# NVIDIA-Merlin/distributed-embeddings

Measured on NVIDIA H100. Metric: DLRM global samples/sec (device-timed, max over ranks), higher is better.
Workload: dtype bf16

## Files before the change

### distributed_embeddings_b200/models/dlrm_fast.py

```python
from __future__ import annotations

import os
from typing import Optional

import torch
from torch import nn

from ..ops import _native
from ..parallel.comm import CommContext
from ..parallel.fused import FusedEngine
from ..utils import nvtx
from ..utils.lr_schedule import LearningRateScheduler
from .dlrm import DLRM


def _pad8(n: int) -> int:
  return (n + 7) // 8 * 8


class _Layer:

  def __init__(self, lin: nn.Linear, relu: bool):
    self.lin = lin
    self.relu = relu
    self.out_f, self.in_f = lin.weight.shape
    self.in_pad = _pad8(self.in_f)
    self.w_off = self.b_off = 0
    self.w_numel = self.out_f * self.in_pad
    self.b_numel = _pad8(self.out_f)


class DLRMTrainStep:

  def __init__(self, model: DLRM, lr: float = 24.0, embedding_optimizer: str = "sgd",
               scheduler: Optional[LearningRateScheduler] = None, use_cuda_graph: bool = True,
               embedding_optimizer_kwargs: Optional[dict] = None, overlap: bool = True,
               gemm: str = "cublas"):
    if gemm not in ("cublas", "fused_dgrad", "tcgen05", "tcgen05_pair"):
      raise ValueError("gemm must be cublas | fused_dgrad | tcgen05 | tcgen05_pair")
    self.gemm = gemm
    self.model = model
    self.emb = model.embedding
    if self.emb.backend != "fused":
      raise ValueError("DLRMTrainStep needs the fused embedding back end")
    self.dev = self.emb.device
    self.ops = _native.require()
    self.world = self.emb.world_size
    self.ctx = CommContext.for_group(self.emb.group, self.dev)
    self.scheduler = scheduler
    self.use_cuda_graph = use_cuda_graph
    self.overlap = overlap
    self.emb.set_optimizer(embedding_optimizer, lr=lr, **(embedding_optimizer_kwargs or {}))
    if self.emb._engine is None:
      self.emb._engine = FusedEngine(self.emb)
    self.engine: FusedEngine = self.emb._engine
    self.n_emb = len(model.table_sizes)
    self.dim = model.embedding_dim
    sp_env = os.environ.get("DE_B200_STREAM_PUSH", "auto")
    self._stream_push = self.world > 1 and (sp_env == "1" or (sp_env == "auto" and self.world >= 4))
    self._push_stream = torch.cuda.Stream(device=self.dev) if self._stream_push else None
    self._push_ready = torch.cuda.Event() if self._stream_push else None

    lins_b = [m for m in model.bottom_mlp.net if isinstance(m, nn.Linear)]
    lins_t = [m for m in model.top_mlp.net if isinstance(m, nn.Linear)]
    self.bottom = [_Layer(l, True) for l in lins_b]
    self.top = [_Layer(l, True) for l in lins_t[:-1]]
    self.head = _Layer(lins_t[-1], False)
    if self.head.out_f != 1:
      raise ValueError("the top MLP must end in a single logit")
    layers = self.bottom + self.top + [self.head]
    self._dp_slots = []
    pos = 0
    if len(self.emb.dp_layers):
      if embedding_optimizer != "sgd":
        raise ValueError("replicated tables in the fast step are updated by the dense SGD "
                         "kernel: use embedding_optimizer='sgd' or data_parallel_threshold=None")
      for layer in self.emb.dp_layers:
        w = layer.embeddings
        self._dp_slots.append((pos, tuple(w.shape)))
        pos += _pad8(w.numel())
    for L in layers:
      L.w_off = pos
      pos += L.w_numel
      L.b_off = pos
      pos += L.b_numel
    self.n_flat = pos
    dev = self.dev
    self.p32 = torch.zeros(pos, dtype=torch.float32, device=dev)
    self.p16 = torch.zeros(pos, dtype=torch.bfloat16, device=dev)
    if self.world > 1:
      self.gsym = self.ctx.alloc_multicast(pos * 4, "dense_grads") or \
          self.ctx.alloc(pos * 4, "dense_grads")
      self.allreduce_kind = "nvls_multimem" if getattr(self.gsym, "mc_ptr", 0) else "p2p"
      self.g32 = self.gsym.view(torch.float32, (pos,))
    else:
      self.gsym = None
      self.allreduce_kind = "none"
      self.g32 = torch.zeros(pos, dtype=torch.float32, device=dev)
    with torch.no_grad():
      dp_targets = []
      for layer, (off, shape) in zip(self.emb.dp_layers, self._dp_slots):
        n = shape[0] * shape[1]
        view = self.p32[off:off + n].view(shape)
        view.copy_(layer.embeddings.data)
        layer.embeddings.data = view
        dp_targets.append(self.g32[off:off + n].view(shape))
      if self._dp_slots:
        self.engine.set_dp_grad_targets(dp_targets)
        self.engine._tables_dirty = True
        self.engine._key = None
      for L in layers:
        wv = self.p32[L.w_off:L.w_off + L.w_numel].view(L.out_f, L.in_pad)
        wv[:, :L.in_f].copy_(L.lin.weight)
        L.lin.weight.data = wv[:, :L.in_f]
        bv = self.p32[L.b_off:L.b_off + L.out_f]
        bv.copy_(L.lin.bias)
        L.lin.bias.data = bv
        L.w16 = self.p16[L.w_off:L.w_off + L.w_numel].view(L.out_f, L.in_pad)
        L.b16 = self.p16[L.b_off:L.b_off + L.out_f]
        L.gw = self.g32[L.w_off:L.w_off + L.w_numel].view(L.out_f, L.in_pad)
        L.gb = self.g32[L.b_off:L.b_off + L.b_numel]
        L.w16T = torch.empty(L.in_pad, L.out_f, dtype=torch.bfloat16, device=dev)
      self.p16.copy_(self.p32)
      self._refresh_transposes()
    self.lr_t = torch.full((1,), float(lr), dtype=torch.float32, device=dev)
    self.engine.share_lr(self.lr_t)
    self.lr = float(lr)
    self.loss = torch.zeros(1, dtype=torch.float32, device=dev)
    self._batch = None
    self._graph = None
    self._side = torch.cuda.Stream(device=dev) if overlap else None
    self._wgrad_overlap = os.environ.get("DE_B200_WGRAD_STREAM", "auto")
    self._wstream = torch.cuda.Stream(device=dev) if overlap else None
    ar_env = os.environ.get("DE_B200_AR_OVERLAP", "auto")
    ar_on = ar_env == "1" or (ar_env == "auto" and self.world >= 4)
    self._ar_stream = torch.cuda.Stream(device=dev) if (overlap and self.world > 1 and ar_on) \
        else None

  def _refresh_transposes(self):
    if self.gemm == "cublas":
      return
    for L in self.bottom[1:] + self.top[1:]:
      L.w16T.copy_(L.w16.t())

  def _linear_fwd(self, L, x):
    if self.gemm in ("tcgen05", "tcgen05_pair"):
      pair = self.gemm == "tcgen05_pair" and L.out_f >= 256
      self.ops.gemm_tn_bias_act(x, L.w16, L.b16, L.y, True, 512 if pair else 0)
    else:
      torch._addmm_activation(L.b16, x, L.w16.t(), out=L.y)
    return L.y

  def _wgrad(self, L, x):
    use = self._wstream is not None and (
        self._wgrad_overlap == "1" or
        (self._wgrad_overlap == "auto" and (self._batch or 0) >= 49152))
    if not use:
      torch.mm(L.dy.t(), x, out_dtype=torch.float32, out=L.gw)
      return
    self._w_used = True
    self._wstream.wait_stream(torch.cuda.current_stream())
    with torch.cuda.stream(self._wstream):
      torch.mm(L.dy.t(), x, out_dtype=torch.float32, out=L.gw)

  def _dgrad_relu(self, L, x_below, dx, gb_below):
    if self.gemm == "cublas":
      torch.mm(L.dy, L.w16, out=dx)
      self.ops.relu_bwd_bias(dx, x_below, gb_below)
    else:
      self.ops.gemm_dgrad_relu_bias(L.dy, L.w16T, x_below, dx, gb_below, 0)

  def _alloc(self, b: int):
    dev, bf = self.dev, torch.bfloat16
    if self._stream_push:
      self.engine.enable_streamed_push(max(1024, -(-b // 16)))
    self.engine.prepare(b, [1] * self.n_emb, ids64=False)
    self.cat_stage = self.engine.in_flat[:self.n_emb * b].view(self.n_emb, b)
    self.num_in = torch.zeros(b, self.bottom[0].in_f, dtype=torch.float32, device=dev)
    self.lab_in = torch.zeros(b, dtype=torch.float32, device=dev)
    self.x0 = torch.zeros(b, self.bottom[0].in_pad, dtype=bf, device=dev)
    for L in self.bottom + self.top:
      L.y = torch.empty(b, L.out_f, dtype=bf, device=dev)
      L.dy = torch.empty(b, L.out_f, dtype=bf, device=dev)
    self.z = torch.zeros(b, self.top[0].in_pad, dtype=bf, device=dev)
    self.dz = torch.empty(b, self.top[0].in_pad, dtype=bf, device=dev)
    self._batch = b
    self._graph = None
    self._stage = [(torch.zeros_like(self.cat_stage), torch.zeros_like(self.num_in),
                    torch.zeros_like(self.lab_in)) for _ in range(2)]
    self._slot_dev = torch.zeros(1, dtype=torch.int32, device=dev)
    self._slot_host = torch.tensor([[0], [1]], dtype=torch.int32).pin_memory()
    self._h2d_done = [torch.cuda.Event(), torch.cuda.Event()]
    self._consumed = [torch.cuda.Event(), torch.cuda.Event()]
    self._prefetched = 0
    self._consumed_n = 0
    self._use_stage = False

  def _forward(self):
    ops = self.ops
    if self._use_stage:
      a, b_ = self._stage
      ops.select_copy([a[0], a[1], a[2]], [b_[0], b_[1], b_[2]],
                      [self.cat_stage, self.num_in, self.lab_in], self._slot_dev)
    eng = self.engine
    if self._side is not None:
      self._side.wait_stream(torch.cuda.current_stream())
      with torch.cuda.stream(self._side):
        eng.launch_forward()
    ops.cast_pad(self.num_in, self.x0)
    x = self.x0
    for L in self.bottom:
      x = self._linear_fwd(L, x)
    if self._side is not None:
      torch.cuda.current_stream().wait_stream(self._side)
    else:
      eng.launch_forward()
    if eng.out_needs_reduce:
      eng.wait_output()
      ops.interact_fwd(x, eng.out, self.n_emb, self.z, [])
    else:
      ops.interact_fwd(x, eng.out, self.n_emb, self.z, eng.sync_out_wait())
    x = self.z
    for L in self.top:
      x = self._linear_fwd(L, x)

  def _backward(self):
    ops, eng = self.ops, self.engine
    b = self._batch
    last = self.top[-1]
    self.loss.zero_()
    H = self.head
    ops.head_loss(last.y, H.w16.view(-1), H.b16, self.lab_in, 1.0 / b, last.dy,
                  H.gw.view(-1), H.gb, last.gb, self.loss, None)
    for i in range(len(self.top) - 1, -1, -1):
      L = self.top[i]
      x = self.top[i - 1].y if i > 0 else self.z
      dx = self.top[i - 1].dy if i > 0 else self.dz
      self._wgrad(L, x)
      if i > 0:
        self._dgrad_relu(L, x, dx, self.top[i - 1].gb)
      else:
        torch.mm(L.dy, L.w16, out=dx)
    if self._ar_stream is not None:
      ar = self._ar_stream
      ar.wait_stream(torch.cuda.current_stream())
      if getattr(self, "_w_used", False):
        ar.wait_stream(self._wstream)
      off = self.top[0].w_off
      with torch.cuda.stream(ar):
        self.ctx.allreduce_(self.gsym, self.n_flat - off, torch.float32, scale=1.0 / self.world,
                            byte_offset=off * 4, max_blocks=32)
    hb = self.bottom[-1]
    pushed = eng.streamed_push
    if pushed:
      eng.push_counters.zero_()
      self._push_ready.record(torch.cuda.current_stream())
      ops.interact_bwd(hb.y, eng.out, self.n_emb, self.dz, hb.dy, 0, 0, 1.0, eng.routes_stage,
                       len(eng.routes_stage_np), [], eng.push_counters, eng.push_chunk_rows)
      self._push_stream.wait_event(self._push_ready)
      with torch.cuda.stream(self._push_stream):
        eng.launch_streamed_push()
    else:
      ops.interact_bwd(hb.y, eng.out, self.n_emb, self.dz, hb.dy, 0, 0, 1.0, eng.routes_all,
                       len(eng.routes_all_np), eng.sync_grad_signal(), None, 0)
    if self._side is not None:
      self._side.wait_stream(torch.cuda.current_stream())
      if pushed:
        self._side.wait_stream(self._push_stream)
      with torch.cuda.stream(self._side):
        eng.backward_inplace()
    else:
      if pushed:
        torch.cuda.current_stream().wait_stream(self._push_stream)
      eng.backward_inplace()
    ops.relu_bwd_bias(hb.dy, hb.y, hb.gb)
    for i in range(len(self.bottom) - 1, -1, -1):
      L = self.bottom[i]
      x = self.bottom[i - 1].y if i > 0 else self.x0
      self._wgrad(L, x)
      if i > 0:
        self._dgrad_relu(L, x, self.bottom[i - 1].dy, self.bottom[i - 1].gb)
    if self._dp_slots and self._side is not None:
      torch.cuda.current_stream().wait_stream(self._side)
    if getattr(self, "_w_used", False):
      torch.cuda.current_stream().wait_stream(self._wstream)
      self._w_used = False
    if self.world > 1:
      if self._ar_stream is not None:
        ar = self._ar_stream
        ar.wait_stream(torch.cuda.current_stream())
        with torch.cuda.stream(ar):
          self.ctx.allreduce_(self.gsym, self.top[0].w_off, torch.float32, scale=1.0 / self.world)
        torch.cuda.current_stream().wait_stream(ar)
      else:
        self.ctx.allreduce_(self.gsym, self.n_flat, torch.float32, scale=1.0 / self.world)
    ops.dense_sgd(self.p32, self.p16, self.g32, self.lr_t, 1.0)
    self._refresh_transposes()
    if self._side is not None:
      torch.cuda.current_stream().wait_stream(self._side)

  def _step_impl(self):
    with nvtx.range("dlrm_forward"):
      self._forward()
    with nvtx.range("dlrm_backward_update"):
      self._backward()

  def set_lr(self, lr: float):
    self.lr = float(lr)
    self.lr_t.fill_(self.lr)
    if self.emb._fused_optimizer is not None:
      self.emb._fused_optimizer["lr"] = self.lr

  def load_batch(self, numerical, categorical, labels):
    b = int(numerical.shape[0])
    if b != self._batch:
      self._alloc(b)
    self.num_in.copy_(numerical, non_blocking=True)
    self.lab_in.copy_(labels.reshape(-1), non_blocking=True)
    if isinstance(categorical, (list, tuple)):
      for v, c in zip(self.engine.in_views, categorical):
        v.copy_(c.reshape(v.shape), non_blocking=True)
    else:
      self.cat_stage.copy_(categorical, non_blocking=True)

  def prefetch(self, numerical, categorical, labels):
    b = int(numerical.shape[0])
    if b != self._batch:
      self._alloc(b)
    if not self._use_stage:
      self._use_stage = True
      self._graph = None
      self._copy_stream = torch.cuda.Stream(device=self.dev)
    slot = self._prefetched & 1
    cs = self._copy_stream
    if self._prefetched >= 2:
      cs.wait_event(self._consumed[slot])
    with torch.cuda.stream(cs):
      st = self._stage[slot]
      st[0].copy_(categorical, non_blocking=True)
      st[1].copy_(numerical, non_blocking=True)
      st[2].copy_(labels.reshape(-1), non_blocking=True)
      self._h2d_done[slot].record(cs)
    self._prefetched += 1

  def run_prefetched(self) -> torch.Tensor:
    assert self._consumed_n < self._prefetched, "call prefetch() first"
    slot = self._consumed_n & 1
    main = torch.cuda.current_stream()
    main.wait_event(self._h2d_done[slot])
    self._slot_dev.copy_(self._slot_host[slot], non_blocking=True)
    loss = self.run()
    self._consumed[slot].record(main)
    self._consumed_n += 1
    return loss

  def run(self) -> torch.Tensor:
    if self.scheduler is not None:
      self.set_lr(self.scheduler.step())
    if not self.use_cuda_graph:
      self._step_impl()
      return self.loss
    if self._graph is None:
      self.lr_t.zero_()
      self.engine.dry_updates(True)
      s = torch.cuda.Stream(device=self.dev)
      s.wait_stream(torch.cuda.current_stream())
      with torch.cuda.stream(s):
        for _ in range(2):
          self._step_impl()
      torch.cuda.current_stream().wait_stream(s)
      torch.cuda.synchronize()
      self.engine.dry_updates(False)
      g = torch.cuda.CUDAGraph()
      with torch.cuda.graph(g):
        self._step_impl()
      self._graph = g
      self.set_lr(self.lr)
    self._graph.replay()
    return self.loss

  def step(self, numerical, categorical, labels) -> torch.Tensor:
    self.load_batch(numerical, categorical, labels)
    return self.run()
```

### distributed_embeddings_b200/ops/_native.py

```python
from __future__ import annotations

import os
import threading

import numpy as np
import torch

_PKG_DIR = os.path.dirname(os.path.dirname(os.path.abspath(__file__)))
SO_PATH = os.path.join(_PKG_DIR, "_C.so")

_lock = threading.Lock()
_loaded = False
_error = None

INPUT_DESC = np.dtype([
    ("table", "<u8"),
    ("ids", "<u8"),
    ("offsets", "<u8"),
    ("ids_off", "<i8"),
    ("id_shift", "<i8"),
    ("sub_rows", "<i8"),
    ("row_base", "<i8"),
    ("width", "<i4"),
    ("hotness", "<i4"),
    ("dst_col", "<i4"),
    ("combiner", "<i4"),
    ("local_table", "<i4"),
    ("flags", "<i4"),
    ("item_off", "<i8"),
    ("pad1", "<i8"),
])
TABLE_DESC = np.dtype([
    ("weight", "<u8"),
    ("state0", "<u8"),
    ("state1", "<u8"),
    ("rows", "<i8"),
    ("key_base", "<i8"),
    ("width", "<i4"),
    ("pad", "<i4"),
])

GRAD_ROUTE = np.dtype([
    ("dst", "<u8"),
    ("dst_stride", "<i8"),
    ("src_col", "<i4"),
    ("width", "<i4"),
    ("dst_col", "<i4"),
    ("pad", "<i4"),
])
SYNC_STATE_WORDS = 64
DTYPE_CODE = {torch.float32: 0, torch.bfloat16: 1, torch.float16: 2}

OPT_SGD, OPT_ADAGRAD, OPT_ROWWISE_ADAGRAD, OPT_ADAM, OPT_EMIT = 0, 1, 2, 3, 4
MAX_PEERS = 16


def load(required: bool = False) -> bool:
  global _loaded, _error
  if _loaded:
    return True
  with _lock:
    if _loaded:
      return True
    if _error is not None and not required:
      return False
    try:
      if not os.path.exists(SO_PATH):
        raise FileNotFoundError(
            f"{SO_PATH} is missing - run `python -m distributed_embeddings_b200.ops._build` "
            "(or `make`) to compile the sm_90a kernels")
      torch.ops.load_library(SO_PATH)
      sizes = list(torch.ops.de_b200.struct_sizes())
      mine = [INPUT_DESC.itemsize, TABLE_DESC.itemsize, MAX_PEERS, GRAD_ROUTE.itemsize,
              SYNC_STATE_WORDS]
      if sizes != mine:
        raise RuntimeError(f"descriptor layout mismatch: native {sizes} vs python {mine} "
                           "(stale _C.so? rebuild with python -m distributed_embeddings_b200.ops._build)")
      _loaded = True
      return True
    except Exception as e:
      _error = e
      if required:
        raise
      return False


def available() -> bool:
  return load(required=False)


_KERNELS_PER_OP = {
    "lookup_fwd": 1, "scatter_add_bwd": 1, "sort_items": 12, "segment_update": 1,
    "sync_only": 1, "push_segments": 1, "push_grad": 1, "rowslice_reduce": 1,
    "embedding_lookup_fwd": 1, "embedding_scatter_add": 1, "embedding_lookup_grad": 14,
    "row_to_split": 1, "hash_init": 1, "integer_lookup": 1, "barrier": 1, "allreduce": 1,
    "gather_segments": 1, "gather_ragged": 1, "copy_cast_2d": 1, "dense_sgd": 1, "interact_fwd": 1, "interact_bwd": 1,
    "relu_bwd_bias": 1, "head_loss": 1, "select_copy": 1, "cast_pad": 1, "gemm_tn_bias_act": 1, "gemm_dgrad_relu_bias": 1,
}
_launches = 0


class _OpsProxy:

  def __init__(self, ns):
    self._ns = ns
    self._cache = {}

  def __getattr__(self, name):
    fn = self._cache.get(name)
    if fn is None:
      raw = getattr(self._ns, name)
      k = _KERNELS_PER_OP.get(name, 0)

      def fn(*args, __raw=raw, __k=k, **kwargs):
        global _launches
        _launches += __k
        return __raw(*args, **kwargs)

      self._cache[name] = fn
    return fn


_proxy = None


def reset_launch_count():
  global _launches
  _launches = 0


def launch_count() -> int:
  return _launches


def require():
  global _proxy
  if not load(required=False):
    raise RuntimeError(
        "distributed_embeddings_b200: the native sm_90a extension is required for CUDA tensors "
        f"but could not be loaded ({_error!r}). There is no eager fallback on GPU.")
  if _proxy is None:
    _proxy = _OpsProxy(torch.ops.de_b200)
  return _proxy


def ops():
  return require()


def upload_struct_array(arr: np.ndarray, device) -> torch.Tensor:
  raw = torch.from_numpy(np.frombuffer(arr.tobytes(), dtype=np.uint8).copy())
  return raw.to(device)
```

### distributed_embeddings_b200/ops/csrc/bindings.cpp

```cpp
#include <ATen/cuda/CUDAContext.h>
#include <c10/cuda/CUDAGuard.h>
#include <c10/cuda/CUDAStream.h>
#include <cuda_runtime.h>
#include <torch/library.h>
#include <torch/torch.h>

#include <cstdlib>
#include <cstring>
#include <mutex>
#include <string>
#include <unordered_map>
#include <vector>

#include "de_b200.h"

namespace {

using at::Tensor;

#define DE_CUDA_CHECK(expr)                                                              \
  do {                                                                                   \
    cudaError_t _e = (expr);                                                             \
    TORCH_CHECK(_e == cudaSuccess, "CUDA error in " #expr ": ", cudaGetErrorString(_e)); \
  } while (0)

cudaStream_t cur_stream() { return at::cuda::getCurrentCUDAStream().stream(); }

int sm_count() {
  static int cached = -1;
  if (cached < 0) cached = at::cuda::getCurrentDeviceProperties()->multiProcessorCount;
  return cached;
}

de::PeerPtrs to_peers(at::IntArrayRef ptrs) {
  TORCH_CHECK(ptrs.size() <= de::kMaxPeers, "at most ", de::kMaxPeers, " peers are supported");
  de::PeerPtrs p;
  std::memset(&p, 0, sizeof(p));
  for (size_t i = 0; i < ptrs.size(); ++i) p.p[i] = reinterpret_cast<void*>(ptrs[i]);
  return p;
}

void check_launch() {
  cudaError_t e = cudaGetLastError();
  TORCH_CHECK(e == cudaSuccess, "kernel launch failed: ", cudaGetErrorString(e));
}

struct SyncCtx {
  de::PeerPtrs flags;
  uint32_t* state;
  int* error_flag;
  unsigned long long timeout;
  int rank, world;
};
std::vector<SyncCtx>& sync_ctxs() {
  static std::vector<SyncCtx> v;
  return v;
}
std::mutex& sync_mutex() {
  static std::mutex m;
  return m;
}

int64_t sync_ctx_create(at::IntArrayRef flag_ptrs, Tensor state, int64_t rank, int64_t world,
                        int64_t timeout_cycles, int64_t error_ptr) {
  TORCH_CHECK(state.is_cuda() && state.scalar_type() == at::kInt && state.is_contiguous() &&
                  state.numel() >= de::kSyncStateWords,
              "sync state must be an int32 CUDA tensor of >= ", de::kSyncStateWords, " words");
  SyncCtx c;
  c.flags = to_peers(flag_ptrs);
  c.state = reinterpret_cast<uint32_t*>(state.data_ptr<int>());
  c.error_flag = reinterpret_cast<int*>(error_ptr);
  c.timeout = static_cast<unsigned long long>(timeout_cycles);
  c.rank = static_cast<int>(rank);
  c.world = static_cast<int>(world);
  std::lock_guard<std::mutex> lock(sync_mutex());
  sync_ctxs().push_back(c);
  return static_cast<int64_t>(sync_ctxs().size()) - 1;
}

de::SyncArgs to_sync(at::IntArrayRef spec) {
  de::SyncArgs a = de::no_sync();
  if (spec.size() == 0) return a;
  TORCH_CHECK(spec.size() == 5, "sync spec = {handle, wait_ch, wait_abs_ch, signal_ch, slot}");
  SyncCtx c;
  {
    std::lock_guard<std::mutex> lock(sync_mutex());
    TORCH_CHECK(spec[0] >= 0 && spec[0] < static_cast<int64_t>(sync_ctxs().size()),
                "unknown sync context");
    c = sync_ctxs()[spec[0]];
  }
  for (int i = 1; i <= 3; ++i)
    TORCH_CHECK(spec[i] >= -1 && spec[i] < de::kSyncChannels, "sync channel out of range");
  TORCH_CHECK(spec[4] >= 0 && spec[4] < 2 * de::kSyncChannels, "sync counter slot out of range");
  a.flags = c.flags;
  a.state = c.state;
  a.error_flag = c.error_flag;
  a.timeout = c.timeout;
  a.rank = c.rank;
  a.world = c.world;
  a.wait_ch = static_cast<int32_t>(spec[1]);
  a.wait_abs_ch = static_cast<int32_t>(spec[2]);
  a.signal_ch = static_cast<int32_t>(spec[3]);
  a.counter_slot = static_cast<int32_t>(spec[4]);
  return a;
}

int dtype_code(at::ScalarType t) {
  if (t == at::kFloat) return 0;
  if (t == at::kBFloat16) return 1;
  if (t == at::kHalf) return 2;
  TORCH_CHECK(false, "activations / gradients must be fp32, bf16 or fp16");
  return -1;
}

void sync_only(at::IntArrayRef sync) {
  de::launch_sync_only(to_sync(sync), cur_stream());
  check_launch();
}

std::vector<int64_t> struct_sizes() {
  return {static_cast<int64_t>(sizeof(de::InputDesc)), static_cast<int64_t>(sizeof(de::TableDesc)),
          static_cast<int64_t>(de::kMaxPeers), static_cast<int64_t>(sizeof(de::GradRoute)),
          static_cast<int64_t>(de::kSyncStateWords)};
}

void lookup_fwd(const Tensor& descs, int64_t n_inputs, int64_t batch, int64_t src_batch,
                int64_t dst_batch, int64_t dst_stride, at::IntArrayRef src_ptrs,
                at::IntArrayRef dst_ptrs, int64_t rot, bool ids64, int64_t act_dtype, bool vec4,
                at::IntArrayRef sync, int64_t tile_samples, int64_t table_dtype, bool vec8) {
  TORCH_CHECK(descs.is_cuda(), "descs must live on the GPU");
  TORCH_CHECK(table_dtype >= 0 && table_dtype <= 2, "table_dtype: 0 fp32, 1 bf16, 2 fp16");
  c10::cuda::CUDAGuard guard(descs.device());
  de::launch_lookup_fwd(reinterpret_cast<const de::InputDesc*>(descs.data_ptr()),
                        static_cast<int>(n_inputs), batch, src_batch, dst_batch, dst_stride,
                        to_peers(src_ptrs), to_peers(dst_ptrs), static_cast<int>(rot), ids64,
                        static_cast<int>(act_dtype), vec4, sm_count(), cur_stream(),
                        to_sync(sync), static_cast<int>(tile_samples),
                        static_cast<int>(table_dtype), vec8);
  check_launch();
}

void scatter_add_bwd(const Tensor& descs, int64_t n_inputs, int64_t batch, int64_t src_batch,
                     int64_t grad_batch, int64_t grad_stride, at::IntArrayRef src_ptrs,
                     at::IntArrayRef grad_ptrs, int64_t rot, double scale, int64_t scale_ptr,
                     bool ids64, int64_t act_dtype, bool vec4, bool vec8, at::IntArrayRef sync,
                     bool staged) {
  TORCH_CHECK(descs.is_cuda(), "descs must live on the GPU");
  c10::cuda::CUDAGuard guard(descs.device());
  de::launch_scatter_add_bwd(reinterpret_cast<const de::InputDesc*>(descs.data_ptr()),
                             static_cast<int>(n_inputs), batch, src_batch, grad_batch, grad_stride,
                             to_peers(src_ptrs), to_peers(grad_ptrs), static_cast<int>(rot),
                             static_cast<float>(scale), reinterpret_cast<const float*>(scale_ptr),
                             ids64, static_cast<int>(act_dtype), vec4, sm_count(), cur_stream(),
                             vec8, to_sync(sync), staged);
  check_launch();
}

int bit_length(int64_t v) {
  int b = 0;
  while (v > 0) {
    ++b;
    v >>= 1;
  }
  return b < 1 ? 1 : b;
}

bool use_own_sort() {
  static const bool own = [] {
    const char* v = std::getenv("DE_B200_SORT");
    return !(v != nullptr && std::string(v) == "cub");
  }();
  return own;
}

std::tuple<Tensor, Tensor> radix_sort_pairs(const Tensor& keys, const Tensor& items,
                                            int64_t end_bit) {
  TORCH_CHECK(keys.is_cuda() && keys.scalar_type() == at::kLong && keys.is_contiguous());
  TORCH_CHECK(items.is_cuda() && items.scalar_type() == at::kInt && items.is_contiguous() &&
              items.numel() == keys.numel());
  c10::cuda::CUDAGuard guard(keys.device());
  const int64_t n = keys.numel();
  TORCH_CHECK(n < (int64_t(1) << 31), "own radix sort: too many items");
  Tensor ka = keys.clone(), ia = items.clone();
  Tensor kb = at::empty_like(ka), ib = at::empty_like(ia);
  if (n == 0) return {ka, ia};
  Tensor temp = at::empty({static_cast<int64_t>(de::radix_sort_temp_bytes(n))},
                          at::TensorOptions().device(keys.device()).dtype(at::kByte));
  int where = de::radix_sort_pairs(temp.data_ptr(), ka.data_ptr<int64_t>(),
                                   reinterpret_cast<uint32_t*>(ia.data_ptr<int>()),
                                   kb.data_ptr<int64_t>(),
                                   reinterpret_cast<uint32_t*>(ib.data_ptr<int>()), n,
                                   static_cast<int>(end_bit), cur_stream());
  check_launch();
  if (where == 0) return {ka, ia};
  return {kb, ib};
}

std::tuple<Tensor, Tensor> radix_sort_pairs32(const Tensor& keys, const Tensor& items,
                                              int64_t end_bit) {
  TORCH_CHECK(keys.is_cuda() && keys.scalar_type() == at::kInt && keys.is_contiguous());
  TORCH_CHECK(items.is_cuda() && items.scalar_type() == at::kInt && items.is_contiguous() &&
              items.numel() == keys.numel());
  c10::cuda::CUDAGuard guard(keys.device());
  const int64_t n = keys.numel();
  TORCH_CHECK(n < (int64_t(1) << 31), "own radix sort: too many items");
  Tensor ka = keys.clone(), ia = items.clone();
  Tensor kb = at::empty_like(ka), ib = at::empty_like(ia);
  Tensor out = at::empty({n}, keys.options().dtype(at::kLong));
  if (n == 0) return {out, ia};
  Tensor temp = at::empty({static_cast<int64_t>(de::radix_sort_temp_bytes(n))},
                          at::TensorOptions().device(keys.device()).dtype(at::kByte));
  int where = de::radix_sort_pairs32(
      temp.data_ptr(), reinterpret_cast<uint32_t*>(ka.data_ptr<int>()),
      reinterpret_cast<uint32_t*>(ia.data_ptr<int>()),
      reinterpret_cast<uint32_t*>(kb.data_ptr<int>()),
      reinterpret_cast<uint32_t*>(ib.data_ptr<int>()), out.data_ptr<int64_t>(), n,
      static_cast<int>(end_bit), cur_stream());
  check_launch();
  return {out, where == 0 ? ia : ib};
}

std::tuple<Tensor, Tensor> head_segments(const Tensor& sorted_keys) {
  TORCH_CHECK(sorted_keys.is_cuda() && sorted_keys.scalar_type() == at::kLong &&
              sorted_keys.is_contiguous());
  c10::cuda::CUDAGuard guard(sorted_keys.device());
  const int64_t n = sorted_keys.numel();
  auto i64 = at::TensorOptions().device(sorted_keys.device()).dtype(at::kLong);
  Tensor seg_start = at::empty({n + 1}, i64);
  Tensor n_unique = at::zeros({1}, i64);
  if (n == 0) return {seg_start, n_unique};
  Tensor temp = at::empty({static_cast<int64_t>(de::head_segments_temp_bytes(n))},
                          at::TensorOptions().device(sorted_keys.device()).dtype(at::kByte));
  de::head_segments(temp.data_ptr(), sorted_keys.data_ptr<int64_t>(), n,
                    seg_start.data_ptr<int64_t>(), n_unique.data_ptr<int64_t>(), cur_stream());
  check_launch();
  return {seg_start, n_unique};
}

std::tuple<Tensor, Tensor, Tensor, Tensor> sort_items(const Tensor& descs, const Tensor& tables,
                                                      int64_t n_tables, int64_t n_inputs,
                                                      int64_t batch, int64_t src_batch,
                                                      at::IntArrayRef src_ptrs, bool ids64,
                                                      int64_t n_items, int64_t total_rows,
                                                      bool prefill_sentinel) {
  TORCH_CHECK(descs.is_cuda() && tables.is_cuda());
  TORCH_CHECK(n_inputs * batch < (int64_t(1) << 32),
              "sorted update: n_inputs * batch = ", n_inputs * batch, " does not fit 32-bit items");
  c10::cuda::CUDAGuard guard(descs.device());
  auto stream = cur_stream();
  auto i64 = at::TensorOptions().device(descs.device()).dtype(at::kLong);
  auto i32 = at::TensorOptions().device(descs.device()).dtype(at::kInt);
  Tensor keys = prefill_sentinel ? at::full({n_items}, total_rows, i64) : at::empty({n_items}, i64);
  Tensor keys_sorted = at::empty({n_items}, i64);
  Tensor items = at::empty({n_items}, i32), items_sorted = at::empty({n_items}, i32);
  Tensor seg_start = at::empty({n_items + 1}, i64);
  Tensor n_unique = at::zeros({1}, i64);
  if (n_items == 0) return {keys_sorted, items_sorted, seg_start, n_unique};
  if (use_own_sort() && total_rows < (int64_t(1) << 32) - 1) {
    TORCH_CHECK(n_items < (int64_t(1) << 31), "own radix sort: too many items");
    Tensor k32a = prefill_sentinel
                      ? at::full({n_items}, static_cast<int64_t>(static_cast<int32_t>(
                                                static_cast<uint32_t>(total_rows))), i32)
                      : at::empty({n_items}, i32);
    Tensor k32b = at::empty({n_items}, i32);
    de::launch_build_keys(reinterpret_cast<const de::InputDesc*>(descs.data_ptr()),
                          reinterpret_cast<const de::TableDesc*>(tables.data_ptr()),
                          static_cast<int>(n_tables), static_cast<int>(n_inputs), batch,
                          src_batch, to_peers(src_ptrs), ids64, k32a.data_ptr(),
                          reinterpret_cast<uint32_t*>(items.data_ptr<int>()), sm_count(), stream,
                          true);
    check_launch();
    size_t sort_bytes = de::radix_sort_temp_bytes(n_items);
    size_t head_bytes = de::head_segments_temp_bytes(n_items);
    Tensor temp = at::empty({static_cast<int64_t>(std::max(sort_bytes, head_bytes))},
                            at::TensorOptions().device(descs.device()).dtype(at::kByte));
    int where = de::radix_sort_pairs32(
        temp.data_ptr(), reinterpret_cast<uint32_t*>(k32a.data_ptr<int>()),
        reinterpret_cast<uint32_t*>(items.data_ptr<int>()),
        reinterpret_cast<uint32_t*>(k32b.data_ptr<int>()),
        reinterpret_cast<uint32_t*>(items_sorted.data_ptr<int>()),
        keys_sorted.data_ptr<int64_t>(), n_items, bit_length(total_rows), stream);
    if (where == 0) std::swap(items, items_sorted);
    de::head_segments(temp.data_ptr(), keys_sorted.data_ptr<int64_t>(), n_items,
                      seg_start.data_ptr<int64_t>(), n_unique.data_ptr<int64_t>(), stream);
    check_launch();
    return {keys_sorted, items_sorted, seg_start, n_unique};
  }
  de::launch_build_keys(reinterpret_cast<const de::InputDesc*>(descs.data_ptr()),
                        reinterpret_cast<const de::TableDesc*>(tables.data_ptr()),
                        static_cast<int>(n_tables), static_cast<int>(n_inputs), batch, src_batch,
                        to_peers(src_ptrs), ids64, keys.data_ptr<int64_t>(),
                        reinterpret_cast<uint32_t*>(items.data_ptr<int>()), sm_count(), stream);
  check_launch();
  if (use_own_sort()) {
    TORCH_CHECK(n_items < (int64_t(1) << 31), "own radix sort: too many items");
    size_t sort_bytes = de::radix_sort_temp_bytes(n_items);
    size_t head_bytes = de::head_segments_temp_bytes(n_items);
    Tensor temp = at::empty({static_cast<int64_t>(std::max(sort_bytes, head_bytes))},
                            at::TensorOptions().device(descs.device()).dtype(at::kByte));
    int where = de::radix_sort_pairs(temp.data_ptr(), keys.data_ptr<int64_t>(),
                                     reinterpret_cast<uint32_t*>(items.data_ptr<int>()),
                                     keys_sorted.data_ptr<int64_t>(),
                                     reinterpret_cast<uint32_t*>(items_sorted.data_ptr<int>()),
                                     n_items, bit_length(total_rows), stream);
    if (where == 0) {
      std::swap(keys, keys_sorted);
      std::swap(items, items_sorted);
    }
    de::head_segments(temp.data_ptr(), keys_sorted.data_ptr<int64_t>(), n_items,
                      seg_start.data_ptr<int64_t>(), n_unique.data_ptr<int64_t>(), stream);
    check_launch();
    return {keys_sorted, items_sorted, seg_start, n_unique};
  }
  size_t sort_bytes = de::sort_pairs_temp_bytes(n_items);
  size_t uniq_bytes = de::unique_temp_bytes(n_items);
  Tensor temp = at::empty({static_cast<int64_t>(std::max(sort_bytes, uniq_bytes)) + 16},
                          at::TensorOptions().device(descs.device()).dtype(at::kByte));
  de::sort_pairs(temp.data_ptr(), sort_bytes, keys.data_ptr<int64_t>(),
                 keys_sorted.data_ptr<int64_t>(),
                 reinterpret_cast<const uint32_t*>(items.data_ptr<int>()),
                 reinterpret_cast<uint32_t*>(items_sorted.data_ptr<int>()), n_items,
                 bit_length(total_rows), stream);
  de::unique_segments(temp.data_ptr(), uniq_bytes, keys_sorted.data_ptr<int64_t>(), n_items,
                      seg_start.data_ptr<int64_t>(), n_unique.data_ptr<int64_t>(), stream);
  check_launch();
  return {keys_sorted, items_sorted, seg_start, n_unique};
}

void segment_update(const Tensor& descs, const Tensor& tables, int64_t n_tables, int64_t batch,
                    int64_t grad_batch, int64_t grad_stride, at::IntArrayRef grad_ptrs,
                    const Tensor& sorted_keys, const Tensor& sorted_items, const Tensor& seg_start,
                    const Tensor& n_unique, int64_t opt_kind, double lr, double eps, double beta1,
                    double beta2, double bias1, double bias2, double grad_scale,
                    double weight_decay, int64_t lr_ptr, const c10::optional<Tensor>& emit_keys,
                    const c10::optional<Tensor>& emit_rows, int64_t max_width, int64_t act_dtype,
                    bool vec4, const c10::optional<Tensor>& scratch, int64_t step_ptr,
                    int64_t table_dtype) {
  c10::cuda::CUDAGuard guard(descs.device());
  TORCH_CHECK(table_dtype >= 0 && table_dtype <= 2, "table_dtype: 0 fp32, 1 bf16, 2 fp16");
  de::OptimizerArgs opt;
  opt.kind = static_cast<int32_t>(opt_kind);
  opt.lr = static_cast<float>(lr);
  opt.eps = static_cast<float>(eps);
  opt.beta1 = static_cast<float>(beta1);
  opt.beta2 = static_cast<float>(beta2);
  opt.bias1 = static_cast<float>(bias1);
  opt.bias2 = static_cast<float>(bias2);
  opt.grad_scale = static_cast<float>(grad_scale);
  opt.weight_decay = static_cast<float>(weight_decay);
  opt.lr_ptr = reinterpret_cast<const float*>(lr_ptr);
  opt.step_ptr = reinterpret_cast<const float*>(step_ptr);
  if (opt.kind == de::kOptEmit) TORCH_CHECK(emit_keys.has_value() && emit_rows.has_value());
  if (scratch.has_value() && vec4 && max_width <= 128 && opt.kind != de::kOptEmit) {
    const int64_t n_items = sorted_keys.numel();
    const int64_t sw = (max_width + 3) / 4 * 4;
    TORCH_CHECK(scratch->scalar_type() == at::kFloat && scratch->is_contiguous() &&
                    scratch->numel() >= ((n_items + 31) / 32) * sw,
                "scratch too small for the balanced update");
    bool ok = de::launch_balanced_update(
        reinterpret_cast<const de::InputDesc*>(descs.data_ptr()),
        reinterpret_cast<const de::TableDesc*>(tables.data_ptr()), static_cast<int>(n_tables),
        batch, grad_batch, grad_stride, to_peers(grad_ptrs), sorted_keys.data_ptr<int64_t>(),
        reinterpret_cast<const uint32_t*>(sorted_items.data_ptr<int>()), n_items,
        seg_start.data_ptr<int64_t>(), n_unique.data_ptr<int64_t>(), opt,
        scratch->data_ptr<float>(), static_cast<int>(sw), static_cast<int>(max_width),
        static_cast<int>(act_dtype), sm_count(), cur_stream(), static_cast<int>(table_dtype));
    TORCH_CHECK(ok, "balanced update launch failed");
    check_launch();
    return;
  }
  de::launch_segment_update(
      reinterpret_cast<const de::InputDesc*>(descs.data_ptr()),
      reinterpret_cast<const de::TableDesc*>(tables.data_ptr()), static_cast<int>(n_tables), batch,
      grad_batch, grad_stride, to_peers(grad_ptrs), sorted_keys.data_ptr<int64_t>(),
      reinterpret_cast<const uint32_t*>(sorted_items.data_ptr<int>()),
      seg_start.data_ptr<int64_t>(), n_unique.data_ptr<int64_t>(), sorted_keys.numel(), opt,
      emit_keys.has_value() ? emit_keys->data_ptr<int64_t>() : nullptr,
      emit_rows.has_value() ? emit_rows->data_ptr<float>() : nullptr, static_cast<int>(max_width),
      static_cast<int>(act_dtype), vec4, sm_count(), cur_stream(), static_cast<int>(table_dtype));
  check_launch();
}

Tensor upload_bytes(const void* host, size_t bytes, const at::Device& dev) {
  Tensor t = at::empty({static_cast<int64_t>(bytes)},
                       at::TensorOptions().device(dev).dtype(at::kByte));
  DE_CUDA_CHECK(cudaMemcpyAsync(t.data_ptr(), host, bytes, cudaMemcpyHostToDevice, cur_stream()));
  return t;
}

de::InputDesc single_desc(const void* table, const Tensor& values,
                          const c10::optional<Tensor>& offsets, int64_t hotness, int64_t rows,
                          int64_t width, int64_t combiner) {
  de::InputDesc d;
  std::memset(&d, 0, sizeof(d));
  d.table = table;
  d.ids = values.data_ptr();
  d.offsets = offsets.has_value() ? offsets->data_ptr<int64_t>() : nullptr;
  d.sub_rows = rows;
  d.width = static_cast<int32_t>(width);
  d.hotness = offsets.has_value() ? 0 : static_cast<int32_t>(hotness);
  d.combiner = static_cast<int32_t>(combiner);
  return d;
}

void check_ids(const Tensor& values, const c10::optional<Tensor>& offsets) {
  TORCH_CHECK(values.is_cuda() && values.is_contiguous(), "ids must be a contiguous CUDA tensor");
  TORCH_CHECK(values.scalar_type() == at::kInt || values.scalar_type() == at::kLong,
              "ids must be int32 or int64");
  if (offsets.has_value())
    TORCH_CHECK(offsets->is_cuda() && offsets->scalar_type() == at::kLong &&
                    offsets->is_contiguous(),
                "row_splits must be a contiguous int64 CUDA tensor");
}

Tensor embedding_lookup_fwd(const Tensor& param, const Tensor& values,
                            const c10::optional<Tensor>& offsets, int64_t hotness, int64_t batch,
                            int64_t combiner, bool out_bf16) {
  const auto pt = param.scalar_type();
  TORCH_CHECK(param.is_cuda() && param.dim() == 2 &&
                  (pt == at::kFloat || pt == at::kBFloat16 || pt == at::kHalf) &&
                  param.is_contiguous(),
              "param must be a contiguous fp32, bf16 or fp16 [rows, width] CUDA tensor");
  check_ids(values, offsets);
  c10::cuda::CUDAGuard guard(param.device());
  const int64_t width = param.size(1);
  const int tdt = dtype_code(pt);
  Tensor out = at::empty({batch, width}, param.options().dtype(out_bf16 ? at::kBFloat16 : pt));
  if (batch == 0) return out;
  de::InputDesc d = single_desc(param.data_ptr(), values, offsets, hotness, param.size(0), width,
                                combiner);
  Tensor dd = upload_bytes(&d, sizeof(d), param.device());
  de::PeerPtrs src, dst;
  std::memset(&src, 0, sizeof(src));
  std::memset(&dst, 0, sizeof(dst));
  dst.p[0] = out.data_ptr();
  const int64_t avg_hot = std::max<int64_t>(1, values.numel() / std::max<int64_t>(batch, 1));
  int64_t lanes_per_row = 1;
  while (lanes_per_row < (width + 3) / 4 && lanes_per_row < 32) lanes_per_row *= 2;
  const int64_t ts = std::max<int64_t>(32 / lanes_per_row, std::min<int64_t>(32, 64 / avg_hot));
  de::launch_lookup_fwd(reinterpret_cast<const de::InputDesc*>(dd.data_ptr()), 1, batch, batch,
                        batch, width, src, dst, 0, values.scalar_type() == at::kLong,
                        out_bf16 ? 1 : tdt, width % 4 == 0, sm_count(), cur_stream(),
                        de::no_sync(), static_cast<int>(std::max<int64_t>(1, ts)), tdt,
                        width % 8 == 0 && reinterpret_cast<uintptr_t>(param.data_ptr()) % 16 == 0);
  check_launch();
  return out;
}

void embedding_scatter_add(Tensor dst, const Tensor& values, const c10::optional<Tensor>& offsets,
                           int64_t hotness, int64_t batch, int64_t combiner, const Tensor& grad,
                           double scale) {
  TORCH_CHECK(dst.is_cuda() && dst.dim() == 2 && dst.scalar_type() == at::kFloat &&
              dst.is_contiguous());
  TORCH_CHECK(grad.is_cuda() && grad.dim() == 2 && grad.stride(1) == 1);
  check_ids(values, offsets);
  if (batch == 0) return;
  c10::cuda::CUDAGuard guard(dst.device());
  const int64_t width = dst.size(1);
  de::InputDesc d = single_desc(dst.data_ptr(), values, offsets, hotness, dst.size(0), width,
                                combiner);
  Tensor dd = upload_bytes(&d, sizeof(d), dst.device());
  de::PeerPtrs src, gp;
  std::memset(&src, 0, sizeof(src));
  std::memset(&gp, 0, sizeof(gp));
  gp.p[0] = grad.data_ptr();
  const int gdt = dtype_code(grad.scalar_type());
  const int64_t gstride = grad.stride(0);
  const bool vec4 = (width % 4 == 0) && (gstride % 4 == 0) &&
                    (reinterpret_cast<uintptr_t>(grad.data_ptr()) % 16 == 0);
  de::launch_scatter_add_bwd(reinterpret_cast<const de::InputDesc*>(dd.data_ptr()), 1, batch,
                             batch, batch, gstride, src, gp, 0, static_cast<float>(scale), nullptr,
                             values.scalar_type() == at::kLong, gdt, vec4, sm_count(),
                             cur_stream(), false, de::no_sync());
  check_launch();
}

std::tuple<Tensor, Tensor> embedding_lookup_grad(const Tensor& values,
                                                 const c10::optional<Tensor>& offsets,
                                                 int64_t hotness, int64_t batch, int64_t combiner,
                                                 const Tensor& grad, int64_t num_rows) {
  TORCH_CHECK(grad.is_cuda() && grad.dim() == 2 && grad.stride(1) == 1);
  check_ids(values, offsets);
  c10::cuda::CUDAGuard guard(grad.device());
  const int64_t width = grad.size(1);
  const int64_t n_items = values.numel();
  auto f32 = grad.options().dtype(at::kFloat);
  auto i64 = grad.options().dtype(at::kLong);
  if (n_items == 0) return {at::empty({0}, i64), at::empty({0, width}, f32)};
  de::InputDesc d = single_desc(nullptr, values, offsets, hotness, num_rows, width, combiner);
  de::TableDesc t;
  std::memset(&t, 0, sizeof(t));
  t.rows = num_rows;
  t.width = static_cast<int32_t>(width);
  Tensor dd = upload_bytes(&d, sizeof(d), grad.device());
  Tensor td = upload_bytes(&t, sizeof(t), grad.device());
  auto sorted = sort_items(dd, td, 1, 1, batch, batch, {}, values.scalar_type() == at::kLong,
                           n_items, num_rows, false);
  Tensor emit_keys = at::empty({n_items}, i64);
  Tensor emit_rows = at::empty({n_items, width}, f32);
  const int gdt = dtype_code(grad.scalar_type());
  const int64_t gstride = grad.stride(0);
  const bool vec4 = (width % 4 == 0) && (gstride % 4 == 0) &&
                    (reinterpret_cast<uintptr_t>(grad.data_ptr()) % 16 == 0);
  std::vector<int64_t> gp = {reinterpret_cast<int64_t>(grad.data_ptr())};
  segment_update(dd, td, 1, batch, batch, gstride, gp, std::get<0>(sorted), std::get<1>(sorted),
                 std::get<2>(sorted), std::get<3>(sorted), de::kOptEmit, 0, 0, 0, 0, 1, 1, 1.0, 0, 0,
                 emit_keys, emit_rows, width, gdt, vec4, c10::nullopt, 0, 0);
  int64_t n_unique = std::get<3>(sorted).item<int64_t>();
  if (n_unique > 0) {
    int64_t last = emit_keys.narrow(0, n_unique - 1, 1).item<int64_t>();
    if (last >= num_rows) --n_unique;
  }
  return {emit_keys.narrow(0, 0, n_unique), emit_rows.narrow(0, 0, n_unique)};
}

Tensor row_to_split(const Tensor& indices, int64_t num_rows) {
  TORCH_CHECK(indices.is_cuda() && indices.dim() == 2 && indices.size(1) == 2 &&
                  indices.scalar_type() == at::kLong && indices.is_contiguous(),
              "indices must be a contiguous int64 [nnz, 2] CUDA tensor");
  c10::cuda::CUDAGuard guard(indices.device());
  Tensor splits = at::empty({num_rows + 1}, indices.options());
  de::launch_row_to_split(indices.data_ptr<int64_t>(), indices.size(0), num_rows,
                          splits.data_ptr<int64_t>(), cur_stream());
  check_launch();
  return splits;
}

void hash_init(Tensor table) {
  TORCH_CHECK(table.is_cuda() && table.scalar_type() == at::kLong && table.is_contiguous());
  c10::cuda::CUDAGuard guard(table.device());
  de::launch_hash_init(table.data_ptr<int64_t>(), table.numel() / 2, cur_stream());
  check_launch();
}

Tensor integer_lookup(Tensor table, Tensor count, Tensor next_index, const Tensor& keys,
                      int64_t capacity) {
  TORCH_CHECK(table.is_cuda() && count.is_cuda() && next_index.is_cuda() && keys.is_cuda());
  TORCH_CHECK(table.scalar_type() == at::kLong && keys.scalar_type() == at::kLong &&
              next_index.scalar_type() == at::kLong && count.scalar_type() == at::kInt);
  c10::cuda::CUDAGuard guard(table.device());
  Tensor k = keys.contiguous();
  Tensor out = at::empty_like(k);
  de::launch_integer_lookup(table.data_ptr<int64_t>(), table.numel() / 2,
                            reinterpret_cast<uint32_t*>(count.data_ptr<int>()),
                            next_index.data_ptr<int64_t>(), k.data_ptr<int64_t>(), k.numel(),
                            capacity, out.data_ptr<int64_t>(), cur_stream());
  check_launch();
  return out;
}

void barrier(at::IntArrayRef flag_ptrs, Tensor epoch, int64_t rank, int64_t world, int64_t channel,
             int64_t timeout_cycles, int64_t error_ptr) {
  c10::cuda::CUDAGuard guard(epoch.device());
  de::launch_barrier(to_peers(flag_ptrs), reinterpret_cast<uint32_t*>(epoch.data_ptr<int>()),
                     static_cast<int>(rank), static_cast<int>(world), static_cast<int>(channel),
                     static_cast<unsigned long long>(timeout_cycles),
                     reinterpret_cast<int*>(error_ptr), cur_stream());
  check_launch();
}

void allreduce(at::IntArrayRef buf_ptrs, at::IntArrayRef flag_ptrs, Tensor epoch, int64_t rank,
               int64_t world, int64_t n_elems, double scale, bool bf16, int64_t channel,
               int64_t timeout_cycles, int64_t error_ptr, int64_t mc_ptr, int64_t max_blocks) {
  c10::cuda::CUDAGuard guard(epoch.device());
  if (mc_ptr != 0) {
    de::launch_allreduce_multimem(reinterpret_cast<void*>(mc_ptr), to_peers(flag_ptrs),
                                  reinterpret_cast<uint32_t*>(epoch.data_ptr<int>()),
                                  static_cast<int>(rank), static_cast<int>(world), n_elems,
                                  static_cast<float>(scale), bf16, static_cast<int>(channel),
                                  static_cast<unsigned long long>(timeout_cycles),
                                  reinterpret_cast<int*>(error_ptr), sm_count(), cur_stream(),
                         static_cast<int>(max_blocks));
  } else {
    de::launch_allreduce(to_peers(buf_ptrs), to_peers(flag_ptrs),
                         reinterpret_cast<uint32_t*>(epoch.data_ptr<int>()),
                         static_cast<int>(rank), static_cast<int>(world), n_elems,
                         static_cast<float>(scale), bf16, static_cast<int>(channel),
                         static_cast<unsigned long long>(timeout_cycles),
                         reinterpret_cast<int*>(error_ptr), sm_count(), cur_stream(),
                         static_cast<int>(max_blocks));
  }
  check_launch();
}

void p2p_store_bench(const Tensor& src, int64_t dst_ptr, int64_t n_rows, int64_t row_bytes,
                     int64_t vec_bytes, int64_t dst_stride, int64_t unroll, int64_t blocks,
                     int64_t threads) {
  TORCH_CHECK(src.is_cuda() && src.is_contiguous() &&
              src.numel() * src.element_size() >= n_rows * row_bytes);
  TORCH_CHECK(row_bytes % vec_bytes == 0 && (vec_bytes == 4 || vec_bytes == 8 || vec_bytes == 16));
  TORCH_CHECK((row_bytes / vec_bytes >= 32 && (row_bytes / vec_bytes) % 32 == 0) ||
              32 % (row_bytes / vec_bytes) == 0);
  TORCH_CHECK(unroll >= 1 && unroll <= 8 && threads % 32 == 0 && threads <= 1024);
  c10::cuda::CUDAGuard guard(src.device());
  de::launch_p2p_store_bench(src.data_ptr(), reinterpret_cast<void*>(dst_ptr), n_rows,
                             static_cast<int>(row_bytes), static_cast<int>(vec_bytes), dst_stride,
                             static_cast<int>(unroll), static_cast<int>(blocks),
                             static_cast<int>(threads), cur_stream());
  check_launch();
}

void push_segments(const Tensor& segs, const Tensor& src, at::IntArrayRef dst_ptrs,
                   int64_t max_seg_elems, at::IntArrayRef sync) {
  TORCH_CHECK(segs.is_cuda() && segs.scalar_type() == at::kLong && segs.is_contiguous() &&
              segs.dim() == 2 && segs.size(1) == 4);
  TORCH_CHECK(src.is_cuda() && src.is_contiguous() &&
              (src.element_size() == 4 || src.element_size() == 8));
  c10::cuda::CUDAGuard guard(src.device());
  de::launch_push_segments(segs.data_ptr<int64_t>(), static_cast<int>(segs.size(0)),
                           src.data_ptr(), to_peers(dst_ptrs),
                           static_cast<int>(src.element_size()), max_seg_elems, sm_count(),
                           cur_stream(), to_sync(sync));
  check_launch();
}

void push_grad(const Tensor& routes, int64_t n_routes, const Tensor& src, int64_t dst_dtype,
               double scale, at::IntArrayRef sync) {
  TORCH_CHECK(routes.is_cuda() && routes.scalar_type() == at::kByte &&
              routes.numel() >= n_routes * static_cast<int64_t>(sizeof(de::GradRoute)));
  TORCH_CHECK(src.is_cuda() && src.dim() == 2 && src.stride(1) == 1);
  c10::cuda::CUDAGuard guard(src.device());
  de::launch_push_grad(reinterpret_cast<const de::GradRoute*>(routes.data_ptr()),
                       static_cast<int>(n_routes), src.data_ptr(), src.stride(0),
                       dtype_code(src.scalar_type()), static_cast<int>(dst_dtype), src.size(0),
                       static_cast<float>(scale), sm_count(), cur_stream(), to_sync(sync));
  check_launch();
}

void stream_push(at::IntArrayRef src_ptrs, at::IntArrayRef dst_ptrs, at::IntArrayRef row_bytes,
                 const Tensor& counters, int64_t chunk_rows, int64_t rows, int64_t blocks,
                 at::IntArrayRef sync) {
  TORCH_CHECK(src_ptrs.size() == dst_ptrs.size() && src_ptrs.size() == row_bytes.size() &&
              src_ptrs.size() <= de::kMaxPeers);
  TORCH_CHECK(counters.is_cuda() && counters.scalar_type() == at::kInt && chunk_rows > 0 &&
              counters.numel() >= (rows + chunk_rows - 1) / chunk_rows);
  de::PushPlan plan;
  std::memset(&plan, 0, sizeof(plan));
  plan.n = static_cast<int32_t>(src_ptrs.size());
  for (size_t i = 0; i < src_ptrs.size(); ++i) {
    TORCH_CHECK(row_bytes[i] % 16 == 0 && src_ptrs[i] % 16 == 0 && dst_ptrs[i] % 16 == 0,
                "streamed push needs 16-byte aligned rows");
    plan.src[i] = reinterpret_cast<const void*>(src_ptrs[i]);
    plan.dst[i] = reinterpret_cast<void*>(dst_ptrs[i]);
    plan.row_bytes[i] = row_bytes[i];
  }
  c10::cuda::CUDAGuard guard(counters.device());
  de::SyncArgs sa = to_sync(sync);
  de::launch_stream_push(plan, reinterpret_cast<const uint32_t*>(counters.data_ptr<int>()),
                         static_cast<int>(chunk_rows), rows, sa.timeout, sa.error_flag,
                         static_cast<int>(blocks), cur_stream(), sa);
  check_launch();
}

void rowslice_reduce(const Tensor& partial, int64_t out_ptr, int64_t out_stride,
                     int64_t out_dtype, const Tensor& cols) {
  TORCH_CHECK(partial.is_cuda() && partial.dim() == 3 && partial.scalar_type() == at::kFloat &&
              partial.is_contiguous());
  TORCH_CHECK(cols.is_cuda() && cols.scalar_type() == at::kInt && cols.is_contiguous() &&
              cols.dim() == 2 && cols.size(1) == 3);
  c10::cuda::CUDAGuard guard(partial.device());
  de::launch_rowslice_reduce(partial.data_ptr<float>(), static_cast<int>(partial.size(0)),
                             partial.size(1), partial.size(2), reinterpret_cast<void*>(out_ptr),
                             out_stride, static_cast<int>(out_dtype), cols.data_ptr<int>(),
                             static_cast<int>(cols.size(0)), cur_stream());
  check_launch();
}

void gather_segments(const Tensor& segs, at::IntArrayRef src_ptrs, Tensor dst,
                     int64_t max_seg_elems) {
  TORCH_CHECK(segs.is_cuda() && segs.scalar_type() == at::kLong && segs.is_contiguous());
  TORCH_CHECK(dst.is_cuda() && dst.is_contiguous());
  c10::cuda::CUDAGuard guard(dst.device());
  de::launch_gather_segments(segs.data_ptr<int64_t>(), static_cast<int>(segs.size(0)),
                             to_peers(src_ptrs), dst.data_ptr(),
                             static_cast<int>(dst.element_size()), max_seg_elems, cur_stream());
  check_launch();
}

void gather_ragged(const Tensor& segs, at::IntArrayRef val_ptrs, at::IntArrayRef split_ptrs,
                   Tensor dst_vals, Tensor goff, int64_t b, int64_t max_cap) {
  TORCH_CHECK(segs.is_cuda() && segs.scalar_type() == at::kLong && segs.is_contiguous());
  TORCH_CHECK(goff.is_cuda() && goff.scalar_type() == at::kLong && dst_vals.is_cuda());
  c10::cuda::CUDAGuard guard(dst_vals.device());
  de::launch_gather_ragged(segs.data_ptr<int64_t>(), static_cast<int>(segs.size(0)),
                           to_peers(val_ptrs), to_peers(split_ptrs), dst_vals.data_ptr(),
                           goff.data_ptr<int64_t>(), b, static_cast<int>(val_ptrs.size()),
                           static_cast<int>(dst_vals.element_size()), max_cap, cur_stream());
  check_launch();
}

void select_copy(at::TensorList src0, at::TensorList src1, at::TensorList dst,
                 const Tensor& slot_flag) {
  TORCH_CHECK(src0.size() == dst.size() && src1.size() == dst.size() && dst.size() <= 4);
  TORCH_CHECK(slot_flag.is_cuda() && slot_flag.scalar_type() == at::kInt);
  const void* s0[4];
  const void* s1[4];
  void* d[4];
  int64_t nb[4];
  for (size_t i = 0; i < dst.size(); ++i) {
    TORCH_CHECK(src0[i].is_contiguous() && src1[i].is_contiguous() && dst[i].is_contiguous());
    nb[i] = dst[i].numel() * dst[i].element_size();
    TORCH_CHECK(src0[i].numel() * src0[i].element_size() == nb[i] &&
                src1[i].numel() * src1[i].element_size() == nb[i] && nb[i] % 16 == 0,
                "select_copy segments must match and be multiples of 16 bytes");
    s0[i] = src0[i].data_ptr();
    s1[i] = src1[i].data_ptr();
    d[i] = dst[i].data_ptr();
  }
  c10::cuda::CUDAGuard guard(slot_flag.device());
  de::launch_select_copy(s0, s1, d, nb, static_cast<int>(dst.size()), slot_flag.data_ptr<int>(),
                         sm_count(), cur_stream());
  check_launch();
}

void copy_cast_2d(const Tensor& src, int64_t dst_ptr, int64_t dst_stride, int64_t dst_dtype,
                  double scale) {
  TORCH_CHECK(src.is_cuda() && src.dim() == 2 && src.stride(1) == 1);
  c10::cuda::CUDAGuard guard(src.device());
  de::launch_copy_cast_2d(src.data_ptr(), src.stride(0), reinterpret_cast<void*>(dst_ptr),
                          dst_stride, src.size(0), src.size(1), dtype_code(src.scalar_type()),
                          static_cast<int>(dst_dtype), static_cast<float>(scale), cur_stream());
  check_launch();
}

void check_bf16_2d(const Tensor& t, const char* name) {
  TORCH_CHECK(t.is_cuda() && t.dim() == 2 && t.scalar_type() == at::kBFloat16 && t.stride(1) == 1,
              name, " must be a 2-D bf16 CUDA tensor with unit inner stride");
}

void interact_fwd(const Tensor& bottom, const Tensor& emb, int64_t n_emb, Tensor z,
                  at::IntArrayRef sync) {
  check_bf16_2d(bottom, "bottom");
  check_bf16_2d(emb, "emb");
  check_bf16_2d(z, "z");
  c10::cuda::CUDAGuard guard(bottom.device());
  const int64_t dim = bottom.size(1);
  TORCH_CHECK(emb.size(1) == n_emb * dim);
  const int64_t need = (n_emb + 1) * n_emb / 2 + dim;
  TORCH_CHECK(z.size(1) >= need, "z is too narrow");
  bool ok = de::launch_interact_fwd(bottom.data_ptr(), bottom.stride(0), emb.data_ptr(),
                                    emb.stride(0), static_cast<int>(n_emb), static_cast<int>(dim),
                                    z.data_ptr(), z.stride(0), static_cast<int>(z.size(1)),
                                    bottom.size(0), sm_count(), cur_stream(), to_sync(sync));
  TORCH_CHECK(ok, "unsupported interaction shape (n_emb <= 31, dim in {16,32,64,128})");
  check_launch();
}

void interact_bwd(const Tensor& bottom, const Tensor& emb, int64_t n_emb, const Tensor& dz,
                  Tensor dbottom, int64_t demb_ptr, int64_t demb_stride, double emb_grad_scale,
                  const c10::optional<Tensor>& routes, int64_t n_routes, at::IntArrayRef sync,
                  const c10::optional<Tensor>& done_counters, int64_t chunk_rows) {
  check_bf16_2d(bottom, "bottom");
  check_bf16_2d(emb, "emb");
  check_bf16_2d(dz, "dz");
  check_bf16_2d(dbottom, "dbottom");
  if (routes.has_value())
    TORCH_CHECK(routes->is_cuda() && routes->scalar_type() == at::kByte &&
                routes->numel() >= n_routes * static_cast<int64_t>(sizeof(de::GradRoute)));
  c10::cuda::CUDAGuard guard(bottom.device());
  const int64_t dim = bottom.size(1);
  bool ok = de::launch_interact_bwd(bottom.data_ptr(), bottom.stride(0), emb.data_ptr(),
                                    emb.stride(0), static_cast<int>(n_emb), static_cast<int>(dim),
                                    dz.data_ptr(), dz.stride(0), dbottom.data_ptr(),
                                    dbottom.stride(0), reinterpret_cast<void*>(demb_ptr),
                                    demb_stride, static_cast<float>(emb_grad_scale),
                                    bottom.size(0), sm_count(), cur_stream(),
                                    routes.has_value()
                                        ? reinterpret_cast<const de::GradRoute*>(routes->data_ptr())
                                        : nullptr,
                                    static_cast<int>(n_routes), to_sync(sync),
                                    done_counters.has_value()
                                        ? reinterpret_cast<uint32_t*>(done_counters->data_ptr<int>())
                                        : nullptr,
                                    static_cast<int>(chunk_rows));
  TORCH_CHECK(ok, "unsupported interaction shape (n_emb <= 31, dim in {32,64,128}; routed / "
                  "signalling launches need dim in {64,128} and 16-byte aligned rows)");
  check_launch();
}

void avgpool_fwd(const Tensor& x, int64_t n, Tensor out, int64_t stride) {
  check_bf16_2d(x, "x");
  check_bf16_2d(out, "out");
  const int64_t out_len = (n + stride - 1) / stride;
  TORCH_CHECK(x.size(1) >= n && out.size(1) >= out_len && out.size(0) == x.size(0));
  const int64_t pad = std::max<int64_t>(0, (out_len - 1) * stride + stride - n);
  c10::cuda::CUDAGuard guard(x.device());
  de::launch_avgpool_fwd(x.data_ptr(), x.stride(0), static_cast<int>(n), out.data_ptr(),
                         out.stride(0), static_cast<int>(out_len), static_cast<int>(stride),
                         static_cast<int>(pad / 2), x.size(0), cur_stream());
  check_launch();
}

void avgpool_bwd(const Tensor& dout, Tensor dx, int64_t n, int64_t stride) {
  check_bf16_2d(dout, "dout");
  check_bf16_2d(dx, "dx");
  const int64_t out_len = (n + stride - 1) / stride;
  TORCH_CHECK(dx.size(1) >= n && dout.size(1) >= out_len && dout.size(0) == dx.size(0));
  const int64_t pad = std::max<int64_t>(0, (out_len - 1) * stride + stride - n);
  c10::cuda::CUDAGuard guard(dx.device());
  de::launch_avgpool_bwd(dout.data_ptr(), dout.stride(0), static_cast<int>(out_len),
                         dx.data_ptr(), dx.stride(0), static_cast<int>(n),
                         static_cast<int>(stride), static_cast<int>(pad / 2), dx.size(0),
                         cur_stream());
  check_launch();
}

void relu_bwd_bias(Tensor dy, const Tensor& y, Tensor db) {
  check_bf16_2d(dy, "dy");
  check_bf16_2d(y, "y");
  TORCH_CHECK(dy.is_contiguous() && y.is_contiguous() && dy.size(1) % 8 == 0);
  TORCH_CHECK(db.is_cuda() && db.scalar_type() == at::kFloat && db.numel() >= dy.size(1));
  c10::cuda::CUDAGuard guard(dy.device());
  de::launch_relu_bwd_bias(dy.data_ptr(), y.data_ptr(), db.data_ptr<float>(), dy.size(0),
                           static_cast<int>(dy.size(1)), cur_stream());
  check_launch();
}

void head_loss(const Tensor& x, const Tensor& w, const Tensor& bias, const Tensor& labels,
               double inv_batch, Tensor dx, Tensor dw, Tensor db, Tensor dbias_prev,
               Tensor loss_sum, const c10::optional<Tensor>& logits) {
  check_bf16_2d(x, "x");
  TORCH_CHECK(x.is_contiguous() && dx.is_contiguous());
  TORCH_CHECK(w.scalar_type() == at::kBFloat16 && bias.scalar_type() == at::kBFloat16);
  TORCH_CHECK(labels.scalar_type() == at::kFloat && labels.is_contiguous());
  c10::cuda::CUDAGuard guard(x.device());
  bool ok = de::launch_head_loss(x.data_ptr(), static_cast<int>(x.size(1)), w.data_ptr(),
                                 bias.data_ptr(), labels.data_ptr<float>(), x.size(0),
                                 static_cast<float>(inv_batch), dx.data_ptr(),
                                 dw.data_ptr<float>(), db.data_ptr<float>(),
                                 dbias_prev.data_ptr<float>(), loss_sum.data_ptr<float>(),
                                 logits.has_value() ? logits->data_ptr<float>() : nullptr,
                                 sm_count(), cur_stream());
  TORCH_CHECK(ok, "head_loss supports K in {64,128,256,512,1024}");
  check_launch();
}

void dense_sgd(Tensor p32, Tensor p16, Tensor g32, const Tensor& lr, double grad_scale) {
  TORCH_CHECK(p32.is_cuda() && p32.scalar_type() == at::kFloat && g32.scalar_type() == at::kFloat &&
              p16.scalar_type() == at::kBFloat16 && lr.scalar_type() == at::kFloat);
  TORCH_CHECK(p32.numel() % 4 == 0 && p32.numel() == g32.numel() && p32.numel() == p16.numel());
  c10::cuda::CUDAGuard guard(p32.device());
  de::launch_sgd_update(p32.data_ptr<float>(), p16.data_ptr(), g32.data_ptr<float>(),
                        lr.data_ptr<float>(), static_cast<float>(grad_scale), p32.numel(),
                        sm_count(), cur_stream());
  check_launch();
}

void cast_pad(const Tensor& src, Tensor dst) {
  TORCH_CHECK(src.is_cuda() && src.scalar_type() == at::kFloat && src.is_contiguous());
  TORCH_CHECK(dst.scalar_type() == at::kBFloat16 && dst.is_contiguous() &&
              dst.size(0) == src.size(0) && dst.size(1) >= src.size(1));
  c10::cuda::CUDAGuard guard(src.device());
  de::launch_cast_pad(src.data_ptr<float>(), static_cast<int>(src.size(1)), dst.data_ptr(),
                      static_cast<int>(dst.size(1)), src.size(0), cur_stream());
  check_launch();
}

void gemm_tn_bias_act(const Tensor& a, const Tensor& b, const c10::optional<Tensor>& bias,
                      Tensor out, bool relu, int64_t block_n) {
  check_bf16_2d(a, "a");
  check_bf16_2d(b, "b");
  check_bf16_2d(out, "out");
  TORCH_CHECK(a.size(1) == b.size(1) && out.size(0) == a.size(0) && out.size(1) == b.size(0),
              "shape mismatch");
  if (bias.has_value())
    TORCH_CHECK(bias->is_cuda() && bias->scalar_type() == at::kBFloat16 && bias->is_contiguous() &&
                bias->numel() == b.size(0));
  c10::cuda::CUDAGuard guard(a.device());
  bool ok = de::launch_gemm_tn_bias_act(
      a.data_ptr(), a.stride(0), b.data_ptr(), b.stride(0),
      bias.has_value() ? bias->data_ptr() : nullptr, out.data_ptr(), out.stride(0),
      static_cast<int>(a.size(0)), static_cast<int>(b.size(0)), static_cast<int>(a.size(1)), relu,
      static_cast<int>(block_n), sm_count(), cur_stream());
  TORCH_CHECK(ok, "gemm_tn_bias_act: unsupported shape/alignment or launch failure");
  check_launch();
}

void gemm_dgrad_relu_bias(const Tensor& dy, const Tensor& wt, const Tensor& act, Tensor dx,
                          Tensor colsum, int64_t block_n) {
  check_bf16_2d(dy, "dy");
  check_bf16_2d(wt, "wt");
  check_bf16_2d(act, "act");
  check_bf16_2d(dx, "dx");
  TORCH_CHECK(dy.size(1) == wt.size(1) && dx.size(0) == dy.size(0) && dx.size(1) == wt.size(0) &&
              act.size(0) == dx.size(0) && act.size(1) == dx.size(1), "shape mismatch");
  TORCH_CHECK(colsum.is_cuda() && colsum.scalar_type() == at::kFloat &&
              colsum.numel() >= dx.size(1));
  c10::cuda::CUDAGuard guard(dy.device());
  bool ok = de::launch_gemm_tn_fused(
      dy.data_ptr(), dy.stride(0), wt.data_ptr(), wt.stride(0), nullptr, dx.data_ptr(),
      dx.stride(0), static_cast<int>(dy.size(0)), static_cast<int>(wt.size(0)),
      static_cast<int>(dy.size(1)), 2, act.data_ptr(), act.stride(0), colsum.data_ptr<float>(),
      static_cast<int>(block_n), sm_count(), cur_stream());
  TORCH_CHECK(ok, "gemm_dgrad_relu_bias: unsupported shape/alignment or launch failure");
  check_launch();
}

Tensor symm_alloc(int64_t nbytes, int64_t device_index) {
  c10::cuda::CUDAGuard guard(static_cast<c10::DeviceIndex>(device_index));
  void* ptr = nullptr;
  const size_t padded = (static_cast<size_t>(nbytes) + 255) & ~static_cast<size_t>(255);
  DE_CUDA_CHECK(cudaMalloc(&ptr, padded));
  DE_CUDA_CHECK(cudaMemset(ptr, 0, padded));
  DE_CUDA_CHECK(cudaDeviceSynchronize());
  auto deleter = [](void* p) { cudaFree(p); };
  return at::from_blob(ptr, {static_cast<int64_t>(padded)}, deleter,
                       at::TensorOptions()
                           .device(at::Device(at::kCUDA, static_cast<c10::DeviceIndex>(device_index)))
                           .dtype(at::kByte));
}

Tensor ipc_get_handle(const Tensor& buf) {
  TORCH_CHECK(buf.is_cuda());
  cudaIpcMemHandle_t h;
  DE_CUDA_CHECK(cudaIpcGetMemHandle(&h, buf.data_ptr()));
  Tensor out = at::empty({static_cast<int64_t>(sizeof(h))}, at::TensorOptions().dtype(at::kByte));
  std::memcpy(out.data_ptr(), &h, sizeof(h));
  return out;
}

int64_t ipc_open(const Tensor& handle, int64_t device_index) {
  TORCH_CHECK(!handle.is_cuda() && handle.numel() == sizeof(cudaIpcMemHandle_t));
  c10::cuda::CUDAGuard guard(static_cast<c10::DeviceIndex>(device_index));
  cudaIpcMemHandle_t h;
  std::memcpy(&h, handle.data_ptr(), sizeof(h));
  void* ptr = nullptr;
  DE_CUDA_CHECK(cudaIpcOpenMemHandle(&ptr, h, cudaIpcMemLazyEnablePeerAccess));
  return reinterpret_cast<int64_t>(ptr);
}

void ipc_close(int64_t ptr, int64_t device_index) {
  c10::cuda::CUDAGuard guard(static_cast<c10::DeviceIndex>(device_index));
  cudaIpcCloseMemHandle(reinterpret_cast<void*>(ptr));
}

int64_t host_device_pointer(const Tensor& host) {
  TORCH_CHECK(!host.is_cuda());
  void* dptr = nullptr;
  DE_CUDA_CHECK(cudaHostGetDevicePointer(&dptr, host.data_ptr(), 0));
  return reinterpret_cast<int64_t>(dptr);
}

}

TORCH_LIBRARY(de_b200, m) {
  m.def("struct_sizes() -> int[]", &struct_sizes);
  m.def(
      "sync_ctx_create(int[] flag_ptrs, Tensor state, int rank, int world, int timeout_cycles, "
      "int error_ptr) -> int",
      &sync_ctx_create);
  m.def("sync_only(int[] sync) -> ()", &sync_only);
  m.def(
      "lookup_fwd(Tensor descs, int n_inputs, int batch, int src_batch, int dst_batch, "
      "int dst_stride, int[] src_ptrs, int[] dst_ptrs, int rot, bool ids64, int act_dtype, "
      "bool vec4, int[] sync, int tile_samples, int table_dtype=0, bool vec8=False) -> ()",
      &lookup_fwd);
  m.def(
      "scatter_add_bwd(Tensor descs, int n_inputs, int batch, int src_batch, int grad_batch, "
      "int grad_stride, int[] src_ptrs, int[] grad_ptrs, int rot, float scale, int scale_ptr, bool ids64, "
      "int act_dtype, bool vec4, bool vec8, int[] sync, bool staged) -> ()",
      &scatter_add_bwd);
  m.def(
      "sort_items(Tensor descs, Tensor tables, int n_tables, int n_inputs, int batch, "
      "int src_batch, int[] src_ptrs, bool ids64, int n_items, int total_rows, "
      "bool prefill_sentinel) -> "
      "(Tensor, Tensor, Tensor, Tensor)",
      &sort_items);
  m.def("radix_sort_pairs(Tensor keys, Tensor items, int end_bit) -> (Tensor, Tensor)",
        &radix_sort_pairs);
  m.def("radix_sort_pairs32(Tensor keys, Tensor items, int end_bit) -> (Tensor, Tensor)",
        &radix_sort_pairs32);
  m.def("head_segments(Tensor sorted_keys) -> (Tensor, Tensor)", &head_segments);
  m.def(
      "segment_update(Tensor descs, Tensor tables, int n_tables, int batch, int grad_batch, "
      "int grad_stride, int[] grad_ptrs, Tensor sorted_keys, Tensor sorted_items, "
      "Tensor seg_start, Tensor n_unique, int opt_kind, float lr, float eps, float beta1, "
      "float beta2, float bias1, float bias2, float grad_scale, float weight_decay, int lr_ptr, "
      "Tensor? emit_keys, Tensor? emit_rows, int max_width, int act_dtype, bool vec4, "
      "Tensor? scratch, int step_ptr, int table_dtype=0) -> ()",
      &segment_update);
  m.def(
      "embedding_lookup_fwd(Tensor param, Tensor values, Tensor? offsets, int hotness, int batch, "
      "int combiner, bool out_bf16) -> Tensor",
      &embedding_lookup_fwd);
  m.def(
      "embedding_scatter_add(Tensor(a!) dst, Tensor values, Tensor? offsets, int hotness, "
      "int batch, int combiner, Tensor grad, float scale) -> ()",
      &embedding_scatter_add);
  m.def(
      "embedding_lookup_grad(Tensor values, Tensor? offsets, int hotness, int batch, int combiner, "
      "Tensor grad, int num_rows) -> (Tensor, Tensor)",
      &embedding_lookup_grad);
  m.def("row_to_split(Tensor indices, int num_rows) -> Tensor", &row_to_split);
  m.def("hash_init(Tensor(a!) table) -> ()", &hash_init);
  m.def(
      "integer_lookup(Tensor(a!) table, Tensor(b!) count, Tensor(c!) next_index, Tensor keys, "
      "int capacity) -> Tensor",
      &integer_lookup);
  m.def(
      "barrier(int[] flag_ptrs, Tensor(a!) epoch, int rank, int world, int channel, "
      "int timeout_cycles, int error_ptr) -> ()",
      &barrier);
  m.def(
      "allreduce(int[] buf_ptrs, int[] flag_ptrs, Tensor(a!) epoch, int rank, int world, "
      "int n_elems, float scale, bool bf16, int channel, int timeout_cycles, "
      "int error_ptr, int mc_ptr, int max_blocks) -> ()",
      &allreduce);
  m.def("gather_segments(Tensor segs, int[] src_ptrs, Tensor(a!) dst, int max_seg_elems) -> ()",
        &gather_segments);
  m.def(
      "p2p_store_bench(Tensor src, int dst_ptr, int n_rows, int row_bytes, int vec_bytes, "
      "int dst_stride, int unroll, int blocks, int threads) -> ()",
      &p2p_store_bench);
  m.def(
      "push_segments(Tensor segs, Tensor src, int[] dst_ptrs, int max_seg_elems, int[] sync) -> ()",
      &push_segments);
  m.def(
      "push_grad(Tensor routes, int n_routes, Tensor src, int dst_dtype, float scale, int[] sync) "
      "-> ()",
      &push_grad);
  m.def(
      "stream_push(int[] src_ptrs, int[] dst_ptrs, int[] row_bytes, Tensor counters, "
      "int chunk_rows, int rows, int blocks, int[] sync) -> ()",
      &stream_push);
  m.def(
      "rowslice_reduce(Tensor partial, int out_ptr, int out_stride, int out_dtype, Tensor cols) "
      "-> ()",
      &rowslice_reduce);
  m.def(
      "gather_ragged(Tensor segs, int[] val_ptrs, int[] split_ptrs, Tensor(a!) dst_vals, "
      "Tensor(b!) goff, int b, int max_cap) -> ()",
      &gather_ragged);
  m.def("select_copy(Tensor[] src0, Tensor[] src1, Tensor(a!)[] dst, Tensor slot_flag) -> ()",
        &select_copy);
  m.def("copy_cast_2d(Tensor src, int dst_ptr, int dst_stride, int dst_dtype, float scale) -> ()",
        &copy_cast_2d);
  m.def("interact_fwd(Tensor bottom, Tensor emb, int n_emb, Tensor(a!) z, int[] sync) -> ()",
        &interact_fwd);
  m.def(
      "interact_bwd(Tensor bottom, Tensor emb, int n_emb, Tensor dz, Tensor(a!) dbottom, "
      "int demb_ptr, int demb_stride, float emb_grad_scale, Tensor? routes, int n_routes, "
      "int[] sync, Tensor? done_counters, int chunk_rows) -> ()",
      &interact_bwd);
  m.def("avgpool_fwd(Tensor x, int n, Tensor(a!) out, int stride) -> ()", &avgpool_fwd);
  m.def("avgpool_bwd(Tensor dout, Tensor(a!) dx, int n, int stride) -> ()", &avgpool_bwd);
  m.def("relu_bwd_bias(Tensor(a!) dy, Tensor y, Tensor(b!) db) -> ()", &relu_bwd_bias);
  m.def(
      "head_loss(Tensor x, Tensor w, Tensor bias, Tensor labels, float inv_batch, Tensor(a!) dx, "
      "Tensor(b!) dw, Tensor(c!) db, Tensor(d!) dbias_prev, Tensor(e!) loss_sum, Tensor? logits) "
      "-> ()",
      &head_loss);
  m.def(
      "dense_sgd(Tensor(a!) p32, Tensor(b!) p16, Tensor(c!) g32, Tensor lr, float grad_scale) "
      "-> ()",
      &dense_sgd);
  m.def("cast_pad(Tensor src, Tensor(a!) dst) -> ()", &cast_pad);
  m.def(
      "gemm_tn_bias_act(Tensor a, Tensor b, Tensor? bias, Tensor(a!) out, bool relu, int block_n) "
      "-> ()",
      &gemm_tn_bias_act);
  m.def(
      "gemm_dgrad_relu_bias(Tensor dy, Tensor wt, Tensor act, Tensor(a!) dx, Tensor(b!) colsum, "
      "int block_n) -> ()",
      &gemm_dgrad_relu_bias);
  m.def("symm_alloc(int nbytes, int device_index) -> Tensor", &symm_alloc);
  m.def("ipc_get_handle(Tensor buf) -> Tensor", &ipc_get_handle);
  m.def("ipc_open(Tensor handle, int device_index) -> int", &ipc_open);
  m.def("ipc_close(int ptr, int device_index) -> ()", &ipc_close);
  m.def("host_device_pointer(Tensor host) -> int", &host_device_pointer);
}
```

### distributed_embeddings_b200/ops/csrc/de_b200.h

```cpp
#pragma once
#include <cuda_runtime.h>
#include <stdint.h>

namespace de {

constexpr int kMaxPeers = 16;
constexpr int kGridCapSms = 132;

struct alignas(16) InputDesc {
  const void* table;
  const void* ids;
  const int64_t* offsets;
  int64_t ids_off;
  int64_t id_shift;
  int64_t sub_rows;
  int64_t row_base;
  int32_t width;
  int32_t hotness;
  int32_t dst_col;
  int32_t combiner;
  int32_t local_table;
  int32_t flags;
  int64_t item_off;
};

struct PeerPtrs {
  void* p[kMaxPeers];
};

constexpr int kSyncChannels = 16;
constexpr int kSyncStateWords = 64;
struct SyncArgs {
  PeerPtrs flags;
  uint32_t* state;
  int* error_flag;
  unsigned long long timeout;
  int32_t rank, world;
  int32_t wait_ch;
  int32_t wait_abs_ch;
  int32_t signal_ch;
  int32_t counter_slot;
};
inline SyncArgs no_sync() {
  SyncArgs s{};
  s.state = nullptr;
  s.wait_ch = s.wait_abs_ch = s.signal_ch = -1;
  return s;
}

struct alignas(16) GradRoute {
  void* dst;
  int64_t dst_stride;
  int32_t src_col;
  int32_t width;
  int32_t dst_col;
  int32_t pad;
};

enum OptimizerKind : int32_t { kOptSGD = 0, kOptAdagrad = 1, kOptRowwiseAdagrad = 2, kOptAdam = 3, kOptEmit = 4 };

struct alignas(16) TableDesc {
  void* weight;
  void* state0;
  void* state1;
  int64_t rows;
  int64_t key_base;
  int32_t width;
  int32_t pad;
};

struct OptimizerArgs {
  int32_t kind;
  float lr;
  float eps;
  float beta1, beta2;
  float bias1, bias2;
  float grad_scale;
  float weight_decay;
  const float* lr_ptr;
  const float* step_ptr;
};

void launch_lookup_fwd(const InputDesc* descs, int n_inputs, int64_t batch, int64_t src_batch,
                       int64_t dst_batch, int64_t dst_stride, const PeerPtrs& src,
                       const PeerPtrs& dst, int rot, bool ids64, int act_dtype, bool vec4,
                       int sm_count, cudaStream_t stream, const SyncArgs& sync,
                       int tile_samples = 32, int table_dtype = 0, bool vec8 = false);

void launch_scatter_add_bwd(const InputDesc* descs, int n_inputs, int64_t batch, int64_t src_batch,
                            int64_t grad_batch, int64_t grad_stride, const PeerPtrs& src,
                            const PeerPtrs& grad, int rot, float scale, const float* scale_ptr,
                            bool ids64, int act_dtype, bool vec4, int sm_count,
                            cudaStream_t stream, bool vec8, const SyncArgs& sync,
                            bool staged = false);

void launch_build_keys(const InputDesc* descs, const TableDesc* tables, int n_tables, int n_inputs,
                       int64_t batch, int64_t src_batch, const PeerPtrs& src, bool ids64, void* keys,
                       uint32_t* items, int sm_count, cudaStream_t stream, bool keys32 = false);
size_t sort_pairs_temp_bytes(int64_t n);
void sort_pairs(void* temp, size_t temp_bytes, const int64_t* keys_in, int64_t* keys_out,
                const uint32_t* items_in, uint32_t* items_out, int64_t n, int end_bit,
                cudaStream_t stream);
size_t unique_temp_bytes(int64_t n);
void unique_segments(void* temp, size_t temp_bytes, const int64_t* sorted_keys, int64_t n,
                     int64_t* seg_start, int64_t* n_unique, cudaStream_t stream);
size_t radix_sort_temp_bytes(int64_t n);
int radix_sort_pairs(void* temp, int64_t* keys_a, uint32_t* items_a, int64_t* keys_b,
                     uint32_t* items_b, int64_t n, int end_bit, cudaStream_t stream);
int radix_sort_pairs32(void* temp, uint32_t* keys_a, uint32_t* items_a, uint32_t* keys_b,
                       uint32_t* items_b, int64_t* keys_out64, int64_t n, int end_bit,
                       cudaStream_t stream);
size_t head_segments_temp_bytes(int64_t n);
void head_segments(void* temp, const int64_t* sorted_keys, int64_t n, int64_t* seg_start,
                   int64_t* n_unique, cudaStream_t stream);
void launch_segment_update(const InputDesc* descs, const TableDesc* tables, int n_tables,
                           int64_t batch, int64_t grad_batch, int64_t grad_stride,
                           const PeerPtrs& grad, const int64_t* sorted_keys,
                           const uint32_t* sorted_items, const int64_t* seg_start,
                           const int64_t* n_unique, int64_t n_items, const OptimizerArgs& opt,
                           int64_t* emit_keys, float* emit_rows, int max_width, int act_dtype,
                           bool vec4, int sm_count, cudaStream_t stream, int table_dtype = 0);

bool launch_balanced_update(const InputDesc* descs, const TableDesc* tables, int n_tables,
                            int64_t batch, int64_t grad_batch, int64_t grad_stride,
                            const PeerPtrs& grad, const int64_t* sorted_keys,
                            const uint32_t* sorted_items, int64_t n_items,
                            const int64_t* seg_start, const int64_t* n_unique,
                            const OptimizerArgs& opt, float* scratch, int scratch_width,
                            int max_width, int act_dtype, int sm_count, cudaStream_t stream,
                            int table_dtype = 0);

void launch_row_to_split(const int64_t* coo_indices, int64_t nnz, int64_t num_rows,
                         int64_t* row_splits, cudaStream_t stream);
void launch_hash_init(int64_t* table, int64_t n_slots, cudaStream_t stream);
void launch_integer_lookup(int64_t* table, int64_t n_slots, uint32_t* counts, int64_t* next_index,
                           const int64_t* keys, int64_t n, int64_t capacity, int64_t* out,
                           cudaStream_t stream);

void launch_barrier(const PeerPtrs& flags, uint32_t* epoch, int rank, int world, int channel,
                    unsigned long long timeout_cycles, int* error_flag, cudaStream_t stream);
void launch_allreduce(const PeerPtrs& bufs, const PeerPtrs& flags, uint32_t* epoch, int rank,
                      int world, int64_t n_elems, float scale, bool bf16, int channel,
                      unsigned long long timeout_cycles, int* error_flag, int sm_count,
                      cudaStream_t stream, int max_blocks = 0);
void launch_allreduce_multimem(void* mc_ptr, const PeerPtrs& flags, uint32_t* epoch, int rank,
                               int world, int64_t n_elems, float scale, bool bf16, int channel,
                               unsigned long long timeout_cycles, int* error_flag, int sm_count,
                               cudaStream_t stream, int max_blocks = 0);
void launch_p2p_store_bench(const void* src, void* dst, int64_t n_rows, int row_bytes,
                            int vec_bytes, int64_t dst_stride, int unroll, int blocks, int threads,
                            cudaStream_t stream);
void launch_sync_only(const SyncArgs& sync, cudaStream_t stream);
void launch_push_segments(const int64_t* segs, int n_seg, const void* src, const PeerPtrs& dst,
                          int elem_bytes, int64_t max_seg_elems, int sm_count,
                          cudaStream_t stream, const SyncArgs& sync);
void launch_push_grad(const GradRoute* routes, int n_routes, const void* src, int64_t src_stride,
                      int src_dtype, int dst_dtype, int64_t rows, float scale, int sm_count,
                      cudaStream_t stream, const SyncArgs& sync);
struct PushPlan {
  const void* src[kMaxPeers];
  void* dst[kMaxPeers];
  int64_t row_bytes[kMaxPeers];
  int32_t n;
};
void launch_stream_push(const PushPlan& plan, const uint32_t* counters, int chunk_rows,
                        int64_t rows, unsigned long long timeout, int* error_flag, int blocks,
                        cudaStream_t stream, const SyncArgs& sync);
void launch_rowslice_reduce(const float* partial, int world, int64_t rows, int64_t part_stride,
                            void* out, int64_t out_stride, int out_dtype, const int32_t* cols,
                            int n_cols, cudaStream_t stream);
void launch_gather_segments(const int64_t* segs, int n_seg, const PeerPtrs& src, void* dst,
                            int elem_bytes, int64_t max_seg_elems, cudaStream_t stream);
void launch_gather_ragged(const int64_t* segs, int n_seg, const PeerPtrs& src_vals,
                          const PeerPtrs& src_splits, void* dst_vals, int64_t* goff, int64_t b,
                          int world, int elem_bytes, int64_t max_cap, cudaStream_t stream);
void launch_select_copy(const void* const* src0, const void* const* src1, void* const* dst,
                        const int64_t* nbytes, int count, const int* slot_flag, int sm_count,
                        cudaStream_t stream);
void launch_copy_cast_2d(const void* src, int64_t src_stride, void* dst, int64_t dst_stride,
                         int64_t rows, int64_t cols, int src_dtype, int dst_dtype, float scale,
                         cudaStream_t stream);

bool launch_interact_fwd(const void* bottom, int64_t bottom_stride, const void* emb,
                         int64_t emb_stride, int n_emb, int dim, void* z, int64_t z_stride,
                         int z_width, int64_t batch, int sm_count, cudaStream_t stream,
                         const SyncArgs& sync);
bool launch_interact_bwd(const void* bottom, int64_t bottom_stride, const void* emb,
                         int64_t emb_stride, int n_emb, int dim, const void* dz,
                         int64_t dz_stride, void* dbottom, int64_t dbottom_stride, void* demb,
                         int64_t demb_stride, float emb_grad_scale, int64_t batch, int sm_count,
                         cudaStream_t stream, const GradRoute* routes, int n_routes,
                         const SyncArgs& sync, uint32_t* done_counters = nullptr,
                         int chunk_rows = 0);
void launch_avgpool_fwd(const void* x, int64_t x_stride, int n, void* out, int64_t out_stride,
                        int out_len, int stride, int left, int64_t rows, cudaStream_t stream);
void launch_avgpool_bwd(const void* dout, int64_t dout_stride, int out_len, void* dx,
                        int64_t dx_stride, int n, int stride, int left, int64_t rows,
                        cudaStream_t stream);
void launch_relu_bwd_bias(void* dy, const void* y, float* db, int64_t rows, int cols,
                          cudaStream_t stream);
bool launch_head_loss(const void* x, int K, const void* w, const void* bias, const float* labels,
                      int64_t batch, float inv_batch, void* dx, float* dw, float* db,
                      float* dbias_prev, float* loss_sum, float* logits_out, int sm_count,
                      cudaStream_t stream);
void launch_sgd_update(float* p32, void* p16, float* g32, const float* lr_ptr, float grad_scale,
                       int64_t n, int sm_count, cudaStream_t stream);
void launch_cast_pad(const float* src, int src_cols, void* dst, int dst_cols, int64_t rows,
                     cudaStream_t stream);

bool launch_gemm_tn_fused(const void* A, int64_t lda, const void* B, int64_t ldb, const void* bias,
                          void* C, int64_t ldc, int M, int N, int K, int epi, const void* act,
                          int64_t ldact, float* colsum, int block_n, int sm_count,
                          cudaStream_t stream);
bool launch_gemm_tn_bias_act(const void* A, int64_t lda, const void* B, int64_t ldb,
                             const void* bias, void* C, int64_t ldc, int M, int N, int K,
                             bool relu, int block_n, int sm_count, cudaStream_t stream);

}
```

### distributed_embeddings_b200/ops/csrc/dense_kernels.cu

```cuda
#include <cuda_bf16.h>
#include <cuda_runtime.h>
#include <stdint.h>

#include <cstdlib>

#include "common.cuh"
#include "de_b200.h"

namespace de {

namespace {

using bf16 = __nv_bfloat16;

__device__ __forceinline__ uint32_t smem_u32(const void* p) {
  return static_cast<uint32_t>(__cvta_generic_to_shared(p));
}

__device__ __forceinline__ void ldmatrix_x4(uint32_t (&r)[4], uint32_t addr) {
  asm volatile("ldmatrix.sync.aligned.m8n8.x4.shared.b16 {%0,%1,%2,%3}, [%4];"
               : "=r"(r[0]), "=r"(r[1]), "=r"(r[2]), "=r"(r[3])
               : "r"(addr));
}
__device__ __forceinline__ void ldmatrix_x4_trans(uint32_t (&r)[4], uint32_t addr) {
  asm volatile("ldmatrix.sync.aligned.m8n8.x4.trans.shared.b16 {%0,%1,%2,%3}, [%4];"
               : "=r"(r[0]), "=r"(r[1]), "=r"(r[2]), "=r"(r[3])
               : "r"(addr));
}
__device__ __forceinline__ void mma_bf16(float (&c)[4], const uint32_t (&a)[4], uint32_t b0,
                                         uint32_t b1) {
  asm volatile(
      "mma.sync.aligned.m16n8k16.row.col.f32.bf16.bf16.f32 {%0,%1,%2,%3}, {%4,%5,%6,%7}, "
      "{%8,%9}, {%0,%1,%2,%3};"
      : "+f"(c[0]), "+f"(c[1]), "+f"(c[2]), "+f"(c[3])
      : "r"(a[0]), "r"(a[1]), "r"(a[2]), "r"(a[3]), "r"(b0), "r"(b1));
}

constexpr int kMaxFeat = 32;
constexpr int kWarps = 4;

__host__ __device__ constexpr int fwd_warp_bytes(int d) {
  return (kMaxFeat * (d + 8) * 2 > kMaxFeat * 33 * 4) ? kMaxFeat * (d + 8) * 2 : kMaxFeat * 33 * 4;
}

__device__ __forceinline__ void cp_async16(void* smem_dst, const void* gmem_src) {
  asm volatile("cp.async.cg.shared.global [%0], [%1], 16;" ::"r"(smem_u32(smem_dst)),
               "l"(gmem_src)
               : "memory");
}
__device__ __forceinline__ void cp_async_wait_all() {
  asm volatile("cp.async.commit_group;\ncp.async.wait_group 0;" ::: "memory");
}

template <int D>
__device__ __forceinline__ void stage_features(bf16* sF, int LD, const bf16* bottom,
                                               const bf16* emb, int n_emb, int lane) {
  constexpr int kChunks = D / 8;
  const int total = (n_emb + 1) * kChunks;
#pragma unroll 4
  for (int c = lane; c < total; c += 32) {
    const int row = c / kChunks, ch = c - row * kChunks;
    const bf16* src = row == 0 ? bottom + ch * 8 : emb + (row - 1) * D + ch * 8;
    cp_async16(sF + row * LD + ch * 8, src);
  }
  cp_async_wait_all();
}

template <int D>
__device__ __forceinline__ void zero_pad_rows(bf16* sF, int LD, int n_emb, int lane) {
  constexpr int kChunks = D / 8;
  for (int c = (n_emb + 1) * kChunks + lane; c < kMaxFeat * kChunks; c += 32) {
    const int row = c / kChunks, ch = c - row * kChunks;
    *reinterpret_cast<uint4*>(sF + row * LD + ch * 8) = make_uint4(0, 0, 0, 0);
  }
}

template <int D>
__global__ void __launch_bounds__(kWarps * 32)
interact_fwd_kernel(const bf16* __restrict__ bottom, int64_t bottom_stride,
                    const bf16* __restrict__ emb, int64_t emb_stride, int n_emb,
                    bf16* __restrict__ z, int64_t z_stride, int z_width, int64_t batch,
                    const __grid_constant__ SyncArgs sync) {
  sync_head(sync);
  constexpr int LD = D + 8;
  constexpr int kWarpBytes = fwd_warp_bytes(D);
  extern __shared__ __align__(16) unsigned char smem_raw[];
  const int warp = threadIdx.x >> 5, lane = threadIdx.x & 31;
  bf16* sF = reinterpret_cast<bf16*>(smem_raw + warp * kWarpBytes);
  float* sC = reinterpret_cast<float*>(sF);
  const int nf = n_emb + 1;
  const int n_inter = nf * (nf - 1) / 2;

  for (int64_t s = static_cast<int64_t>(blockIdx.x) * kWarps + warp; s < batch;
       s += static_cast<int64_t>(gridDim.x) * kWarps) {
    const bf16* bp = bottom + s * bottom_stride;
    zero_pad_rows<D>(sF, LD, n_emb, lane);
    stage_features<D>(sF, LD, bp, emb + s * emb_stride, n_emb, lane);
    __syncwarp();
    float acc0[2][4] = {}, acc1[4][4] = {};
#pragma unroll
    for (int k = 0; k < D; k += 16) {
      uint32_t a0[4], a1[4], b01[4], b23[4];
      const int arow = lane & 15, acol = k + ((lane >> 4) << 3);
      ldmatrix_x4(a0, smem_u32(sF + arow * LD + acol));
      ldmatrix_x4(a1, smem_u32(sF + (16 + arow) * LD + acol));
      const int brow = (lane & 7) + ((lane >> 4) << 3), bcol = k + (((lane >> 3) & 1) << 3);
      ldmatrix_x4(b01, smem_u32(sF + brow * LD + bcol));
      ldmatrix_x4(b23, smem_u32(sF + (16 + brow) * LD + bcol));
      mma_bf16(acc0[0], a0, b01[0], b01[1]);
      mma_bf16(acc0[1], a0, b01[2], b01[3]);
      mma_bf16(acc1[0], a1, b01[0], b01[1]);
      mma_bf16(acc1[1], a1, b01[2], b01[3]);
      mma_bf16(acc1[2], a1, b23[0], b23[1]);
      mma_bf16(acc1[3], a1, b23[2], b23[3]);
    }
    __syncwarp();
    const int cr = lane >> 2, cc = (lane & 3) << 1;
#pragma unroll
    for (int nt = 0; nt < 2; ++nt) {
      sC[cr * 33 + nt * 8 + cc] = acc0[nt][0];
      sC[cr * 33 + nt * 8 + cc + 1] = acc0[nt][1];
      sC[(cr + 8) * 33 + nt * 8 + cc] = acc0[nt][2];
      sC[(cr + 8) * 33 + nt * 8 + cc + 1] = acc0[nt][3];
    }
#pragma unroll
    for (int nt = 0; nt < 4; ++nt) {
      sC[(16 + cr) * 33 + nt * 8 + cc] = acc1[nt][0];
      sC[(16 + cr) * 33 + nt * 8 + cc + 1] = acc1[nt][1];
      sC[(24 + cr) * 33 + nt * 8 + cc] = acc1[nt][2];
      sC[(24 + cr) * 33 + nt * 8 + cc + 1] = acc1[nt][3];
    }
    __syncwarp();
    bf16* zp = z + s * z_stride;
    for (int idx = lane; idx < n_inter; idx += 32) {
      int i = static_cast<int>((1.0f + sqrtf(1.0f + 8.0f * idx)) * 0.5f);
      while (i * (i - 1) / 2 > idx) --i;
      while ((i + 1) * i / 2 <= idx) ++i;
      const int j = idx - i * (i - 1) / 2;
      zp[idx] = __float2bfloat16_rn(sC[i * 33 + j]);
    }
    for (int c = lane; c < D; c += 32) zp[n_inter + c] = bp[c];
    for (int c = n_inter + D + lane; c < z_width; c += 32) zp[c] = __float2bfloat16_rn(0.f);
    __syncwarp();
  }
  sync_tail(sync);
}

template <int D>
__global__ void __launch_bounds__(kWarps * 32)
interact_bwd_kernel(const bf16* __restrict__ bottom, int64_t bottom_stride,
                    const bf16* __restrict__ emb, int64_t emb_stride, int n_emb,
                    const bf16* __restrict__ dz, int64_t dz_stride, bf16* __restrict__ dbottom,
                    int64_t dbottom_stride, bf16* __restrict__ demb, int64_t demb_stride,
                    float emb_grad_scale, int64_t batch) {
  constexpr int LD = D + 8;
  constexpr int LDG = 40;
  extern __shared__ __align__(16) unsigned char smem_raw[];
  const int warp = threadIdx.x >> 5, lane = threadIdx.x & 31;
  bf16* sF = reinterpret_cast<bf16*>(smem_raw) + warp * (kMaxFeat * LD + kMaxFeat * LDG);
  bf16* sG = sF + kMaxFeat * LD;
  const int nf = n_emb + 1;
  const int n_inter = nf * (nf - 1) / 2;
  zero_pad_rows<D>(sF, LD, n_emb, lane);

  for (int64_t s = static_cast<int64_t>(blockIdx.x) * kWarps + warp; s < batch;
       s += static_cast<int64_t>(gridDim.x) * kWarps) {
    stage_features<D>(sF, LD, bottom + s * bottom_stride, emb + s * emb_stride, n_emb, lane);
    const bf16* dzp = dz + s * dz_stride;
    for (int c = lane; c < kMaxFeat * LDG / 8; c += 32)
      reinterpret_cast<uint4*>(sG)[c] = make_uint4(0, 0, 0, 0);
    __syncwarp();
    for (int idx = lane; idx < n_inter; idx += 32) {
      int i = static_cast<int>((1.0f + sqrtf(1.0f + 8.0f * idx)) * 0.5f);
      while (i * (i - 1) / 2 > idx) --i;
      while ((i + 1) * i / 2 <= idx) ++i;
      const int j = idx - i * (i - 1) / 2;
      const bf16 v = dzp[idx];
      sG[i * LDG + j] = v;
      sG[j * LDG + i] = v;
    }
    __syncwarp();
    uint32_t ga[2][2][4];
#pragma unroll
    for (int mt = 0; mt < 2; ++mt)
#pragma unroll
      for (int ks = 0; ks < 2; ++ks)
        ldmatrix_x4(ga[mt][ks],
                    smem_u32(sG + (mt * 16 + (lane & 15)) * LDG + ks * 16 + ((lane >> 4) << 3)));
    const int cr = lane >> 2, cc = (lane & 3) << 1;
    bf16* dbp = dbottom + s * dbottom_stride;
    bf16* dep = demb + s * demb_stride;
#pragma unroll 1
    for (int n0 = 0; n0 < D; n0 += 32) {
      float acc[2][4][4] = {};
#pragma unroll
      for (int ks = 0; ks < 2; ++ks) {
        uint32_t b01[4], b23[4];
        const int krow = ks * 16 + (lane & 7) + (((lane >> 3) & 1) << 3);
        const int ncol = n0 + ((lane >> 4) << 3);
        ldmatrix_x4_trans(b01, smem_u32(sF + krow * LD + ncol));
        ldmatrix_x4_trans(b23, smem_u32(sF + krow * LD + ncol + 16));
#pragma unroll
        for (int mt = 0; mt < 2; ++mt) {
          mma_bf16(acc[mt][0], ga[mt][ks], b01[0], b01[1]);
          mma_bf16(acc[mt][1], ga[mt][ks], b01[2], b01[3]);
          mma_bf16(acc[mt][2], ga[mt][ks], b23[0], b23[1]);
          mma_bf16(acc[mt][3], ga[mt][ks], b23[2], b23[3]);
        }
      }
#pragma unroll
      for (int mt = 0; mt < 2; ++mt) {
#pragma unroll
        for (int nt = 0; nt < 4; ++nt) {
#pragma unroll
          for (int half = 0; half < 2; ++half) {
            const int row = mt * 16 + cr + half * 8;
            const int col = n0 + nt * 8 + cc;
            float v0 = acc[mt][nt][half * 2], v1 = acc[mt][nt][half * 2 + 1];
            if (row == 0) {
              v0 += __bfloat162float(dzp[n_inter + col]);
              v1 += __bfloat162float(dzp[n_inter + col + 1]);
              *reinterpret_cast<__nv_bfloat162*>(dbp + col) = __floats2bfloat162_rn(v0, v1);
            } else if (row <= n_emb) {
              *reinterpret_cast<__nv_bfloat162*>(dep + (row - 1) * D + col) =
                  __floats2bfloat162_rn(v0 * emb_grad_scale, v1 * emb_grad_scale);
            }
          }
        }
      }
    }
    __syncwarp();
  }
}

__device__ __forceinline__ void cp_async_commit() {
  asm volatile("cp.async.commit_group;" ::: "memory");
}
template <int N>
__device__ __forceinline__ void cp_async_wait_group() {
  asm volatile("cp.async.wait_group %0;" ::"n"(N) : "memory");
}

constexpr int kDzMax = 512;

template <int D>
__device__ __forceinline__ void issue_sample(bf16* sF, int LD, bf16* sDz, const bf16* bottom,
                                             const bf16* emb, const bf16* dz, int n_emb,
                                             int dz_chunks, int lane) {
  constexpr int kChunks = D / 8;
  const int total = (n_emb + 1) * kChunks;
#pragma unroll 4
  for (int c = lane; c < total; c += 32) {
    const int row = c / kChunks, ch = c - row * kChunks;
    const bf16* src = row == 0 ? bottom + ch * 8 : emb + (row - 1) * D + ch * 8;
    cp_async16(sF + row * LD + ch * 8, src);
  }
  for (int c = lane; c < dz_chunks; c += 32) cp_async16(sDz + c * 8, dz + c * 8);
}

struct ChunkDst {
  unsigned long long base;
  long long stride;
};

template <int D>
__global__ void __launch_bounds__(kWarps * 32)
interact_bwd_v2_kernel(const bf16* __restrict__ bottom, int64_t bottom_stride,
                       const bf16* __restrict__ emb, int64_t emb_stride, int n_emb,
                       const bf16* __restrict__ dz, int64_t dz_stride, bf16* __restrict__ dbottom,
                       int64_t dbottom_stride, bf16* __restrict__ demb, int64_t demb_stride,
                       float emb_grad_scale, int64_t batch,
                       const GradRoute* __restrict__ routes, int n_routes,
                       const __grid_constant__ SyncArgs sync, uint32_t* __restrict__ done_counters,
                       int chunk_rows) {
  constexpr int LD = D + 8;
  constexpr int LDG = 40;
  constexpr int kWarpElems = 2 * kMaxFeat * LD + 2 * kDzMax + kMaxFeat * LDG;
  constexpr int kRowChunks = D / 8;
  extern __shared__ __align__(16) unsigned char smem_raw[];
  const int warp = threadIdx.x >> 5, lane = threadIdx.x & 31;
  bf16* base = reinterpret_cast<bf16*>(smem_raw) + warp * kWarpElems;
  bf16* sDz0 = base + 2 * kMaxFeat * LD;
  bf16* sG = sDz0 + 2 * kDzMax;
  ChunkDst* sDst = reinterpret_cast<ChunkDst*>(reinterpret_cast<bf16*>(smem_raw) +
                                               kWarps * kWarpElems);
  const int nf = n_emb + 1;
  const int n_inter = nf * (nf - 1) / 2;
  const int dz_chunks = (n_inter + D + 7) >> 3;
  const int n_chunks = n_emb * kRowChunks;
  if (routes == nullptr) {
    for (int c = threadIdx.x; c < n_chunks; c += blockDim.x) {
      sDst[c].base = reinterpret_cast<unsigned long long>(demb + c * 8);
      sDst[c].stride = demb_stride * 2;
    }
  } else {
    for (int r = 0; r < n_routes; ++r) {
      const GradRoute R = routes[r];
      const int c0 = R.src_col >> 3, nc = R.width >> 3;
      for (int c = threadIdx.x; c < nc; c += blockDim.x) {
        sDst[c0 + c].base =
            reinterpret_cast<unsigned long long>(reinterpret_cast<bf16*>(R.dst) + R.dst_col + c * 8);
        sDst[c0 + c].stride = R.dst_stride * 2;
      }
    }
  }
  zero_pad_rows<D>(base, LD, n_emb, lane);
  zero_pad_rows<D>(base + kMaxFeat * LD, LD, n_emb, lane);
  __syncthreads();

  const int64_t stride = static_cast<int64_t>(gridDim.x) * kWarps;
  int64_t s = static_cast<int64_t>(blockIdx.x) * kWarps + warp;
  int cur = 0;
  if (s < batch)
    issue_sample<D>(base, LD, sDz0, bottom + s * bottom_stride, emb + s * emb_stride,
                    dz + s * dz_stride, n_emb, dz_chunks, lane);
  cp_async_commit();
  for (; s < batch; s += stride, cur ^= 1) {
    const int64_t nxt = s + stride;
    if (nxt < batch)
      issue_sample<D>(base + (cur ^ 1) * (kMaxFeat * LD), LD, sDz0 + (cur ^ 1) * kDzMax,
                      bottom + nxt * bottom_stride, emb + nxt * emb_stride, dz + nxt * dz_stride,
                      n_emb, dz_chunks, lane);
    cp_async_commit();
    cp_async_wait_group<1>();
    __syncwarp();
    bf16* sF = base + cur * (kMaxFeat * LD);
    const bf16* sDz = sDz0 + cur * kDzMax;
    for (int c = lane; c < kMaxFeat * LDG / 8; c += 32)
      reinterpret_cast<uint4*>(sG)[c] = make_uint4(0, 0, 0, 0);
    __syncwarp();
    for (int idx = lane; idx < n_inter; idx += 32) {
      int i = static_cast<int>((1.0f + sqrtf(1.0f + 8.0f * idx)) * 0.5f);
      while (i * (i - 1) / 2 > idx) --i;
      while ((i + 1) * i / 2 <= idx) ++i;
      const int j = idx - i * (i - 1) / 2;
      const bf16 v = sDz[idx];
      sG[i * LDG + j] = v;
      sG[j * LDG + i] = v;
    }
    __syncwarp();
    uint32_t ga[2][2][4];
#pragma unroll
    for (int mt = 0; mt < 2; ++mt)
#pragma unroll
      for (int ks = 0; ks < 2; ++ks)
        ldmatrix_x4(ga[mt][ks],
                    smem_u32(sG + (mt * 16 + (lane & 15)) * LDG + ks * 16 + ((lane >> 4) << 3)));
    const int cr = lane >> 2, cc = (lane & 3) << 1;
#pragma unroll 1
    for (int n0 = 0; n0 < D; n0 += 32) {
      float acc[2][4][4] = {};
#pragma unroll
      for (int ks = 0; ks < 2; ++ks) {
        uint32_t b01[4], b23[4];
        const int krow = ks * 16 + (lane & 7) + (((lane >> 3) & 1) << 3);
        const int ncol = n0 + ((lane >> 4) << 3);
        ldmatrix_x4_trans(b01, smem_u32(sF + krow * LD + ncol));
        ldmatrix_x4_trans(b23, smem_u32(sF + krow * LD + ncol + 16));
#pragma unroll
        for (int mt = 0; mt < 2; ++mt) {
          mma_bf16(acc[mt][0], ga[mt][ks], b01[0], b01[1]);
          mma_bf16(acc[mt][1], ga[mt][ks], b01[2], b01[3]);
          mma_bf16(acc[mt][2], ga[mt][ks], b23[0], b23[1]);
          mma_bf16(acc[mt][3], ga[mt][ks], b23[2], b23[3]);
        }
      }
#pragma unroll
      for (int mt = 0; mt < 2; ++mt) {
#pragma unroll
        for (int nt = 0; nt < 4; ++nt) {
#pragma unroll
          for (int half = 0; half < 2; ++half) {
            const int row = mt * 16 + cr + half * 8;
            const int col = n0 + nt * 8 + cc;
            float v0 = acc[mt][nt][half * 2], v1 = acc[mt][nt][half * 2 + 1];
            if (row == 0) {
              v0 += __bfloat162float(sDz[n_inter + col]);
              v1 += __bfloat162float(sDz[n_inter + col + 1]);
            } else {
              v0 *= emb_grad_scale;
              v1 *= emb_grad_scale;
            }
            if (row <= n_emb)
              *reinterpret_cast<__nv_bfloat162*>(sF + row * LD + col) =
                  __floats2bfloat162_rn(v0, v1);
          }
        }
      }
    }
    __syncwarp();
    if (lane < kRowChunks)
      *reinterpret_cast<uint4*>(dbottom + s * dbottom_stride + lane * 8) =
          *reinterpret_cast<const uint4*>(sF + lane * 8);
    for (int c = lane; c < n_chunks; c += 32) {
      const int row = 1 + c / kRowChunks, ch = c - (row - 1) * kRowChunks;
      const ChunkDst d = sDst[c];
      *reinterpret_cast<uint4*>(d.base + static_cast<unsigned long long>(s * d.stride)) =
          *reinterpret_cast<const uint4*>(sF + row * LD + ch * 8);
    }
    __syncwarp();
    if (done_counters != nullptr && lane == 0) {
      __threadfence();
      atomicAdd(done_counters + s / chunk_rows, 1u);
    }
  }
  cp_async_wait_group<0>();
  sync_tail(sync);
}

constexpr int kRbUnroll = 4;
__global__ void __launch_bounds__(256)
relu_bwd_bias_kernel(bf16* __restrict__ dy, const bf16* __restrict__ y, float* __restrict__ db,
                     int64_t rows, int cols, int rows_per_block) {
  extern __shared__ float s_part[];
  const int tpr = cols >> 3;
  const int rows_par = blockDim.x / tpr;
  const int tr = threadIdx.x / tpr, tc = threadIdx.x - tr * tpr;
  const int64_t r0 = static_cast<int64_t>(blockIdx.x) * rows_per_block;
  const int64_t r1 = min(rows, r0 + rows_per_block);
  float acc[8] = {0, 0, 0, 0, 0, 0, 0, 0};
  if (tr < rows_par) {
    for (int64_t r = r0 + tr; r < r1; r += static_cast<int64_t>(rows_par) * kRbUnroll) {
      uint4 g[kRbUnroll], a[kRbUnroll];
#pragma unroll
      for (int u = 0; u < kRbUnroll; ++u) {
        const int64_t rr = r + static_cast<int64_t>(u) * rows_par;
        if (rr < r1) {
          g[u] = *reinterpret_cast<const uint4*>(dy + rr * cols + tc * 8);
          a[u] = *reinterpret_cast<const uint4*>(y + rr * cols + tc * 8);
        }
      }
#pragma unroll
      for (int u = 0; u < kRbUnroll; ++u) {
        const int64_t rr = r + static_cast<int64_t>(u) * rows_par;
        if (rr < r1) {
          uint32_t* gw = reinterpret_cast<uint32_t*>(&g[u]);
          const uint32_t* aw = reinterpret_cast<const uint32_t*>(&a[u]);
#pragma unroll
          for (int i = 0; i < 4; ++i) {
            float2 gf = __bfloat1622float2(*reinterpret_cast<__nv_bfloat162*>(&gw[i]));
            const float2 af = __bfloat1622float2(*reinterpret_cast<const __nv_bfloat162*>(&aw[i]));
            gf.x = af.x > 0.f ? gf.x : 0.f;
            gf.y = af.y > 0.f ? gf.y : 0.f;
            acc[2 * i] += gf.x;
            acc[2 * i + 1] += gf.y;
            __nv_bfloat162 h = __floats2bfloat162_rn(gf.x, gf.y);
            gw[i] = *reinterpret_cast<uint32_t*>(&h);
          }
          *reinterpret_cast<uint4*>(dy + rr * cols + tc * 8) = g[u];
        }
      }
    }
#pragma unroll
    for (int i = 0; i < 8; ++i) s_part[tr * cols + tc * 8 + i] = acc[i];
  }
  __syncthreads();
  for (int c = threadIdx.x; c < cols; c += blockDim.x) {
    float v = 0.f;
    for (int t = 0; t < rows_par; ++t) v += s_part[t * cols + c];
    atomicAdd(db + c, v);
  }
}

template <int PL>
__global__ void __launch_bounds__(256)
head_loss_kernel(const bf16* __restrict__ x, int K, const bf16* __restrict__ w,
                 const bf16* __restrict__ bias, const float* __restrict__ labels, int64_t batch,
                 float inv_batch, bf16* __restrict__ dx, float* __restrict__ dw,
                 float* __restrict__ db, float* __restrict__ dbias_prev,
                 float* __restrict__ loss_sum, float* __restrict__ logits_out) {
  extern __shared__ float sred[];
  float* s_dw = sred;
  float* s_dbp = sred + K;
  float* s_misc = sred + 2 * K;
  for (int i = threadIdx.x; i < 2 * K + 2; i += blockDim.x) sred[i] = 0.f;
  __syncthreads();
  const int warp = threadIdx.x >> 5, lane = threadIdx.x & 31;
  const int wpb = blockDim.x >> 5;
  constexpr int per_lane = PL;
  const float b0 = __bfloat162float(bias[0]);
  float wreg[PL];
#pragma unroll
  for (int i = 0; i < PL; ++i) wreg[i] = __bfloat162float(w[lane + 32 * i]);
  float dw_acc[PL], dbp_acc[PL];
#pragma unroll
  for (int i = 0; i < PL; ++i) dw_acc[i] = dbp_acc[i] = 0.f;
  float loss_acc = 0.f, db_acc = 0.f;
  for (int64_t s = static_cast<int64_t>(blockIdx.x) * wpb + warp; s < batch;
       s += static_cast<int64_t>(gridDim.x) * wpb) {
    float xv[PL];
    float dot = 0.f;
#pragma unroll
    for (int i = 0; i < PL; ++i) {
      if (i < per_lane) {
        xv[i] = __bfloat162float(x[s * K + lane + 32 * i]);
        dot = fmaf(xv[i], wreg[i], dot);
      }
    }
#pragma unroll
    for (int off = 16; off > 0; off >>= 1) dot += __shfl_xor_sync(0xffffffffu, dot, off);
    const float logit = dot + b0;
    const float label = labels[s];
    const float loss = fmaxf(logit, 0.f) - logit * label + log1pf(__expf(-fabsf(logit)));
    const float sig = 1.f / (1.f + __expf(-logit));
    const float dl = (sig - label) * inv_batch;
    if (lane == 0) {
      loss_acc += loss;
      db_acc += dl;
      if (logits_out) logits_out[s] = logit;
    }
#pragma unroll
    for (int i = 0; i < PL; ++i) {
      if (i < per_lane) {
        dw_acc[i] = fmaf(dl, xv[i], dw_acc[i]);
        const float g = xv[i] > 0.f ? dl * wreg[i] : 0.f;
        dbp_acc[i] += g;
        dx[s * K + lane + 32 * i] = __float2bfloat16_rn(g);
      }
    }
  }
#pragma unroll
  for (int i = 0; i < PL; ++i) {
    if (i < per_lane) {
      atomicAdd(&s_dw[lane + 32 * i], dw_acc[i]);
      atomicAdd(&s_dbp[lane + 32 * i], dbp_acc[i]);
    }
  }
  if (lane == 0) {
    atomicAdd(&s_misc[0], loss_acc);
    atomicAdd(&s_misc[1], db_acc);
  }
  __syncthreads();
  for (int i = threadIdx.x; i < K; i += blockDim.x) {
    atomicAdd(dw + i, s_dw[i]);
    atomicAdd(dbias_prev + i, s_dbp[i]);
  }
  if (threadIdx.x == 0) {
    atomicAdd(loss_sum, s_misc[0] * inv_batch);
    atomicAdd(db, s_misc[1]);
  }
}

__global__ void __launch_bounds__(256)
sgd_update_kernel(float* __restrict__ p32, bf16* __restrict__ p16, float* __restrict__ g32,
                  const float* __restrict__ lr_ptr, float grad_scale, int64_t n_vec4) {
  const float step = -(*lr_ptr) * grad_scale;
  const int64_t stride = static_cast<int64_t>(gridDim.x) * blockDim.x;
  for (int64_t i = static_cast<int64_t>(blockIdx.x) * blockDim.x + threadIdx.x; i < n_vec4;
       i += stride) {
    float4 p = reinterpret_cast<float4*>(p32)[i];
    const float4 g = reinterpret_cast<const float4*>(g32)[i];
    p.x = fmaf(step, g.x, p.x);
    p.y = fmaf(step, g.y, p.y);
    p.z = fmaf(step, g.z, p.z);
    p.w = fmaf(step, g.w, p.w);
    reinterpret_cast<float4*>(p32)[i] = p;
    reinterpret_cast<float4*>(g32)[i] = make_float4(0.f, 0.f, 0.f, 0.f);
    __nv_bfloat162 a = __floats2bfloat162_rn(p.x, p.y), b = __floats2bfloat162_rn(p.z, p.w);
    uint2 o;
    o.x = *reinterpret_cast<uint32_t*>(&a);
    o.y = *reinterpret_cast<uint32_t*>(&b);
    reinterpret_cast<uint2*>(p16)[i] = o;
  }
}

__global__ void cast_pad_kernel(const float* __restrict__ src, int src_cols, bf16* __restrict__ dst,
                                int dst_cols, int64_t rows) {
  const int64_t n = rows * dst_cols;
  const int64_t stride = static_cast<int64_t>(gridDim.x) * blockDim.x;
  for (int64_t i = static_cast<int64_t>(blockIdx.x) * blockDim.x + threadIdx.x; i < n;
       i += stride) {
    const int64_t r = i / dst_cols;
    const int c = static_cast<int>(i - r * dst_cols);
    dst[i] = __float2bfloat16_rn(c < src_cols ? src[r * src_cols + c] : 0.f);
  }
}

__global__ void __launch_bounds__(256)
avgpool_fwd_kernel(const bf16* __restrict__ x, int64_t x_stride, int n, bf16* __restrict__ out,
                   int64_t out_stride, int out_len, int stride, int left, int64_t rows) {
  const int64_t total = rows * out_len;
  const int64_t step = static_cast<int64_t>(gridDim.x) * blockDim.x;
  for (int64_t i = static_cast<int64_t>(blockIdx.x) * blockDim.x + threadIdx.x; i < total;
       i += step) {
    const int64_t r = i / out_len;
    const int j = static_cast<int>(i - r * out_len);
    const int lo = max(0, j * stride - left), hi = min(n, (j + 1) * stride - left);
    const bf16* xp = x + r * x_stride;
    float acc = 0.f;
    for (int c = lo; c < hi; ++c) acc += __bfloat162float(xp[c]);
    out[r * out_stride + j] = __float2bfloat16_rn(hi > lo ? acc / static_cast<float>(hi - lo) : 0.f);
  }
}

__global__ void __launch_bounds__(256)
avgpool_bwd_kernel(const bf16* __restrict__ dout, int64_t dout_stride, int out_len,
                   bf16* __restrict__ dx, int64_t dx_stride, int n, int stride, int left,
                   int64_t rows) {
  const int64_t total = rows * n;
  const int64_t step = static_cast<int64_t>(gridDim.x) * blockDim.x;
  for (int64_t i = static_cast<int64_t>(blockIdx.x) * blockDim.x + threadIdx.x; i < total;
       i += step) {
    const int64_t r = i / n;
    const int c = static_cast<int>(i - r * n);
    const int j = (c + left) / stride;
    const int lo = max(0, j * stride - left), hi = min(n, (j + 1) * stride - left);
    const float g = j < out_len ? __bfloat162float(dout[r * dout_stride + j]) : 0.f;
    dx[r * dx_stride + c] = __float2bfloat16_rn(g / static_cast<float>(hi - lo));
  }
}

}

void launch_avgpool_fwd(const void* x, int64_t x_stride, int n, void* out, int64_t out_stride,
                        int out_len, int stride, int left, int64_t rows, cudaStream_t stream) {
  if (rows <= 0 || out_len <= 0) return;
  int64_t blocks = (rows * out_len + 255) / 256;
  if (blocks > kGridCapSms * 16) blocks = kGridCapSms * 16;
  avgpool_fwd_kernel<<<static_cast<unsigned>(blocks), 256, 0, stream>>>(
      reinterpret_cast<const bf16*>(x), x_stride, n, reinterpret_cast<bf16*>(out), out_stride,
      out_len, stride, left, rows);
}

void launch_avgpool_bwd(const void* dout, int64_t dout_stride, int out_len, void* dx,
                        int64_t dx_stride, int n, int stride, int left, int64_t rows,
                        cudaStream_t stream) {
  if (rows <= 0 || n <= 0) return;
  int64_t blocks = (rows * n + 255) / 256;
  if (blocks > kGridCapSms * 16) blocks = kGridCapSms * 16;
  avgpool_bwd_kernel<<<static_cast<unsigned>(blocks), 256, 0, stream>>>(
      reinterpret_cast<const bf16*>(dout), dout_stride, out_len, reinterpret_cast<bf16*>(dx),
      dx_stride, n, stride, left, rows);
}

bool launch_interact_fwd(const void* bottom, int64_t bottom_stride, const void* emb,
                         int64_t emb_stride, int n_emb, int dim, void* z, int64_t z_stride,
                         int z_width, int64_t batch, int sm_count, cudaStream_t stream,
                         const SyncArgs& sync) {
  if (n_emb + 1 > kMaxFeat || batch <= 0) return false;
  int64_t blocks = (batch + kWarps - 1) / kWarps;
  const int64_t cap = static_cast<int64_t>(sm_count) * 8;
  if (blocks > cap) blocks = cap;
#define DE_IFWD(DD)                                                                              \
  {                                                                                              \
    const size_t smem = kWarps * fwd_warp_bytes(DD);                                             \
    cudaFuncSetAttribute(interact_fwd_kernel<DD>, cudaFuncAttributeMaxDynamicSharedMemorySize,   \
                         static_cast<int>(smem));                                                \
    interact_fwd_kernel<DD><<<static_cast<unsigned>(blocks), kWarps * 32, smem, stream>>>(       \
        reinterpret_cast<const bf16*>(bottom), bottom_stride, reinterpret_cast<const bf16*>(emb), \
        emb_stride, n_emb, reinterpret_cast<bf16*>(z), z_stride, z_width, batch, sync);          \
    return true;                                                                                 \
  }
  if (dim == 128) DE_IFWD(128)
  if (dim == 64) DE_IFWD(64)
  if (dim == 32) DE_IFWD(32)
  if (dim == 16) DE_IFWD(16)
#undef DE_IFWD
  return false;
}

bool launch_interact_bwd(const void* bottom, int64_t bottom_stride, const void* emb,
                         int64_t emb_stride, int n_emb, int dim, const void* dz,
                         int64_t dz_stride, void* dbottom, int64_t dbottom_stride, void* demb,
                         int64_t demb_stride, float emb_grad_scale, int64_t batch, int sm_count,
                         cudaStream_t stream, const GradRoute* routes, int n_routes,
                         const SyncArgs& sync, uint32_t* done_counters, int chunk_rows) {
  if (n_emb + 1 > kMaxFeat || batch <= 0 || dim % 32 != 0) return false;
  int64_t blocks = (batch + kWarps - 1) / kWarps;
  const int64_t cap = static_cast<int64_t>(sm_count) * 8;
  if (blocks > cap) blocks = cap;
  static const bool force_v1 = [] {
    const char* v = std::getenv("DE_B200_INTERACT_V1");
    return v != nullptr && v[0] == '1';
  }();
  const int nf = n_emb + 1;
  const int dz_elems = (nf * (nf - 1) / 2 + dim + 7) / 8 * 8;
  const bool v2_ok =
      dz_elems <= kDzMax && dz_elems <= dz_stride && dz_stride % 8 == 0 &&
      bottom_stride % 8 == 0 && emb_stride % 8 == 0 && dbottom_stride % 8 == 0 &&
      ((reinterpret_cast<uintptr_t>(dz) | reinterpret_cast<uintptr_t>(bottom) |
        reinterpret_cast<uintptr_t>(emb) | reinterpret_cast<uintptr_t>(dbottom)) & 15) == 0 &&
      (dim == 128 || dim == 64) &&
      (routes != nullptr || (demb_stride % 8 == 0 && (reinterpret_cast<uintptr_t>(demb) & 15) == 0));
  if ((routes != nullptr || done_counters != nullptr) && !v2_ok) return false;
  const bool has_sync = sync.state != nullptr && (sync.wait_ch >= 0 || sync.signal_ch >= 0);
  if (v2_ok && (!force_v1 || routes != nullptr || has_sync || done_counters != nullptr)) {
    int64_t blocks2 = (batch + kWarps - 1) / kWarps;
    if (blocks2 > static_cast<int64_t>(sm_count) * 2) blocks2 = static_cast<int64_t>(sm_count) * 2;
#define DE_IBWD2(DD)                                                                             \
  {                                                                                              \
    const size_t smem =                                                                          \
        kWarps * (2 * kMaxFeat * (DD + 8) + 2 * kDzMax + kMaxFeat * 40) * sizeof(bf16) +         \
        static_cast<size_t>(n_emb) * (DD / 8) * sizeof(ChunkDst);                                \
    cudaFuncSetAttribute(interact_bwd_v2_kernel<DD>,                                             \
                         cudaFuncAttributeMaxDynamicSharedMemorySize, static_cast<int>(smem));   \
    interact_bwd_v2_kernel<DD><<<static_cast<unsigned>(blocks2), kWarps * 32, smem, stream>>>(   \
        reinterpret_cast<const bf16*>(bottom), bottom_stride, reinterpret_cast<const bf16*>(emb), \
        emb_stride, n_emb, reinterpret_cast<const bf16*>(dz), dz_stride,                         \
        reinterpret_cast<bf16*>(dbottom), dbottom_stride, reinterpret_cast<bf16*>(demb),         \
        demb_stride, emb_grad_scale, batch, routes, n_routes, sync, done_counters, chunk_rows);  \
    return true;                                                                                 \
  }
    if (dim == 128) DE_IBWD2(128)
    if (dim == 64) DE_IBWD2(64)
#undef DE_IBWD2
  }
  if (has_sync) return false;
#define DE_IBWD(DD)                                                                              \
  {                                                                                              \
    const size_t smem = kWarps * (kMaxFeat * (DD + 8) + kMaxFeat * 40) * sizeof(bf16);           \
    cudaFuncSetAttribute(interact_bwd_kernel<DD>, cudaFuncAttributeMaxDynamicSharedMemorySize,   \
                         static_cast<int>(smem));                                                \
    interact_bwd_kernel<DD><<<static_cast<unsigned>(blocks), kWarps * 32, smem, stream>>>(       \
        reinterpret_cast<const bf16*>(bottom), bottom_stride, reinterpret_cast<const bf16*>(emb), \
        emb_stride, n_emb, reinterpret_cast<const bf16*>(dz), dz_stride,                         \
        reinterpret_cast<bf16*>(dbottom), dbottom_stride, reinterpret_cast<bf16*>(demb),         \
        demb_stride, emb_grad_scale, batch);                                                     \
    return true;                                                                                 \
  }
  if (dim == 128) DE_IBWD(128)
  if (dim == 64) DE_IBWD(64)
  if (dim == 32) DE_IBWD(32)
#undef DE_IBWD
  return false;
}

void launch_relu_bwd_bias(void* dy, const void* y, float* db, int64_t rows, int cols,
                          cudaStream_t stream) {
  if (rows <= 0) return;
  const int tpr = cols / 8;
  const int threads = 256;
  const int rows_par = threads / tpr;
  const int rows_per_block = rows_par * kRbUnroll * 4;
  const int64_t blocks = (rows + rows_per_block - 1) / rows_per_block;
  const size_t smem = static_cast<size_t>(rows_par) * cols * sizeof(float);
  relu_bwd_bias_kernel<<<static_cast<unsigned>(blocks), threads, smem, stream>>>(
      reinterpret_cast<bf16*>(dy), reinterpret_cast<const bf16*>(y), db, rows, cols,
      rows_per_block);
}

bool launch_head_loss(const void* x, int K, const void* w, const void* bias, const float* labels,
                      int64_t batch, float inv_batch, void* dx, float* dw, float* db,
                      float* dbias_prev, float* loss_sum, float* logits_out, int sm_count,
                      cudaStream_t stream) {
  if (batch <= 0) return true;
  const int threads = 256;
  int64_t blocks = (batch + 7) / 8;
  if (blocks > sm_count * 4) blocks = sm_count * 4;
  const size_t smem = (2 * K + 2) * sizeof(float);
#define DE_HEAD(PL)                                                                              \
  head_loss_kernel<PL><<<static_cast<unsigned>(blocks), threads, smem, stream>>>(                \
      reinterpret_cast<const bf16*>(x), K, reinterpret_cast<const bf16*>(w),                     \
      reinterpret_cast<const bf16*>(bias), labels, batch, inv_batch, reinterpret_cast<bf16*>(dx), \
      dw, db, dbias_prev, loss_sum, logits_out)
  switch (K) {
    case 64: DE_HEAD(2); break;
    case 128: DE_HEAD(4); break;
    case 256: DE_HEAD(8); break;
    case 512: DE_HEAD(16); break;
    case 1024: DE_HEAD(32); break;
    default: return false;
  }
#undef DE_HEAD
  return true;
}

void launch_sgd_update(float* p32, void* p16, float* g32, const float* lr_ptr, float grad_scale,
                       int64_t n, int sm_count, cudaStream_t stream) {
  const int64_t n_vec4 = n / 4;
  if (n_vec4 <= 0) return;
  int64_t blocks = (n_vec4 + 255) / 256;
  if (blocks > sm_count * 8) blocks = sm_count * 8;
  sgd_update_kernel<<<static_cast<unsigned>(blocks), 256, 0, stream>>>(
      p32, reinterpret_cast<bf16*>(p16), g32, lr_ptr, grad_scale, n_vec4);
}

void launch_cast_pad(const float* src, int src_cols, void* dst, int dst_cols, int64_t rows,
                     cudaStream_t stream) {
  if (rows <= 0) return;
  int64_t blocks = (rows * dst_cols + 255) / 256;
  if (blocks > kGridCapSms * 8) blocks = kGridCapSms * 8;
  cast_pad_kernel<<<static_cast<unsigned>(blocks), 256, 0, stream>>>(
      src, src_cols, reinterpret_cast<bf16*>(dst), dst_cols, rows);
}

}
```

### distributed_embeddings_b200/parallel/fused.py

```python
from __future__ import annotations

import os
import weakref
from typing import Any, Dict, List, Optional, Sequence, Tuple

import numpy as np
import torch

from ..ops import _native
from ..ops._native import DTYPE_CODE, GRAD_ROUTE, INPUT_DESC, TABLE_DESC
from ..ops.ragged import RaggedIds
from ..utils import nvtx
from .comm import CH_BARRIER0, CH_CONSUMED, CH_GRAD, CH_IDS, CH_OUT, CommContext

_OPT_KIND = {"sgd": _native.OPT_SGD, "adagrad": _native.OPT_ADAGRAD,
             "rowwise_adagrad": _native.OPT_ROWWISE_ADAGRAD, "adam": _native.OPT_ADAM}
_COMB = {None: 0, "sum": 0, "mean": 1}

FLAG_SKIP_EMPTY = 1
FLAG_CATCH_LOW = 2
FLAG_CATCH_HIGH = 4


def _weight(layer):
  return layer.embeddings


def _dev_ptr(t: torch.Tensor) -> int:
  if t.is_cuda:
    return t.data_ptr()
  if not t.is_pinned():
    raise RuntimeError("host-resident tables must live in pinned memory for the fused back end")
  return int(_native.require().host_device_pointer(t))


class _FusedFn(torch.autograd.Function):

  @staticmethod
  def forward(ctx, engine, token, *weights):
    ctx.engine = engine
    ctx.n_weights = len(weights)
    ctx.done = False
    engine._gen += 1
    ctx.gen = engine._gen
    out = engine._run_forward()
    engine._pending = weakref.ref(ctx)
    if not getattr(engine.de, "zero_copy_output", False):
      out = out.clone()
    return out

  @staticmethod
  def backward(ctx, grad_out):
    engine = ctx.engine
    if ctx.gen != engine._gen:
      raise RuntimeError(
          "DistributedEmbedding (fused back end): another forward ran on this layer before the "
          "backward of an earlier one; its index buffers were overwritten.  Call backward first, "
          "or use backend='torch' for several forwards per backward.")
    ctx.done = True
    grads = engine._run_backward(grad_out)
    return (None, None) + tuple(grads)


class FusedEngine:

  def __init__(self, de, dry=None):
    self.de = de
    self.st = de.strategy
    self.W, self.rank = de.world_size, de.rank
    self.device = de.device
    self.dry = dry is not None
    if self.dry:
      self.ops, self.ctx = dry.ops, dry.ctx
      dry.attach(self)
    else:
      self.ops = _native.require()
      self.ctx = CommContext.for_group(de.group, self.device)
    if self.W > 1 and not self.ctx.p2p:
      raise RuntimeError("fused back end needs CUDA peer access between all ranks")
    st = self.st
    imap = st.input_table_map
    self.out_widths = [int(st.global_configs[t]["output_dim"]) for t in imap]
    self.out_cols = [0]
    for w in self.out_widths:
      self.out_cols.append(self.out_cols[-1] + w)
    self.total_width = self.out_cols[-1]
    self.compute_dtype = de.compute_dtype
    if self.compute_dtype not in DTYPE_CODE:
      raise ValueError("fused back end supports fp32, bf16 and fp16 activations")
    self.act = DTYPE_CODE[self.compute_dtype]
    self.table_dtype = getattr(de, "table_dtype", torch.float32)
    self.tab = DTYPE_CODE[self.table_dtype]
    self._key = None
    self._gen = 0
    self._pending = None
    self._token = torch.zeros((), device=self.device)
    self.lr_t = torch.zeros(1, dtype=torch.float32, device=self.device)
    self._lr_external = False
    self.step_t = torch.zeros(1, dtype=torch.float32, device=self.device)
    self.opt_state: Dict[int, List[torch.Tensor]] = {}
    self._tables_dirty = True
    self._dp_targets = None
    self._dp_target_desc = None
    self.out_row_stride = None
    self.push_chunk_rows = None
    self._dry_updates = False
    self.mp_layers = list(de.local_embedding_layers) + list(de.row_layers)
    self.n_col_tables = len(de.local_embedding_layers)
    self.has_offload = any(getattr(l, "cpu_offloaded", False) for l in self.mp_layers)

  def _ptr(self, t: torch.Tensor) -> int:
    return t.data_ptr() if self.dry else _dev_ptr(t)

  def _sync(self, wait: int = -1, wait_abs: int = -1, signal: int = -1):
    return self.ctx.sync(wait=wait, wait_abs=wait_abs, signal=signal) if self.W > 1 else []

  def dry_updates(self, on: bool):
    self._dry_updates = bool(on)

  def enable_streamed_push(self, chunk_rows: Optional[int]):
    if chunk_rows != self.push_chunk_rows:
      self.push_chunk_rows = chunk_rows
      if self._key is not None:
        self.close()

  def set_out_row_stride(self, stride: Optional[int]):
    if stride is not None and (stride < self.total_width or stride % 8):
      raise ValueError("out row stride must be a multiple of 8 and >= the total output width")
    if stride != self.out_row_stride:
      self.out_row_stride = stride
      if self._key is not None:
        self.close()

  def busy(self) -> bool:
    node = self._pending() if self._pending is not None else None
    return node is not None and not node.done

  def supports(self, inputs) -> bool:
    st, de = self.st, self.de
    col_inputs = set(st.input_groups[1]) if de.dp_input else set(range(len(inputs)))
    imap = st.input_table_map
    for i, x in enumerate(inputs):
      if isinstance(x, RaggedIds):
        if i not in col_inputs:
          return False
        continue
      if not isinstance(x, torch.Tensor) or x.dim() > 2:
        return False
      if x.dim() == 2 and x.shape[1] != 1:
        t = imap[i] if de.dp_input else \
            st.table_groups[1][st.map_groups[1][st.input_ids_list[self.rank][i]]]
        if st.global_configs[t].get("combiner") is None:
          return False
    return True

  def _mp_layout(self, r: int, hots: Optional[Tuple[int, ...]], B: int):
    de, st = self.de, self.st
    col_group = st.input_groups[1]
    col_map = st.map_groups[1]
    my_inputs = st.input_ids_list[r] if st.table_groups[1] else []
    items, cols, widths, pos, col = [], [], [], 0, 0
    for li, k in enumerate(my_inputs):
      shard = next(s for s in st.shards[r] if s.table == col_map[k])
      if hots is not None:
        gi = col_group[k] if de.dp_input else li
        items.append(pos)
        pos += B * abs(hots[gi])
      cols.append(col)
      widths.append(int(shard.width))
      col += int(shard.width)
    row_inputs = st.input_groups[2] if de.dp_input else []
    for j, gi in enumerate(row_inputs):
      m = st.map_groups[2][j]
      w = int(st.row_sliced_configs[r][m]["output_dim"])
      if hots is not None:
        items.append(pos)
        pos += B * abs(hots[gi])
      cols.append(col)
      widths.append(w)
      col += w
    return {"items": items, "n_items": pos, "cols": cols, "widths": widths, "width": col,
            "n_col": len(my_inputs)}

  _SYM_BUFS = ("in_buf", "split_buf", "ids_buf", "out_buf", "recv_buf", "rs_buf")
  _SYM_VIEWS = ("in_flat", "in_views", "split_flat", "split_views", "ids_mp", "out", "out_full",
                "recv", "rs", "gstage")

  def close(self):
    bufs = [getattr(self, n, None) for n in self._SYM_BUFS]
    bufs = [b for b in bufs if b is not None]
    if bufs and self.W > 1 and not self.dry:
      torch.cuda.synchronize(self.device)
      for b in bufs:
        b.close()
      torch.distributed.barrier(group=self.de.group)
    for n in self._SYM_BUFS + self._SYM_VIEWS:
      if hasattr(self, n):
        setattr(self, n, None)
    self._key = None

  def _build(self, b: int, hots: Tuple[int, ...], ids64: bool):
    de, st, W, rank = self.de, self.st, self.W, self.rank
    dev = self.device
    if self._key is not None:
      self.close()
    id_dtype = torch.int64 if ids64 else torch.int32
    idsz = 8 if ids64 else 4
    B = b * W if de.dp_input else b
    lb = b if de.dp_input else b // W
    self.B, self.lb, self.hots, self.ids64, self.id_dtype = B, lb, hots, ids64, id_dtype
    csz = 4 if self.act == 0 else 2

    col_group = st.input_groups[1] if de.dp_input else list(range(len(hots)))
    col_map = st.map_groups[1]
    self.ragged = [h < 0 for h in hots]
    self.any_ragged = any(self.ragged)
    n_rag = sum(self.ragged)
    rag_index = {}
    for i, r in enumerate(self.ragged):
      if r:
        rag_index[i] = len(rag_index)
    self.id_mode = "none" if W == 1 or not de.dp_input else ("pull" if self.any_ragged else "push")
    if de.dp_input:
      in_off, pos = [], 0
      for h in hots:
        in_off.append(pos)
        pos += b * abs(h)
      self.in_elems = max(pos, 1)
      if self.id_mode == "pull":
        self.in_buf = self.ctx.alloc(self.in_elems * idsz, "ids_in")
        in_flat = self.in_buf.view(id_dtype, (self.in_elems,))
        self.in_ptrs = self.in_buf.peer_ptrs()
      else:
        self.in_buf = None
        in_flat = torch.zeros(self.in_elems, dtype=id_dtype, device=dev)
        self.in_ptrs = [in_flat.data_ptr()]
      self.in_flat = in_flat
      self.in_views = [in_flat[o:o + b * abs(h)].view(b, abs(h)) for o, h in zip(in_off, hots)]
      if n_rag:
        n_sp = n_rag * (b + 1)
        if W > 1:
          self.split_buf = self.ctx.alloc(n_sp * 8, "ragged_splits")
          self.split_flat = self.split_buf.view(torch.int64, (n_sp,))
          self.split_ptrs = self.split_buf.peer_ptrs()
        else:
          self.split_buf = None
          self.split_flat = torch.zeros(n_sp, dtype=torch.int64, device=dev)
          self.split_ptrs = [self.split_flat.data_ptr()]
        self.split_views = {i: self.split_flat[j * (b + 1):(j + 1) * (b + 1)]
                            for i, j in rag_index.items()}
    else:
      in_off = None
      self.in_buf, self.in_flat, self.in_views, self.in_ptrs = None, None, None, []
      self.split_views = {}

    layouts = [self._mp_layout(r, hots if (de.dp_input or r == rank) else None, B)
               for r in range(W)]
    mine = layouts[rank]
    my_inputs = st.input_ids_list[rank] if st.table_groups[1] else []
    row_inputs = st.input_groups[2] if de.dp_input else []
    n_col, n_row = len(my_inputs), len(row_inputs)
    col_items, row_items = mine["items"][:n_col], mine["items"][n_col:]
    self.n_items = mine["n_items"]
    self.recv_width = max(mine["width"], 1)
    need_copy = (W > 1) or (not de.dp_input)
    if self.id_mode == "push":
      n_sym = max(max(l["n_items"] for l in layouts), 1)
      self.ids_buf = self.ctx.alloc(n_sym * idsz, "ids_mp")
      self.ids_mp = self.ids_buf.view(id_dtype, (n_sym,))
      self.ids_ptrs = self.ids_buf.peer_ptrs()
    else:
      self.ids_buf = None
      self.ids_mp = torch.zeros(max(self.n_items, 1), dtype=id_dtype, device=dev) \
          if need_copy else None
      self.ids_ptrs = []
    my_ragged = [li for li, k in enumerate(my_inputs)
                 if self.ragged[col_group[k] if de.dp_input else li]]
    self.goff = torch.zeros(max(len(my_ragged) * (B + 1), 1), dtype=torch.int64, device=dev)
    goff_index = {li: j for j, li in enumerate(my_ragged)}

    def ids_ptr(item_off, gi):
      if need_copy:
        return self.ids_mp.data_ptr() + item_off * idsz
      return self.in_flat.data_ptr() + in_off[gi] * idsz

    tdesc = np.zeros(len(self.mp_layers), dtype=TABLE_DESC)
    key = 0
    for m, layer in enumerate(self.mp_layers):
      w = _weight(layer)
      tdesc[m]["weight"] = self._ptr(w)
      tdesc[m]["rows"] = w.shape[0]
      tdesc[m]["key_base"] = key
      tdesc[m]["width"] = w.shape[1]
      key += w.shape[0]
    self.total_rows = key
    self.tdesc_np = tdesc
    self.max_width = max([int(_weight(l).shape[1]) for l in self.mp_layers] + [1])

    tw = self.total_width
    ostride = self.out_stride = int(self.out_row_stride or tw)
    out_bytes = max(lb * ostride * csz, 16)
    recv_w_sym = max(max(l["width"] for l in layouts), 1)
    if W > 1:
      self.out_buf = self.ctx.alloc(out_bytes, "emb_out")
      self.out_full = self.out_buf.view(self.compute_dtype, (lb, ostride))
      self.out = self.out_full[:, :tw]
      self.out_ptrs = self.out_buf.peer_ptrs()
      self.recv_buf = self.ctx.alloc(max(B * recv_w_sym * csz, 16), "emb_grad_recv")
      self.recv = self.recv_buf.view(self.compute_dtype, (B, self.recv_width))
      recv_ptrs = self.recv_buf.peer_ptrs()
    else:
      self.out_buf = self.recv_buf = None
      self.out_full = torch.zeros(lb, ostride, dtype=self.compute_dtype, device=dev)
      self.out = self.out_full[:, :tw]
      self.out_ptrs = [self.out.data_ptr()]
      self.recv = torch.zeros(B, self.recv_width, dtype=self.compute_dtype, device=dev)
      recv_ptrs = [self.recv.data_ptr()]
    self.recv_ptr = [self.recv.data_ptr()]
    dp_inputs = st.input_groups[0] if de.dp_input else []
    self.grad = torch.zeros(lb, tw, dtype=self.compute_dtype, device=dev) if len(dp_inputs) \
        else None

    pieces = {(p.rank, p.local_input): p for p in st.output_pieces}
    cdesc = np.zeros(n_col, dtype=INPUT_DESC)
    segs, rsegs = [], []
    for li, k in enumerate(my_inputs):
      gi = col_group[k] if de.dp_input else li
      t_in_group = col_map[k]
      shard = next(s for s in st.shards[rank] if s.table == t_in_group)
      layer = de.local_embedding_layers[shard.local_table]
      w = _weight(layer)
      d = cdesc[li]
      d["table"] = self._ptr(w)
      d["ids"] = ids_ptr(col_items[li], gi)
      d["ids_off"] = 0
      d["sub_rows"] = shard.rows
      d["row_base"] = shard.row_offset
      d["width"] = shard.width
      d["hotness"] = max(hots[gi], 0)
      if self.ragged[gi]:
        if need_copy:
          d["offsets"] = self.goff.data_ptr() + goff_index[li] * (B + 1) * 8
        else:
          d["offsets"] = self.split_views[gi].data_ptr()
      gi_global = st.input_groups[1][k]
      d["dst_col"] = self.out_cols[gi_global] + pieces[(rank, li)].col_offset
      d["combiner"] = _COMB[layer.combiner]
      d["local_table"] = shard.local_table
      d["item_off"] = col_items[li]
      if layer.combiner is None and hots[gi] != 1:
        raise ValueError("table-parallel lookups without a combiner need one id per sample")
      if self.id_mode == "pull":
        if self.ragged[gi]:
          rsegs.append([in_off[gi], col_items[li], rag_index[gi] * (b + 1),
                        goff_index[li] * (B + 1)])
        else:
          for s in range(W):
            segs.append([s, in_off[gi], col_items[li] + s * b * hots[gi], b * hots[gi]])
    self.cdesc_np = cdesc

    rdesc = np.zeros(n_row, dtype=INPUT_DESC)
    self.rs_width = 0
    self.rs_cols = []
    self.row_onehot = []
    for j, gi in enumerate(row_inputs):
      m = st.map_groups[2][j]
      layer = de.row_layers[m]
      w = _weight(layer)
      d = rdesc[j]
      d["table"] = w.data_ptr()
      d["ids"] = ids_ptr(row_items[j], gi)
      d["id_shift"] = st.row_inputs_offsets[rank][m]
      d["sub_rows"] = w.shape[0]
      d["width"] = w.shape[1]
      d["hotness"] = hots[gi]
      d["combiner"] = _COMB[layer.combiner]
      d["local_table"] = self.n_col_tables + m
      d["item_off"] = row_items[j]
      onehot = hots[gi] == 1
      self.row_onehot.append(onehot)
      if onehot:
        d["dst_col"] = self.out_cols[gi]
        d["flags"] = FLAG_SKIP_EMPTY | (FLAG_CATCH_LOW if rank == 0 else 0) | \
            (FLAG_CATCH_HIGH if rank == W - 1 else 0)
      else:
        d["dst_col"] = self.rs_width
        d["flags"] = 0
        self.rs_cols.append((gi, self.rs_width, int(w.shape[1])))
        self.rs_width += int(w.shape[1])
      if self.id_mode == "pull":
        for s in range(W):
          segs.append([s, in_off[gi], row_items[j] + s * b * hots[gi], b * hots[gi]])
    self.rdesc_np = rdesc
    oh = np.array(self.row_onehot, dtype=bool) if n_row else np.zeros(0, dtype=bool)
    self.fwd_main_np = np.concatenate([cdesc, rdesc[oh]]) if n_row else cdesc
    self.fwd_rs_np = rdesc[~oh] if n_row else rdesc
    if len(self.fwd_rs_np):
      self.rs_buf = self.ctx.alloc(W * lb * self.rs_width * 4, "row_slice_partials")
      self.rs = self.rs_buf.view(torch.float32, (W, lb, self.rs_width))
      self.rs_ptrs = self.rs_buf.peer_ptrs(rank * lb * self.rs_width * 4)
      self.rs_cols_t = torch.tensor([[c0, self.out_cols[gi], w] for gi, c0, w in self.rs_cols],
                                    dtype=torch.int32, device=dev)
    else:
      self.rs_buf = None

    ddesc = np.zeros(len(dp_inputs), dtype=INPUT_DESC)
    for j, gi in enumerate(dp_inputs):
      m = st.map_groups[0][j]
      layer = de.dp_layers[m]
      w = _weight(layer)
      d = ddesc[j]
      d["table"] = w.data_ptr()
      d["ids"] = self.in_flat.data_ptr() + in_off[gi] * idsz
      d["sub_rows"] = w.shape[0]
      d["width"] = w.shape[1]
      d["hotness"] = hots[gi]
      d["dst_col"] = self.out_cols[gi]
      d["combiner"] = _COMB[layer.combiner]
      d["local_table"] = m
    self.ddesc_np = ddesc
    self._dp_grad_flat, self._dp_grad_views, self._dp_grad_desc = None, [], None
    self._dp_grad_desc_np = None
    if len(de.dp_layers):
      offs, pos = [], 0
      for layer in de.dp_layers:
        offs.append(pos)
        pos += (_weight(layer).numel() + 3) // 4 * 4
      self._dp_grad_flat = torch.zeros(max(pos, 4), dtype=torch.float32, device=dev)
      self._dp_grad_views = [self._dp_grad_flat[o:o + _weight(l).numel()].view(_weight(l).shape)
                             for o, l in zip(offs, de.dp_layers)]
      dd = ddesc.copy()
      for j in range(len(dd)):
        dd[j]["table"] = self._dp_grad_views[int(dd[j]["local_table"])].data_ptr()
      self._dp_grad_desc_np = dd

    push = []
    if self.id_mode == "push":
      for r in range(W):
        L = layouts[r]
        r_inputs = st.input_ids_list[r] if st.table_groups[1] else []
        for li, k in enumerate(r_inputs):
          gi = col_group[k]
          n = b * hots[gi]
          push.append([r, in_off[gi], L["items"][li] + rank * n, n])
        for j, gi in enumerate(row_inputs):
          n = b * hots[gi]
          push.append([r, in_off[gi], L["items"][L["n_col"] + j] + rank * n, n])
    self.push_segs = torch.tensor(push, dtype=torch.int64, device=dev) if push else None
    self.max_push = max([s[3] for s in push]) if push else 0

    self.gstage, self.push_plan, self.push_counters = None, None, None
    stage_base = {}
    if self.push_chunk_rows and W > 1 and \
        all((layouts[r]["width"] * csz) % 16 == 0 for r in range(W)):
      offs, pos = {}, 0
      for r in range(W):
        if r != rank and layouts[r]["width"]:
          offs[r] = pos
          pos += (lb * layouts[r]["width"] * csz + 255) // 256 * 256
      self.gstage = torch.empty(max(pos, 256), dtype=torch.uint8, device=dev)
      stage_base = {r: self.gstage.data_ptr() + o for r, o in offs.items()}
      peers = sorted(offs, key=lambda r: (r - rank) % W)
      self.push_plan = ([stage_base[r] for r in peers],
                        [recv_ptrs[r] + rank * lb * layouts[r]["width"] * csz for r in peers],
                        [layouts[r]["width"] * csz for r in peers])
      n_chunks = -(-lb // self.push_chunk_rows)
      self.push_counters = torch.zeros(n_chunks, dtype=torch.int32, device=dev)
    routes, routes_stage = [], []
    for r in range(W):
      L = layouts[r]
      base = recv_ptrs[r] + rank * lb * L["width"] * csz
      sbase = stage_base.get(r, base)
      r_inputs = st.input_ids_list[r] if st.table_groups[1] else []
      for li, k in enumerate(r_inputs):
        p = pieces[(r, li)]
        gi_global = st.input_groups[1][k]
        item = (self.out_cols[gi_global] + p.col_offset, L["widths"][li], base, L["width"],
                L["cols"][li])
        routes.append(item)
        routes_stage.append(item[:2] + (sbase,) + item[3:])
      for j, gi in enumerate(row_inputs):
        item = (self.out_cols[gi], L["widths"][L["n_col"] + j], base, L["width"],
                L["cols"][L["n_col"] + j])
        routes.append(item)
        routes_stage.append(item[:2] + (sbase,) + item[3:])
    dp_routes = [(self.out_cols[gi], self.out_widths[gi], self.grad.data_ptr(), tw,
                  self.out_cols[gi]) for gi in dp_inputs]

    def pack(rs):
      rs = sorted(rs, key=lambda x: (x[0], x[2]))
      arr = np.zeros(len(rs), dtype=GRAD_ROUTE)
      for i, (src_col, width, dst, stride, dst_col) in enumerate(rs):
        arr[i]["dst"], arr[i]["dst_stride"] = dst, stride
        arr[i]["src_col"], arr[i]["width"], arr[i]["dst_col"] = src_col, width, dst_col
      return arr
    self.routes_mp_np = pack(routes)
    self.routes_all_np = pack(routes + dp_routes)
    self.routes_stage_np = pack(routes_stage + dp_routes) if self.gstage is not None else None

    self.segs = torch.tensor(segs, dtype=torch.int64, device=dev) if segs else None
    self.max_seg = max([s[3] for s in segs]) if segs else 0
    self.rsegs = torch.tensor(rsegs, dtype=torch.int64, device=dev) if rsegs else None
    self.max_rcap = b * max([abs(h) for h, r in zip(hots, self.ragged) if r] + [0])
    self.my_ragged_mp = my_ragged if not de.dp_input else []
    self.col_items = col_items
    mp = np.concatenate([cdesc, rdesc]) if n_row else cdesc.copy()
    for i in range(len(mp)):
      mp[i]["dst_col"] = mine["cols"][i]
    self.mpdesc_np = mp
    self.n_mp_inputs = len(mp)

    widths = [int(x) for x in list(cdesc["width"]) + list(rdesc["width"]) + list(ddesc["width"])]
    cols = [int(x) for x in list(self.fwd_main_np["dst_col"]) + list(self.fwd_rs_np["dst_col"]) +
            list(ddesc["dst_col"]) + list(mp["dst_col"])]
    self.vec4 = all(w % 4 == 0 for w in widths) and all(c % 4 == 0 for c in cols) and \
        tw % 4 == 0 and self.rs_width % 4 == 0 and self.recv_width % 4 == 0 and ostride % 4 == 0
    fw = [int(x) for x in list(self.fwd_main_np["width"]) + list(self.fwd_rs_np["width"])]
    fc = [int(x) for x in list(self.fwd_main_np["dst_col"]) + list(self.fwd_rs_np["dst_col"])]
    self.fwd_vec8 = self.tab != 0 and self.vec4 and all(w % 8 == 0 for w in fw) and \
        all(c % 8 == 0 for c in fc) and ostride % 8 == 0 and self.rs_width % 8 == 0
    self.vec8 = os.environ.get("DE_B200_VEC8_GRAD", "0") == "1" and self.vec4 and \
        all(w % 8 == 0 for w in widths) and all(c % 8 == 0 for c in cols) and \
        self.recv_width % 8 == 0
    mpw = [int(x) for x in mp["width"]]
    mpc = [int(x) for x in mp["dst_col"]]
    self.staged_update = os.environ.get("DE_B200_SCATTER_STAGED", "1") == "1" and self.vec4 and \
        len(mp) > 0 and all((w * csz) % 16 == 0 and w * csz <= 256 for w in mpw) and \
        all((c * csz) % 16 == 0 for c in mpc) and (self.recv_width * csz) % 16 == 0
    self.staged_dp = os.environ.get("DE_B200_SCATTER_STAGED", "1") == "1" and self.vec4 and \
        len(ddesc) > 0 and (tw * csz) % 16 == 0 and \
        all((int(w) * csz) % 16 == 0 and int(w) * csz <= 256 for w in ddesc["width"]) and \
        all((int(c) * csz) % 16 == 0 for c in ddesc["dst_col"])
    self._upload()
    self._key = (b, hots, ids64)

  def _upload(self):
    dev = self.device
    up = _native.upload_struct_array
    self.fwd_main = up(self.fwd_main_np, dev) if len(self.fwd_main_np) else None
    self.fwd_rs = up(self.fwd_rs_np, dev) if len(self.fwd_rs_np) else None
    self.fwd_launches = []
    if len(self.fwd_main_np):
      hot = self._desc_hotness(self.fwd_main_np)
      low = hot <= 4
      for mask in (low, ~low):
        if mask.any():
          d = self.fwd_main_np[mask]
          self.fwd_launches.append((up(d, dev), int(mask.sum()), self._tile_samples(d, hot[mask])))
    self.fwd_rs_tile = self._tile_samples(self.fwd_rs_np, self._desc_hotness(self.fwd_rs_np)) \
        if len(self.fwd_rs_np) else 32
    self.ddesc = up(self.ddesc_np, dev) if len(self.ddesc_np) else None
    self.mpdesc = up(self.mpdesc_np, dev) if len(self.mpdesc_np) else None
    self.routes_mp = up(self.routes_mp_np, dev) if len(self.routes_mp_np) else None
    self.routes_all = up(self.routes_all_np, dev) if len(self.routes_all_np) else None
    self.routes_stage = up(self.routes_stage_np, dev) if self.routes_stage_np is not None else None
    if self._dp_grad_desc_np is not None and len(self.ddesc_np):
      self._dp_grad_desc = up(self._dp_grad_desc_np, dev)
    self._refresh_tables()

  def _desc_hotness(self, descs) -> np.ndarray:
    hot = descs["hotness"].astype(np.int64).copy()
    rag = hot == 0
    if rag.any():
      cap = max([abs(h) for h in self.hots if h < 0] + [2])
      hot[rag] = max(1, cap // 2)
    return hot

  @staticmethod
  def _tile_samples(descs, hot) -> int:
    if not len(descs):
      return 32
    avg = max(1, int(hot.mean()))
    if avg <= 4:
      return 32
    lpr = 1
    while lpr < (int(descs["width"].min()) + 3) // 4 and lpr < 32:
      lpr *= 2
    return int(max(32 // lpr, min(32, 64 // avg), 1))

  def _refresh_tables(self):
    opt = self.de._fused_optimizer
    t = self.tdesc_np
    for m, layer in enumerate(self.mp_layers):
      t[m]["weight"] = self._ptr(_weight(layer))
      st = self.opt_state.get(m)
      t[m]["state0"] = self._ptr(st[0]) if st else 0
      t[m]["state1"] = self._ptr(st[1]) if st and len(st) > 1 else 0
    self.tdesc = _native.upload_struct_array(t, self.device) if len(t) else None
    self._tables_dirty = False
    if opt is not None and not self._lr_external:
      self.lr_t.fill_(opt["lr"])

  def reset_optimizer_state(self):
    self.opt_state = {}
    opt = self.de._fused_optimizer
    if opt is None:
      return
    kind = opt["kind"]
    self.step_t.fill_(float(opt.get("step", 0)))

    def like(w, value, shape=None):
      t = torch.full(shape or tuple(w.shape), value, dtype=torch.float32, device=w.device)
      return t.pin_memory() if not (w.is_cuda or self.dry) else t

    for m, layer in enumerate(self.mp_layers):
      w = _weight(layer)
      if kind == "adagrad":
        self.opt_state[m] = [like(w, opt["initial_accumulator_value"])]
      elif kind == "rowwise_adagrad":
        self.opt_state[m] = [like(w, opt["initial_accumulator_value"], (w.shape[0],))]
      elif kind == "adam":
        self.opt_state[m] = [like(w, 0.0), like(w, 0.0)]
    self._tables_dirty = True

  def update_lr(self, lr: float):
    self.lr_t.fill_(lr)

  def share_lr(self, lr_t: torch.Tensor):
    self.lr_t = lr_t
    self._lr_external = True

  def step_count(self) -> int:
    return int(round(float(self.step_t.item())))

  def optimizer_state_dict(self) -> Dict[str, Any]:
    return {"state": {m: [s.detach().cpu() for s in st] for m, st in self.opt_state.items()},
            "step": self.step_count()}

  def load_optimizer_state_dict(self, state):
    if not self.opt_state:
      self.reset_optimizer_state()
    for m, tensors in state.get("state", {}).items():
      for dst, src in zip(self.opt_state[int(m)], tensors):
        dst.copy_(src)
    step = int(state.get("step", 0))
    self.step_t.fill_(float(step))
    if self.de._fused_optimizer is not None:
      self.de._fused_optimizer["step"] = step

  def prepare(self, local_batch: int, hotness: Sequence[int], ids64: bool = False):
    key = (int(local_batch), tuple(int(h) for h in hotness), bool(ids64))
    if key != self._key:
      self._build(*key)
    return self

  @property
  def input_views(self) -> List[torch.Tensor]:
    return self.in_views

  def _ragged_capacity(self, inputs, b: int) -> int:
    cap = getattr(self.de, "ragged_capacity", None)
    if cap is None:
      need = max(int(x.values.numel()) for x in inputs if isinstance(x, RaggedIds))
      cap = max(8, 2 * -(-need // max(b, 1)))
      if self.W > 1:
        t = torch.tensor([cap], dtype=torch.int64, device=self.device)
        torch.distributed.all_reduce(t, op=torch.distributed.ReduceOp.MAX, group=self.de.group)
        cap = int(t.item())
      self.de.ragged_capacity = cap
    return int(cap)

  def stage(self, inputs):
    b = inputs[0].nrows if isinstance(inputs[0], RaggedIds) else int(inputs[0].shape[0])
    any_rag = any(isinstance(x, RaggedIds) for x in inputs)
    cap = self._ragged_capacity(inputs, b) if any_rag else 0
    hots = tuple(-cap if isinstance(x, RaggedIds) else (1 if x.dim() == 1 else int(x.shape[1]))
                 for x in inputs)
    ids64 = any((x.values if isinstance(x, RaggedIds) else x).dtype == torch.int64 for x in inputs)
    if self._key is None or self._key[0] != b or self._key[1] != hots or \
        (ids64 and not self._key[2]):
      self._build(b, hots, ids64)
    if self.de.dp_input:
      for i, (v, x) in enumerate(zip(self.in_views, inputs)):
        if isinstance(x, RaggedIds):
          n = int(x.values.numel())
          if n > v.numel():
            raise ValueError(
                f"ragged input {i} holds {n} ids but only {v.numel()} are reserved; raise "
                "DistributedEmbedding.ragged_capacity (ids per sample) on every rank")
          v.view(-1)[:n].copy_(x.values, non_blocking=True)
          self.split_views[i].copy_(x.row_splits, non_blocking=True)
        elif x.data_ptr() != v.data_ptr():
          v.copy_(x.reshape(v.shape), non_blocking=True)
    else:
      for li, x in enumerate(inputs):
        pos = self.col_items[li]
        if isinstance(x, RaggedIds):
          n = int(x.values.numel())
          if n > self.B * cap:
            raise ValueError(f"ragged input {li} holds {n} ids, capacity is {self.B * cap}")
          self.ids_mp[pos:pos + n].copy_(x.values, non_blocking=True)
          j = self.my_ragged_mp.index(li)
          self.goff[j * (self.B + 1):(j + 1) * (self.B + 1)].copy_(x.row_splits,
                                                                     non_blocking=True)
        else:
          n = x.numel()
          self.ids_mp[pos:pos + n].copy_(x.reshape(-1), non_blocking=True)

  def forward(self, inputs, concat: bool):
    self.stage(inputs)
    return self.run(concat)

  def run(self, concat: bool = True):
    if self.de._fused_optimizer is not None and not self.opt_state and \
        self.de._fused_optimizer["kind"] != "sgd":
      self.reset_optimizer_state()
    if self._tables_dirty:
      self._refresh_tables()
    weights = [_weight(l) for l in list(self.de.dp_layers) + self.mp_layers]
    out = _FusedFn.apply(self, self._token, *weights)
    if concat:
      return out
    return list(torch.split(out, self.out_widths, dim=1))

  def _run_forward(self):
    with nvtx.range("emb_forward"):
      self.launch_forward()
      self.wait_output()
      return self.out

  @property
  def has_mp(self) -> bool:
    return self.fwd_main is not None or self.fwd_rs is not None

  @property
  def out_needs_reduce(self) -> bool:
    return self.rs_buf is not None

  def launch_forward(self):
    ops, W, rank = self.ops, self.W, self.rank
    B, lb = self.B, self.lb
    wait_ids = -1
    if W > 1 and self.has_mp:
      if self.id_mode == "push":
        ops.push_segments(self.push_segs, self.in_flat, self.ids_ptrs, self.max_push,
                          self._sync(wait_abs=CH_CONSUMED, signal=CH_IDS))
        wait_ids = CH_IDS
      elif self.id_mode == "pull":
        self.ctx.barrier(CH_BARRIER0)
        if self.segs is not None:
          ops.gather_segments(self.segs, self.in_ptrs, self.ids_mp, self.max_seg)
        if self.rsegs is not None:
          ops.gather_ragged(self.rsegs, self.in_ptrs, self.split_ptrs, self.ids_mp, self.goff,
                            self.lb, self.max_rcap)
      else:
        ops.sync_only(self._sync(signal=CH_IDS))
        wait_ids = CH_IDS
    if self.ddesc is not None:
      ops.lookup_fwd(self.ddesc, len(self.ddesc_np), lb, lb, lb, self.out_stride, [],
                     [self.out.data_ptr()], 0, self.ids64, self.act, self.vec4, [],
                     self._tile_samples(self.ddesc_np, self._desc_hotness(self.ddesc_np)))
    for k, (descs, n, tile) in enumerate(self.fwd_launches):
      last = k == len(self.fwd_launches) - 1 and self.fwd_rs is None
      ops.lookup_fwd(descs, n, B, B, lb, self.out_stride, [], self.out_ptrs, rank, self.ids64,
                     self.act, self.vec4,
                     self._sync(wait=wait_ids, signal=CH_OUT if last else -1), tile, self.tab,
                     self.fwd_vec8)
      wait_ids = -1
    if self.fwd_rs is not None:
      ops.lookup_fwd(self.fwd_rs, len(self.fwd_rs_np), B, B, lb, self.rs_width, [], self.rs_ptrs,
                     rank, self.ids64, 0, self.vec4, self._sync(wait=wait_ids, signal=CH_OUT),
                     self.fwd_rs_tile, self.tab, self.fwd_vec8)

  def sync_out_wait(self):
    return self._sync(wait=CH_OUT) if (self.W > 1 and self.has_mp) else []

  def wait_output(self):
    if self.W > 1 and self.has_mp:
      self.ops.sync_only(self._sync(wait=CH_OUT))
    if self.rs_buf is not None:
      self.ops.rowslice_reduce(self.rs, self.out.data_ptr(), self.out_stride, self.act,
                               self.rs_cols_t)

  def _run_backward(self, grad_out: torch.Tensor):
    ops, de = self.ops, self.de
    lb = self.lb
    if grad_out.dtype not in DTYPE_CODE or grad_out.stride(-1) != 1:
      grad_out = grad_out.float().contiguous()
    self._grad_out_live = grad_out if self.dry else None
    if self.routes_mp is not None:
      ops.push_grad(self.routes_mp, len(self.routes_mp_np), grad_out, self.act, 1.0,
                    self._sync(signal=CH_GRAD))
    grads: List[Optional[torch.Tensor]] = []
    if len(de.dp_layers):
      need = [_weight(l).requires_grad for l in de.dp_layers]
      if any(need) and self._dp_grad_desc is not None:
        self._dp_grad_flat.zero_()
        ops.scatter_add_bwd(self._dp_grad_desc, len(self.ddesc_np), lb, lb, lb,
                            grad_out.stride(0), [], [grad_out.data_ptr()], 0, 1.0, 0, self.ids64,
                            DTYPE_CODE[grad_out.dtype], self._grad_vec4(grad_out), False, [],
                            False)
      for m in range(len(de.dp_layers)):
        grads.append(self._dp_grad_views[m].clone() if need[m] else None)
    grads += self._backward_mp()
    return grads

  def _grad_vec4(self, g: torch.Tensor) -> bool:
    return self.vec4 and g.stride(0) % 4 == 0 and g.data_ptr() % 16 == 0

  def set_dp_grad_targets(self, targets: Optional[Sequence[torch.Tensor]]):
    if targets is not None:
      targets = list(targets)
      if len(targets) != len(self.de.dp_layers):
        raise ValueError(f"expected {len(self.de.dp_layers)} targets, got {len(targets)}")
      for t, layer in zip(targets, self.de.dp_layers):
        w = _weight(layer)
        if t.dtype != torch.float32 or tuple(t.shape) != tuple(w.shape) or not t.is_contiguous():
          raise ValueError("dp gradient targets must be contiguous fp32 tensors of the table shape")
    self._dp_targets = targets
    self._dp_target_desc = None

  def _scatter_dp_grads(self):
    if not len(self.ddesc_np):
      return
    key = (self._key, tuple(t.data_ptr() for t in self._dp_targets))
    if self._dp_target_desc is None or self._dp_target_desc[0] != key:
      d = self.ddesc_np.copy()
      for j in range(len(d)):
        d[j]["table"] = self._dp_targets[int(d[j]["local_table"])].data_ptr()
      self._dp_target_desc = (key, _native.upload_struct_array(d, self.device), len(d))
    _, dd, n = self._dp_target_desc
    self.ops.scatter_add_bwd(dd, n, self.lb, self.lb, self.lb, self.total_width, [],
                             [self.grad.data_ptr()], 0, 1.0, 0, self.ids64, self.act, self.vec4,
                             False, [], self.staged_dp)

  @property
  def streamed_push(self) -> bool:
    return self.gstage is not None

  def launch_streamed_push(self, blocks: int = 32):
    src, dst, row_bytes = self.push_plan
    self.ops.stream_push(src, dst, row_bytes, self.push_counters, self.push_chunk_rows, self.lb,
                         blocks, self._sync(signal=CH_GRAD))

  def sync_grad_signal(self):
    return self._sync(signal=CH_GRAD) if (self.W > 1 and self.mpdesc is not None) else []

  def backward_inplace(self):
    if len(self.de.dp_layers):
      if getattr(self, "_dp_targets", None) is None:
        raise RuntimeError("backward_inplace needs set_dp_grad_targets() for replicated tables")
      self._scatter_dp_grads()
    self._backward_mp()

  def _backward_mp(self) -> List[Optional[torch.Tensor]]:
    with nvtx.range("emb_backward_update"):
      return self._backward_mp_impl()

  def _backward_mp_impl(self) -> List[Optional[torch.Tensor]]:
    ops, de = self.ops, self.de
    n_mp = len(self.mp_layers)
    if self.mpdesc is None:
      return [None] * n_mp
    multi = self.W > 1
    if not any(_weight(l).requires_grad for l in self.mp_layers):
      if multi:
        ops.sync_only(self._sync(wait=CH_GRAD, signal=CH_CONSUMED))
      return [None] * n_mp
    opt = de._fused_optimizer
    if opt is not None and opt["kind"] != "sgd" and not self.opt_state:
      self.reset_optimizer_state()
    if self._tables_dirty:
      self._refresh_tables()
    B = self.B
    gscale = 0.0 if self._dry_updates else de.mp_grad_scale
    if opt is not None and opt["kind"] == "sgd" and not opt.get("deterministic", False) and \
        not self.has_offload and self.tab == 0:
      ops.scatter_add_bwd(self.mpdesc, self.n_mp_inputs, B, B, B, self.recv_width, [],
                          self.recv_ptr, 0, -gscale, self.lr_t.data_ptr(), self.ids64,
                          self.act, self.vec4, self.vec8,
                          self._sync(wait=CH_GRAD, signal=CH_CONSUMED), self.staged_update)
      return [None] * n_mp
    if multi:
      ops.sync_only(self._sync(wait=CH_GRAD))
    keys, items, seg, n_unique = ops.sort_items(self.mpdesc, self.tdesc, n_mp, self.n_mp_inputs,
                                                B, B, [], self.ids64, self.n_items,
                                                self.total_rows, self.any_ragged)
    if opt is not None:
      if not self._dry_updates:
        self.step_t.add_(1.0)
      kind = _OPT_KIND[opt["kind"]]
      if self._dry_updates and opt["kind"] == "adam":
        kind = _OPT_KIND["sgd"]
      ops.segment_update(self.mpdesc, self.tdesc, n_mp, B, B, self.recv_width, self.recv_ptr,
                         keys, items, seg, n_unique, kind, opt["lr"],
                         opt["eps"], opt["beta1"], opt["beta2"], 1.0, 1.0, gscale,
                         opt["weight_decay"], self.lr_t.data_ptr(), None, None, self.max_width,
                         self.act, self.vec4, self._balanced_scratch(), self.step_t.data_ptr(),
                         self.tab)
      if multi:
        ops.sync_only(self._sync(signal=CH_CONSUMED))
      return [None] * n_mp
    emit_keys = torch.empty(self.n_items, dtype=torch.int64, device=self.device)
    emit_rows = torch.empty(self.n_items, self.max_width, dtype=torch.float32, device=self.device)
    ops.segment_update(self.mpdesc, self.tdesc, n_mp, B, B, self.recv_width, self.recv_ptr, keys,
                       items, seg, n_unique, _native.OPT_EMIT, 0.0, 0.0, 0.0, 0.0, 1.0, 1.0,
                       de.mp_grad_scale, 0.0, 0, emit_keys, emit_rows, self.max_width, self.act,
                       self.vec4, None, 0)
    if multi:
      ops.sync_only(self._sync(signal=CH_CONSUMED))
    nu = int(n_unique.item())
    emit_keys, emit_rows = emit_keys[:nu], emit_rows[:nu]
    bases = [int(x) for x in self.tdesc_np["key_base"]] + [self.total_rows]
    bounds = torch.searchsorted(emit_keys, torch.tensor(bases, device=self.device)).tolist()
    out = []
    for m, layer in enumerate(self.mp_layers):
      w = _weight(layer)
      lo, hi = bounds[m], bounds[m + 1]
      ids = (emit_keys[lo:hi] - bases[m]).unsqueeze(0).to(w.device)
      rows = torch.empty(hi - lo, w.shape[1], dtype=w.dtype, device=emit_rows.device)
      rows.copy_(emit_rows[lo:hi, :w.shape[1]])
      rows = rows.to(w.device)
      out.append(torch.sparse_coo_tensor(ids, rows, size=tuple(w.shape), is_coalesced=True,
                                         check_invariants=False))
    return out

  def _balanced_scratch(self):
    if not self.vec4 or self.max_width > 128 or self.n_items == 0:
      return None
    sw = (self.max_width + 3) // 4 * 4
    need = ((self.n_items + 31) // 32) * sw
    cur = getattr(self, "_scratch", None)
    if cur is None or cur.numel() < need:
      self._scratch = torch.zeros(need, dtype=torch.float32, device=self.device)
    return self._scratch
```

Before: 17.08 million.

## Fuse embedding gather into interaction forward and apply SGD updates inside interaction backward

On single-GPU plans with one-hot fp32 tables of equal width, the forward path now uses a new kernel. It gathers embedding rows through a double-buffered cp.async pipeline, casts them to bf16, writes the embedding output and computes the pairwise interaction in one pass, so the separate lookup launch and side-stream overlap are no longer needed. In backward, large tables get their SGD update applied directly inside the interaction backward kernel. The scatter-add pass then runs only for small, hot tables. This removes separate embedding kernels and round trips through the output buffer. The cost is a narrow eligibility path, and atomic-style direct updates on large tables may change the update ordering.

```diff
diff --git a/distributed_embeddings_b200/models/dlrm_fast.py b/distributed_embeddings_b200/models/dlrm_fast.py
--- a/distributed_embeddings_b200/models/dlrm_fast.py
+++ b/distributed_embeddings_b200/models/dlrm_fast.py
@@ -129,6 +129,8 @@
     self.loss = torch.zeros(1, dtype=torch.float32, device=dev)
     self._batch = None
     self._graph = None
+    self._gather_fwd = False
+    self._direct_mask = 0
     self._side = torch.cuda.Stream(device=dev) if overlap else None
     self._wgrad_overlap = os.environ.get("DE_B200_WGRAD_STREAM", "auto")
     self._wstream = torch.cuda.Stream(device=dev) if overlap else None
@@ -176,6 +178,8 @@
       self.engine.enable_streamed_push(max(1024, -(-b // 16)))
     self.engine.prepare(b, [1] * self.n_emb, ids64=False)
     self.cat_stage = self.engine.in_flat[:self.n_emb * b].view(self.n_emb, b)
+    self._gather_fwd = self.engine.gather_interaction_dim == self.dim
+    self._direct_mask = self.engine.direct_update_mask() if self._gather_fwd else 0
     self.num_in = torch.zeros(b, self.bottom[0].in_f, dtype=torch.float32, device=dev)
     self.lab_in = torch.zeros(b, dtype=torch.float32, device=dev)
     self.x0 = torch.zeros(b, self.bottom[0].in_pad, dtype=bf, device=dev)
@@ -203,6 +207,16 @@
       ops.select_copy([a[0], a[1], a[2]], [b_[0], b_[1], b_[2]],
                       [self.cat_stage, self.num_in, self.lab_in], self._slot_dev)
     eng = self.engine
+    if self._gather_fwd:
+      ops.cast_pad(self.num_in, self.x0)
+      x = self.x0
+      for L in self.bottom:
+        x = self._linear_fwd(L, x)
+      ops.interact_fwd_gather(x, eng.gather_desc, self.n_emb, eng.out, self.z)
+      x = self.z
+      for L in self.top:
+        x = self._linear_fwd(L, x)
+      return
     if self._side is not None:
       self._side.wait_stream(torch.cuda.current_stream())
       with torch.cuda.stream(self._side):
@@ -260,6 +274,10 @@
       self._push_stream.wait_event(self._push_ready)
       with torch.cuda.stream(self._push_stream):
         eng.launch_streamed_push()
+    elif self._direct_mask:
+      ops.interact_bwd(hb.y, eng.out, self.n_emb, self.dz, hb.dy, 0, 0, 1.0, eng.routes_all,
+                       len(eng.routes_all_np), [], None, 0, eng.gather_desc, self._direct_mask,
+                       eng.direct_update_scale(), eng.lr_t.data_ptr())
     else:
       ops.interact_bwd(hb.y, eng.out, self.n_emb, self.dz, hb.dy, 0, 0, 1.0, eng.routes_all,
                        len(eng.routes_all_np), eng.sync_grad_signal(), None, 0)
@@ -268,11 +286,11 @@
       if pushed:
         self._side.wait_stream(self._push_stream)
       with torch.cuda.stream(self._side):
-        eng.backward_inplace()
+        eng.backward_inplace(direct=bool(self._direct_mask))
     else:
       if pushed:
         torch.cuda.current_stream().wait_stream(self._push_stream)
-      eng.backward_inplace()
+      eng.backward_inplace(direct=bool(self._direct_mask))
     ops.relu_bwd_bias(hb.dy, hb.y, hb.gb)
     for i in range(len(self.bottom) - 1, -1, -1):
       L = self.bottom[i]
diff --git a/distributed_embeddings_b200/ops/_native.py b/distributed_embeddings_b200/ops/_native.py
--- a/distributed_embeddings_b200/ops/_native.py
+++ b/distributed_embeddings_b200/ops/_native.py
@@ -94,7 +94,8 @@
     "sync_only": 1, "push_segments": 1, "push_grad": 1, "rowslice_reduce": 1,
     "embedding_lookup_fwd": 1, "embedding_scatter_add": 1, "embedding_lookup_grad": 14,
     "row_to_split": 1, "hash_init": 1, "integer_lookup": 1, "barrier": 1, "allreduce": 1,
-    "gather_segments": 1, "gather_ragged": 1, "copy_cast_2d": 1, "dense_sgd": 1, "interact_fwd": 1, "interact_bwd": 1,
+    "gather_segments": 1, "gather_ragged": 1, "copy_cast_2d": 1, "dense_sgd": 1, "interact_fwd": 1,
+    "interact_fwd_gather": 1, "interact_bwd": 1,
     "relu_bwd_bias": 1, "head_loss": 1, "select_copy": 1, "cast_pad": 1, "gemm_tn_bias_act": 1, "gemm_dgrad_relu_bias": 1,
 }
 _launches = 0
diff --git a/distributed_embeddings_b200/ops/csrc/bindings.cpp b/distributed_embeddings_b200/ops/csrc/bindings.cpp
--- a/distributed_embeddings_b200/ops/csrc/bindings.cpp
+++ b/distributed_embeddings_b200/ops/csrc/bindings.cpp
@@ -746,10 +746,34 @@
   check_launch();
 }
 
+void interact_fwd_gather(const Tensor& bottom, const Tensor& descs, int64_t n_emb, Tensor emb,
+                         Tensor z) {
+  check_bf16_2d(bottom, "bottom");
+  check_bf16_2d(emb, "emb");
+  check_bf16_2d(z, "z");
+  TORCH_CHECK(descs.is_cuda() && descs.scalar_type() == at::kByte &&
+                  descs.numel() >= n_emb * static_cast<int64_t>(sizeof(de::InputDesc)),
+              "descs must be an uploaded InputDesc array with n_emb entries");
+  c10::cuda::CUDAGuard guard(bottom.device());
+  const int64_t dim = bottom.size(1);
+  TORCH_CHECK(emb.size(0) == bottom.size(0) && emb.size(1) == n_emb * dim);
+  const int64_t need = (n_emb + 1) * n_emb / 2 + dim;
+  TORCH_CHECK(z.size(0) == bottom.size(0) && z.size(1) >= need, "z is too narrow");
+  bool ok = de::launch_interact_fwd_gather(
+      bottom.data_ptr(), bottom.stride(0), reinterpret_cast<const de::InputDesc*>(descs.data_ptr()),
+      static_cast<int>(n_emb), static_cast<int>(dim), emb.data_ptr(), emb.stride(0), z.data_ptr(),
+      z.stride(0), static_cast<int>(z.size(1)), bottom.size(0), sm_count(), cur_stream());
+  TORCH_CHECK(ok, "unsupported gathering interaction (n_emb <= 31, dim in {64,128}, 16-byte "
+                  "aligned rows)");
+  check_launch();
+}
+
 void interact_bwd(const Tensor& bottom, const Tensor& emb, int64_t n_emb, const Tensor& dz,
                   Tensor dbottom, int64_t demb_ptr, int64_t demb_stride, double emb_grad_scale,
                   const c10::optional<Tensor>& routes, int64_t n_routes, at::IntArrayRef sync,
-                  const c10::optional<Tensor>& done_counters, int64_t chunk_rows) {
+                  const c10::optional<Tensor>& done_counters, int64_t chunk_rows,
+                  const c10::optional<Tensor>& direct_descs, int64_t direct_mask,
+                  double direct_scale, int64_t lr_ptr) {
   check_bf16_2d(bottom, "bottom");
   check_bf16_2d(emb, "emb");
   check_bf16_2d(dz, "dz");
@@ -757,6 +781,19 @@
   if (routes.has_value())
     TORCH_CHECK(routes->is_cuda() && routes->scalar_type() == at::kByte &&
                 routes->numel() >= n_routes * static_cast<int64_t>(sizeof(de::GradRoute)));
+  de::DirectUpdate direct{};
+  if (direct_mask != 0) {
+    TORCH_CHECK(direct_descs.has_value() && direct_descs->is_cuda() &&
+                    direct_descs->scalar_type() == at::kByte &&
+                    direct_descs->numel() >= n_emb * static_cast<int64_t>(sizeof(de::InputDesc)),
+                "direct update: direct_descs must be an uploaded InputDesc array of n_emb entries");
+    TORCH_CHECK(direct_mask > 0 && direct_mask < (int64_t{1} << n_emb) && lr_ptr != 0,
+                "direct update: mask bits must name features, lr_ptr must be set");
+    direct.descs = reinterpret_cast<const de::InputDesc*>(direct_descs->data_ptr());
+    direct.lr_ptr = reinterpret_cast<const float*>(lr_ptr);
+    direct.scale = static_cast<float>(direct_scale);
+    direct.mask = static_cast<uint32_t>(direct_mask);
+  }
   c10::cuda::CUDAGuard guard(bottom.device());
   const int64_t dim = bottom.size(1);
   bool ok = de::launch_interact_bwd(bottom.data_ptr(), bottom.stride(0), emb.data_ptr(),
@@ -772,7 +809,7 @@
                                     done_counters.has_value()
                                         ? reinterpret_cast<uint32_t*>(done_counters->data_ptr<int>())
                                         : nullptr,
-                                    static_cast<int>(chunk_rows));
+                                    static_cast<int>(chunk_rows), direct);
   TORCH_CHECK(ok, "unsupported interaction shape (n_emb <= 31, dim in {32,64,128}; routed / "
                   "signalling launches need dim in {64,128} and 16-byte aligned rows)");
   check_launch();
@@ -1037,10 +1074,14 @@
         &copy_cast_2d);
   m.def("interact_fwd(Tensor bottom, Tensor emb, int n_emb, Tensor(a!) z, int[] sync) -> ()",
         &interact_fwd);
+  m.def("interact_fwd_gather(Tensor bottom, Tensor descs, int n_emb, Tensor(a!) emb, "
+        "Tensor(b!) z) -> ()",
+        &interact_fwd_gather);
   m.def(
       "interact_bwd(Tensor bottom, Tensor emb, int n_emb, Tensor dz, Tensor(a!) dbottom, "
       "int demb_ptr, int demb_stride, float emb_grad_scale, Tensor? routes, int n_routes, "
-      "int[] sync, Tensor? done_counters, int chunk_rows) -> ()",
+      "int[] sync, Tensor? done_counters, int chunk_rows, Tensor? direct_descs=None, "
+      "int direct_mask=0, float direct_scale=0., int lr_ptr=0) -> ()",
       &interact_bwd);
   m.def("avgpool_fwd(Tensor x, int n, Tensor(a!) out, int stride) -> ()", &avgpool_fwd);
   m.def("avgpool_bwd(Tensor dout, Tensor(a!) dx, int n, int stride) -> ()", &avgpool_bwd);
diff --git a/distributed_embeddings_b200/ops/csrc/de_b200.h b/distributed_embeddings_b200/ops/csrc/de_b200.h
--- a/distributed_embeddings_b200/ops/csrc/de_b200.h
+++ b/distributed_embeddings_b200/ops/csrc/de_b200.h
@@ -185,13 +185,23 @@
                          int64_t emb_stride, int n_emb, int dim, void* z, int64_t z_stride,
                          int z_width, int64_t batch, int sm_count, cudaStream_t stream,
                          const SyncArgs& sync);
+bool launch_interact_fwd_gather(const void* bottom, int64_t bottom_stride, const InputDesc* descs,
+                                int n_emb, int dim, void* emb, int64_t emb_stride, void* z,
+                                int64_t z_stride, int z_width, int64_t batch, int sm_count,
+                                cudaStream_t stream);
+struct DirectUpdate {
+  const InputDesc* descs;
+  const float* lr_ptr;
+  float scale;
+  uint32_t mask;
+};
 bool launch_interact_bwd(const void* bottom, int64_t bottom_stride, const void* emb,
                          int64_t emb_stride, int n_emb, int dim, const void* dz,
                          int64_t dz_stride, void* dbottom, int64_t dbottom_stride, void* demb,
                          int64_t demb_stride, float emb_grad_scale, int64_t batch, int sm_count,
                          cudaStream_t stream, const GradRoute* routes, int n_routes,
                          const SyncArgs& sync, uint32_t* done_counters = nullptr,
-                         int chunk_rows = 0);
+                         int chunk_rows = 0, const DirectUpdate& direct = DirectUpdate{});
 void launch_avgpool_fwd(const void* x, int64_t x_stride, int n, void* out, int64_t out_stride,
                         int out_len, int stride, int left, int64_t rows, cudaStream_t stream);
 void launch_avgpool_bwd(const void* dout, int64_t dout_stride, int out_len, void* dx,
diff --git a/distributed_embeddings_b200/ops/csrc/dense_kernels.cu b/distributed_embeddings_b200/ops/csrc/dense_kernels.cu
--- a/distributed_embeddings_b200/ops/csrc/dense_kernels.cu
+++ b/distributed_embeddings_b200/ops/csrc/dense_kernels.cu
@@ -50,6 +50,14 @@
 }
 __device__ __forceinline__ void cp_async_wait_all() {
   asm volatile("cp.async.commit_group;\ncp.async.wait_group 0;" ::: "memory");
+}
+
+__device__ __forceinline__ void cp_async_commit() {
+  asm volatile("cp.async.commit_group;" ::: "memory");
+}
+template <int N>
+__device__ __forceinline__ void cp_async_wait_group() {
+  asm volatile("cp.async.wait_group %0;" ::"n"(N) : "memory");
 }
 
 template <int D>
@@ -144,6 +152,155 @@
     __syncwarp();
   }
   sync_tail(sync);
+}
+
+__device__ __forceinline__ void cp_async16_zfill(void* smem_dst, const void* gmem_src, int bytes) {
+  asm volatile("cp.async.cg.shared.global [%0], [%1], 16, %2;" ::"r"(smem_u32(smem_dst)),
+               "l"(gmem_src), "r"(bytes)
+               : "memory");
+}
+
+constexpr int kGatherWarps = 2;
+
+__host__ __device__ constexpr int gather_stage_bytes(int d, int n_emb) {
+  return n_emb * d * 4 + d * 2;
+}
+__host__ __device__ constexpr int gather_warp_bytes(int d, int n_emb) {
+  return 2 * gather_stage_bytes(d, n_emb) + fwd_warp_bytes(d);
+}
+
+template <int D>
+__global__ void __launch_bounds__(kGatherWarps * 32)
+interact_fwd_gather_kernel(const bf16* __restrict__ bottom, int64_t bottom_stride,
+                           const InputDesc* __restrict__ descs, int n_emb,
+                           bf16* __restrict__ emb, int64_t emb_stride, bf16* __restrict__ z,
+                           int64_t z_stride, int z_width, int64_t batch) {
+  constexpr int LD = D + 8;
+  constexpr int kRowChunks32 = D / 4;
+  constexpr int kRowChunks16 = D / 8;
+  extern __shared__ __align__(16) unsigned char smem_raw[];
+  const int warp = threadIdx.x >> 5, lane = threadIdx.x & 31;
+  const int stage_bytes = gather_stage_bytes(D, n_emb);
+  unsigned char* wbase = smem_raw + warp * gather_warp_bytes(D, n_emb);
+  bf16* sF = reinterpret_cast<bf16*>(wbase + 2 * stage_bytes);
+  float* sC = reinterpret_cast<float*>(sF);
+  const int nf = n_emb + 1;
+  const int n_inter = nf * (nf - 1) / 2;
+
+  const float* tab = nullptr;
+  const int32_t* ids = nullptr;
+  int64_t id_shift = 0, sub_rows = 0;
+  if (lane < n_emb) {
+    const InputDesc& Df = descs[lane];
+    tab = reinterpret_cast<const float*>(Df.table) + Df.row_base * D;
+    ids = reinterpret_cast<const int32_t*>(Df.ids);
+    id_shift = Df.id_shift;
+    sub_rows = Df.sub_rows;
+  }
+  auto row_of = [&](int32_t id_raw) -> const float* {
+    const int64_t id = static_cast<int64_t>(id_raw) + id_shift;
+    return (lane < n_emb && static_cast<uint64_t>(id) < static_cast<uint64_t>(sub_rows))
+               ? tab + id * D : nullptr;
+  };
+  auto issue = [&](unsigned char* stage, const float* my_row, int64_t s) {
+    const unsigned long long mine = reinterpret_cast<unsigned long long>(my_row);
+    const int total = n_emb * kRowChunks32;
+#pragma unroll 4
+    for (int c = lane; c < total; c += 32) {
+      const int r = c / kRowChunks32, ch = c - r * kRowChunks32;
+      const float* src = reinterpret_cast<const float*>(__shfl_sync(0xffffffffu, mine, r));
+      cp_async16_zfill(stage + c * 16,
+                       src != nullptr ? src + ch * 4 : reinterpret_cast<const float*>(descs),
+                       src != nullptr ? 16 : 0);
+    }
+    if (lane < kRowChunks16)
+      cp_async16(stage + n_emb * D * 4 + lane * 16, bottom + s * bottom_stride + lane * 8);
+  };
+
+  const int64_t stride = static_cast<int64_t>(gridDim.x) * kGatherWarps;
+  int64_t s = static_cast<int64_t>(blockIdx.x) * kGatherWarps + warp;
+  int cur = 0;
+  int32_t id_next = 0;
+  if (s < batch) {
+    issue(wbase, row_of(lane < n_emb ? ids[s] : 0), s);
+    if (s + stride < batch && lane < n_emb) id_next = ids[s + stride];
+  }
+  cp_async_commit();
+  for (; s < batch; s += stride, cur ^= 1) {
+    const int64_t nxt = s + stride;
+    if (nxt < batch) {
+      issue(wbase + (cur ^ 1) * stage_bytes, row_of(id_next), nxt);
+      if (nxt + stride < batch && lane < n_emb) id_next = ids[nxt + stride];
+    }
+    cp_async_commit();
+    cp_async_wait_group<1>();
+    __syncwarp();
+    const float* stage = reinterpret_cast<const float*>(wbase + cur * stage_bytes);
+    const bf16* sb = reinterpret_cast<const bf16*>(stage + n_emb * D);
+    zero_pad_rows<D>(sF, LD, n_emb, lane);
+    bf16* ep = emb + s * emb_stride;
+    for (int c = lane; c < n_emb * kRowChunks16; c += 32) {
+      const int r = c / kRowChunks16, ch = c - r * kRowChunks16;
+      const float4 a = *reinterpret_cast<const float4*>(stage + r * D + ch * 8);
+      const float4 b = *reinterpret_cast<const float4*>(stage + r * D + ch * 8 + 4);
+      uint4 o;
+      o.x = pack2<bf16>(a.x, a.y);
+      o.y = pack2<bf16>(a.z, a.w);
+      o.z = pack2<bf16>(b.x, b.y);
+      o.w = pack2<bf16>(b.z, b.w);
+      *reinterpret_cast<uint4*>(ep + c * 8) = o;
+      *reinterpret_cast<uint4*>(sF + (r + 1) * LD + ch * 8) = o;
+    }
+    if (lane < kRowChunks16)
+      *reinterpret_cast<uint4*>(sF + lane * 8) = *reinterpret_cast<const uint4*>(sb + lane * 8);
+    __syncwarp();
+    float acc0[2][4] = {}, acc1[4][4] = {};
+#pragma unroll
+    for (int k = 0; k < D; k += 16) {
+      uint32_t a0[4], a1[4], b01[4], b23[4];
+      const int arow = lane & 15, acol = k + ((lane >> 4) << 3);
+      ldmatrix_x4(a0, smem_u32(sF + arow * LD + acol));
+      ldmatrix_x4(a1, smem_u32(sF + (16 + arow) * LD + acol));
+      const int brow = (lane & 7) + ((lane >> 4) << 3), bcol = k + (((lane >> 3) & 1) << 3);
+      ldmatrix_x4(b01, smem_u32(sF + brow * LD + bcol));
+      ldmatrix_x4(b23, smem_u32(sF + (16 + brow) * LD + bcol));
+      mma_bf16(acc0[0], a0, b01[0], b01[1]);
+      mma_bf16(acc0[1], a0, b01[2], b01[3]);
+      mma_bf16(acc1[0], a1, b01[0], b01[1]);
+      mma_bf16(acc1[1], a1, b01[2], b01[3]);
+      mma_bf16(acc1[2], a1, b23[0], b23[1]);
+      mma_bf16(acc1[3], a1, b23[2], b23[3]);
+    }
+    __syncwarp();
+    const int cr = lane >> 2, cc = (lane & 3) << 1;
+#pragma unroll
+    for (int nt = 0; nt < 2; ++nt) {
+      sC[cr * 33 + nt * 8 + cc] = acc0[nt][0];
+      sC[cr * 33 + nt * 8 + cc + 1] = acc0[nt][1];
+      sC[(cr + 8) * 33 + nt * 8 + cc] = acc0[nt][2];
+      sC[(cr + 8) * 33 + nt * 8 + cc + 1] = acc0[nt][3];
+    }
+#pragma unroll
+    for (int nt = 0; nt < 4; ++nt) {
+      sC[(16 + cr) * 33 + nt * 8 + cc] = acc1[nt][0];
+      sC[(16 + cr) * 33 + nt * 8 + cc + 1] = acc1[nt][1];
+      sC[(24 + cr) * 33 + nt * 8 + cc] = acc1[nt][2];
+      sC[(24 + cr) * 33 + nt * 8 + cc + 1] = acc1[nt][3];
+    }
+    __syncwarp();
+    bf16* zp = z + s * z_stride;
+    for (int idx = lane; idx < n_inter; idx += 32) {
+      int i = static_cast<int>((1.0f + sqrtf(1.0f + 8.0f * idx)) * 0.5f);
+      while (i * (i - 1) / 2 > idx) --i;
+      while ((i + 1) * i / 2 <= idx) ++i;
+      const int j = idx - i * (i - 1) / 2;
+      zp[idx] = __float2bfloat16_rn(sC[i * 33 + j]);
+    }
+    for (int c = lane; c < D; c += 32) zp[n_inter + c] = sb[c];
+    for (int c = n_inter + D + lane; c < z_width; c += 32) zp[c] = __float2bfloat16_rn(0.f);
+    __syncwarp();
+  }
+  cp_async_wait_group<0>();
 }
 
 template <int D>
@@ -233,13 +390,6 @@
   }
 }
 
-__device__ __forceinline__ void cp_async_commit() {
-  asm volatile("cp.async.commit_group;" ::: "memory");
-}
-template <int N>
-__device__ __forceinline__ void cp_async_wait_group() {
-  asm volatile("cp.async.wait_group %0;" ::"n"(N) : "memory");
-}
 
 constexpr int kDzMax = 512;
 
@@ -258,6 +408,10 @@
   for (int c = lane; c < dz_chunks; c += 32) cp_async16(sDz + c * 8, dz + c * 8);
 }
 
+__device__ __forceinline__ void prefetch_l2_line(const void* p) {
+  asm volatile("prefetch.global.L2 [%0];" ::"l"(p));
+}
+
 struct ChunkDst {
   unsigned long long base;
   long long stride;
@@ -272,7 +426,7 @@
                        float emb_grad_scale, int64_t batch,
                        const GradRoute* __restrict__ routes, int n_routes,
                        const __grid_constant__ SyncArgs sync, uint32_t* __restrict__ done_counters,
-                       int chunk_rows) {
+                       int chunk_rows, const __grid_constant__ DirectUpdate direct) {
   constexpr int LD = D + 8;
   constexpr int LDG = 40;
   constexpr int kWarpElems = 2 * kMaxFeat * LD + 2 * kDzMax + kMaxFeat * LDG;
@@ -288,6 +442,7 @@
   const int n_inter = nf * (nf - 1) / 2;
   const int dz_chunks = (n_inter + D + 7) >> 3;
   const int n_chunks = n_emb * kRowChunks;
+  float** sRow = reinterpret_cast<float**>(sDst + n_chunks) + warp * kMaxFeat;
   if (routes == nullptr) {
     for (int c = threadIdx.x; c < n_chunks; c += blockDim.x) {
       sDst[c].base = reinterpret_cast<unsigned long long>(demb + c * 8);
@@ -315,12 +470,41 @@
     issue_sample<D>(base, LD, sDz0, bottom + s * bottom_stride, emb + s * emb_stride,
                     dz + s * dz_stride, n_emb, dz_chunks, lane);
   cp_async_commit();
+  const bool dlane = (direct.mask >> lane) & 1u;
+  float* dtab = nullptr;
+  const int32_t* dids = nullptr;
+  int64_t dshift = 0, dsub = 0;
+  float dscale = 0.f;
+  int32_t id_c = 0, id_n = 0;
+  if (direct.mask != 0) {
+    dscale = direct.scale * *direct.lr_ptr;
+    if (dlane) {
+      const InputDesc& Df = direct.descs[lane];
+      dtab = reinterpret_cast<float*>(const_cast<void*>(Df.table)) + Df.row_base * D;
+      dids = reinterpret_cast<const int32_t*>(Df.ids);
+      dshift = Df.id_shift;
+      dsub = Df.sub_rows;
+      if (s < batch) id_c = dids[s];
+      if (s + stride < batch) id_n = dids[s + stride];
+    }
+  }
   for (; s < batch; s += stride, cur ^= 1) {
     const int64_t nxt = s + stride;
     if (nxt < batch)
       issue_sample<D>(base + (cur ^ 1) * (kMaxFeat * LD), LD, sDz0 + (cur ^ 1) * kDzMax,
                       bottom + nxt * bottom_stride, emb + nxt * emb_stride, dz + nxt * dz_stride,
                       n_emb, dz_chunks, lane);
+    if (dlane) {
+      const int64_t id = static_cast<int64_t>(id_c) + dshift;
+      sRow[lane] = static_cast<uint64_t>(id) < static_cast<uint64_t>(dsub) ? dtab + id * D : nullptr;
+      const int64_t idn = static_cast<int64_t>(id_n) + dshift;
+      if (nxt < batch && static_cast<uint64_t>(idn) < static_cast<uint64_t>(dsub)) {
+#pragma unroll
+        for (int l = 0; l < D * 4 / 128; ++l) prefetch_l2_line(dtab + idn * D + l * 32);
+      }
+      id_c = id_n;
+      if (nxt + stride < batch) id_n = dids[nxt + stride];
+    }
     cp_async_commit();
     cp_async_wait_group<1>();
     __syncwarp();
@@ -394,9 +578,25 @@
           *reinterpret_cast<const uint4*>(sF + lane * 8);
     for (int c = lane; c < n_chunks; c += 32) {
       const int row = 1 + c / kRowChunks, ch = c - (row - 1) * kRowChunks;
-      const ChunkDst d = sDst[c];
-      *reinterpret_cast<uint4*>(d.base + static_cast<unsigned long long>(s * d.stride)) =
-          *reinterpret_cast<const uint4*>(sF + row * LD + ch * 8);
+      const uint4 v = *reinterpret_cast<const uint4*>(sF + row * LD + ch * 8);
+      if ((direct.mask >> (row - 1)) & 1u) {
+        float* p = sRow[row - 1];
+        if (p != nullptr) {
+          FVec<8> g;
+          const uint32_t w[4] = {v.x, v.y, v.z, v.w};
+#pragma unroll
+          for (int i = 0; i < 4; ++i) {
+            const float2 f = unpack2<bf16>(w[i]);
+            g.v[2 * i] = f.x;
+            g.v[2 * i + 1] = f.y;
+          }
+          g.scale(dscale);
+          red_add_f32<8>(p + ch * 8, g);
+        }
+      } else {
+        const ChunkDst d = sDst[c];
+        *reinterpret_cast<uint4*>(d.base + static_cast<unsigned long long>(s * d.stride)) = v;
+      }
     }
     __syncwarp();
     if (done_counters != nullptr && lane == 0) {
@@ -659,13 +859,50 @@
   return false;
 }
 
+bool launch_interact_fwd_gather(const void* bottom, int64_t bottom_stride, const InputDesc* descs,
+                                int n_emb, int dim, void* emb, int64_t emb_stride, void* z,
+                                int64_t z_stride, int z_width, int64_t batch, int sm_count,
+                                cudaStream_t stream) {
+  if (n_emb < 1 || n_emb + 1 > kMaxFeat || batch <= 0) return false;
+  if (bottom_stride % 8 != 0 || emb_stride % 8 != 0 ||
+      ((reinterpret_cast<uintptr_t>(bottom) | reinterpret_cast<uintptr_t>(emb)) & 15) != 0)
+    return false;
+#define DE_IFWDG(DD)                                                                             \
+  {                                                                                              \
+    const size_t smem = static_cast<size_t>(kGatherWarps) * gather_warp_bytes(DD, n_emb);       \
+    cudaFuncSetAttribute(interact_fwd_gather_kernel<DD>,                                         \
+                         cudaFuncAttributeMaxDynamicSharedMemorySize, static_cast<int>(smem));   \
+    int per_sm = 0;                                                                              \
+    cudaOccupancyMaxActiveBlocksPerMultiprocessor(&per_sm, interact_fwd_gather_kernel<DD>,       \
+                                                  kGatherWarps * 32, smem);                      \
+    if (per_sm < 1) return false;                                                                \
+    int64_t blocks = (batch + kGatherWarps - 1) / kGatherWarps;                                  \
+    const int64_t cap = static_cast<int64_t>(sm_count) * per_sm;                                 \
+    if (blocks > cap) blocks = cap;                                                              \
+    interact_fwd_gather_kernel<DD><<<static_cast<unsigned>(blocks), kGatherWarps * 32, smem,     \
+                                     stream>>>(                                                  \
+        reinterpret_cast<const bf16*>(bottom), bottom_stride, descs, n_emb,                      \
+        reinterpret_cast<bf16*>(emb), emb_stride, reinterpret_cast<bf16*>(z), z_stride, z_width, \
+        batch);                                                                                  \
+    return true;                                                                                 \
+  }
+  if (dim == 128) DE_IFWDG(128)
+  if (dim == 64) DE_IFWDG(64)
+#undef DE_IFWDG
+  return false;
+}
+
 bool launch_interact_bwd(const void* bottom, int64_t bottom_stride, const void* emb,
                          int64_t emb_stride, int n_emb, int dim, const void* dz,
                          int64_t dz_stride, void* dbottom, int64_t dbottom_stride, void* demb,
                          int64_t demb_stride, float emb_grad_scale, int64_t batch, int sm_count,
                          cudaStream_t stream, const GradRoute* routes, int n_routes,
-                         const SyncArgs& sync, uint32_t* done_counters, int chunk_rows) {
+                         const SyncArgs& sync, uint32_t* done_counters, int chunk_rows,
+                         const DirectUpdate& direct) {
   if (n_emb + 1 > kMaxFeat || batch <= 0 || dim % 32 != 0) return false;
+  if (direct.mask != 0 &&
+      (direct.descs == nullptr || direct.lr_ptr == nullptr || (direct.mask >> n_emb) != 0))
+    return false;
   int64_t blocks = (batch + kWarps - 1) / kWarps;
   const int64_t cap = static_cast<int64_t>(sm_count) * 8;
   if (blocks > cap) blocks = cap;
@@ -682,23 +919,27 @@
         reinterpret_cast<uintptr_t>(emb) | reinterpret_cast<uintptr_t>(dbottom)) & 15) == 0 &&
       (dim == 128 || dim == 64) &&
       (routes != nullptr || (demb_stride % 8 == 0 && (reinterpret_cast<uintptr_t>(demb) & 15) == 0));
-  if ((routes != nullptr || done_counters != nullptr) && !v2_ok) return false;
+  if ((routes != nullptr || done_counters != nullptr || direct.mask != 0) && !v2_ok)
+    return false;
   const bool has_sync = sync.state != nullptr && (sync.wait_ch >= 0 || sync.signal_ch >= 0);
-  if (v2_ok && (!force_v1 || routes != nullptr || has_sync || done_counters != nullptr)) {
+  if (v2_ok &&
+      (!force_v1 || routes != nullptr || has_sync || done_counters != nullptr || direct.mask)) {
     int64_t blocks2 = (batch + kWarps - 1) / kWarps;
     if (blocks2 > static_cast<int64_t>(sm_count) * 2) blocks2 = static_cast<int64_t>(sm_count) * 2;
 #define DE_IBWD2(DD)                                                                             \
   {                                                                                              \
     const size_t smem =                                                                          \
         kWarps * (2 * kMaxFeat * (DD + 8) + 2 * kDzMax + kMaxFeat * 40) * sizeof(bf16) +         \
-        static_cast<size_t>(n_emb) * (DD / 8) * sizeof(ChunkDst);                                \
+        static_cast<size_t>(n_emb) * (DD / 8) * sizeof(ChunkDst) +                               \
+        kWarps * kMaxFeat * sizeof(float*);                                                      \
     cudaFuncSetAttribute(interact_bwd_v2_kernel<DD>,                                             \
                          cudaFuncAttributeMaxDynamicSharedMemorySize, static_cast<int>(smem));   \
     interact_bwd_v2_kernel<DD><<<static_cast<unsigned>(blocks2), kWarps * 32, smem, stream>>>(   \
         reinterpret_cast<const bf16*>(bottom), bottom_stride, reinterpret_cast<const bf16*>(emb), \
         emb_stride, n_emb, reinterpret_cast<const bf16*>(dz), dz_stride,                         \
         reinterpret_cast<bf16*>(dbottom), dbottom_stride, reinterpret_cast<bf16*>(demb),         \
-        demb_stride, emb_grad_scale, batch, routes, n_routes, sync, done_counters, chunk_rows);  \
+        demb_stride, emb_grad_scale, batch, routes, n_routes, sync, done_counters, chunk_rows,   \
+        direct);                                                                                 \
     return true;                                                                                 \
   }
     if (dim == 128) DE_IBWD2(128)
diff --git a/distributed_embeddings_b200/parallel/fused.py b/distributed_embeddings_b200/parallel/fused.py
--- a/distributed_embeddings_b200/parallel/fused.py
+++ b/distributed_embeddings_b200/parallel/fused.py
@@ -24,6 +24,22 @@
 
 def _weight(layer):
   return layer.embeddings
+
+
+GATHER_INTERACTION_DIMS = (64, 128)
+DIRECT_UPDATE_MIN_ROWS = 16384
+
+
+def gather_interaction_eligible(*, world, table_dtype, has_offload, n_replicated, n_row_sliced,
+                                dp_input, hots, ids64, compute_dtype, dim, widths, cols,
+                                out_stride) -> bool:
+  n = len(widths)
+  return (world == 1 and table_dtype == torch.float32 and not has_offload and
+          n_replicated == 0 and n_row_sliced == 0 and dp_input and
+          1 <= n <= 31 and len(hots) == n and all(h == 1 for h in hots) and not ids64 and
+          compute_dtype == torch.bfloat16 and dim in GATHER_INTERACTION_DIMS and
+          all(w == dim for w in widths) and sorted(cols) == [j * dim for j in range(n)] and
+          out_stride == n * dim)
 
 
 def _dev_ptr(t: torch.Tensor) -> int:
@@ -531,8 +547,40 @@
         len(ddesc) > 0 and (tw * csz) % 16 == 0 and \
         all((int(w) * csz) % 16 == 0 and int(w) * csz <= 256 for w in ddesc["width"]) and \
         all((int(c) * csz) % 16 == 0 for c in ddesc["dst_col"])
+    self.gather_desc_np = self._gather_descs(cdesc, hots, ids64, ostride)
+    self.mpdesc_hot_np = mp[mp["sub_rows"] < DIRECT_UPDATE_MIN_ROWS] \
+        if self.gather_desc_np is not None else None
     self._upload()
     self._key = (b, hots, ids64)
+
+  def _gather_descs(self, cdesc, hots, ids64: bool, ostride: int):
+    de = self.de
+    widths = [int(w) for w in cdesc["width"]]
+    dim = widths[0] if widths else 0
+    ok = gather_interaction_eligible(
+        world=self.W, table_dtype=self.table_dtype, has_offload=self.has_offload,
+        n_replicated=len(de.dp_layers), n_row_sliced=len(self.rdesc_np), dp_input=de.dp_input,
+        hots=hots, ids64=ids64, compute_dtype=self.compute_dtype, dim=dim,
+        widths=widths, cols=[int(c) for c in cdesc["dst_col"]],
+        out_stride=ostride)
+    if not ok:
+      return None
+    return cdesc[np.argsort(cdesc["dst_col"], kind="stable")].copy()
+
+  def direct_update_mask(self) -> int:
+    opt = self.de._fused_optimizer
+    if self.gather_desc_np is None or opt is None or opt["kind"] != "sgd" or \
+        opt.get("deterministic", False) or not self.staged_update:
+      return 0
+    return sum(1 << f for f, r in enumerate(self.gather_desc_np["sub_rows"])
+               if int(r) >= DIRECT_UPDATE_MIN_ROWS)
+
+  def direct_update_scale(self) -> float:
+    return -(0.0 if self._dry_updates else self.de.mp_grad_scale)
+
+  @property
+  def gather_interaction_dim(self) -> Optional[int]:
+    return int(self.gather_desc_np["width"][0]) if self.gather_desc_np is not None else None
 
   def _upload(self):
     dev = self.device
@@ -549,6 +597,9 @@
           self.fwd_launches.append((up(d, dev), int(mask.sum()), self._tile_samples(d, hot[mask])))
     self.fwd_rs_tile = self._tile_samples(self.fwd_rs_np, self._desc_hotness(self.fwd_rs_np)) \
         if len(self.fwd_rs_np) else 32
+    self.gather_desc = up(self.gather_desc_np, dev) if self.gather_desc_np is not None else None
+    self.mpdesc_hot = up(self.mpdesc_hot_np, dev) \
+        if self.mpdesc_hot_np is not None and len(self.mpdesc_hot_np) else None
     self.ddesc = up(self.ddesc_np, dev) if len(self.ddesc_np) else None
     self.mpdesc = up(self.mpdesc_np, dev) if len(self.mpdesc_np) else None
     self.routes_mp = up(self.routes_mp_np, dev) if len(self.routes_mp_np) else None
@@ -836,18 +887,18 @@
   def sync_grad_signal(self):
     return self._sync(signal=CH_GRAD) if (self.W > 1 and self.mpdesc is not None) else []
 
-  def backward_inplace(self):
+  def backward_inplace(self, direct: bool = False):
     if len(self.de.dp_layers):
       if getattr(self, "_dp_targets", None) is None:
         raise RuntimeError("backward_inplace needs set_dp_grad_targets() for replicated tables")
       self._scatter_dp_grads()
-    self._backward_mp()
-
-  def _backward_mp(self) -> List[Optional[torch.Tensor]]:
+    self._backward_mp(direct)
+
+  def _backward_mp(self, direct: bool = False) -> List[Optional[torch.Tensor]]:
     with nvtx.range("emb_backward_update"):
-      return self._backward_mp_impl()
-
-  def _backward_mp_impl(self) -> List[Optional[torch.Tensor]]:
+      return self._backward_mp_impl(direct)
+
+  def _backward_mp_impl(self, direct: bool = False) -> List[Optional[torch.Tensor]]:
     ops, de = self.ops, self.de
     n_mp = len(self.mp_layers)
     if self.mpdesc is None:
@@ -864,6 +915,14 @@
       self._refresh_tables()
     B = self.B
     gscale = 0.0 if self._dry_updates else de.mp_grad_scale
+    if direct:
+      if not self.direct_update_mask():
+        raise RuntimeError("backward_inplace(direct=True) needs a plan with direct updates")
+      if self.mpdesc_hot is not None:
+        ops.scatter_add_bwd(self.mpdesc_hot, len(self.mpdesc_hot_np), B, B, B, self.recv_width,
+                            [], self.recv_ptr, 0, -gscale, self.lr_t.data_ptr(), self.ids64,
+                            self.act, self.vec4, self.vec8, [], self.staged_update)
+      return [None] * n_mp
     if opt is not None and opt["kind"] == "sgd" and not opt.get("deterministic", False) and \
         not self.has_offload and self.tab == 0:
       ops.scatter_add_bwd(self.mpdesc, self.n_mp_inputs, B, B, B, self.recv_width, [],
```

Measured after the change: 18.58 million (median of 6 runs). 1.09x the previous value.
